# robustrobotics/multi_view_stereonet

Measured on AMD Instinct MI355X. Metric: depthmaps/sec at 512x256, 64 hypotheses, 2 src views; L1 vs ref, higher is better.
Workload: dtype f32; 1 GPU; GTA-SfM-shaped 512x256, D=64 hypotheses, 2 source views, cost-volume filter + 5 refiners; global_batch=256, parallelism=dp1 (independent images, all-gather of metric rows)

## Files before the change

include/mvsn_hip.h:

```cpp
#ifndef MVSN_HIP_H
#define MVSN_HIP_H

#include <stddef.h>
#include <stdint.h>

#ifdef __cplusplus
extern "C" {
#endif

#define MVSN_ABI_VERSION 7

#define MVSN_E_BADARG (-1)
#define MVSN_E_TOOLARGE (-2)
#define MVSN_E_WORKSPACE (-3)

typedef void *mvsn_stream_t;

int mvsn_abi_version(void);
const char *mvsn_last_error(void);

int mvsn_plane_sweep_setup(const float *T_right_in_left, const float *K_lvl0, const float *K_lvl4,
                           int n_chains, int rows4, int cols4, int num_idepth_samples,
                           float *idepth_samples, float *H_lvl4, float *H_inc, float *H_lvl0_plane0,
                           float *baseline, mvsn_stream_t stream);
int mvsn_plane_sweep_setup_sources(const float *const *T_right_in_lefts, int n_sources, const float *K_lvl0,
                                   const float *K_lvl4, int batch, int rows4, int cols4, int num_idepth_samples,
                                   float *idepth_samples, float *H_lvl4, float *H_inc, float *H_lvl0_plane0,
                                   float *baseline, mvsn_stream_t stream);

int mvsn_plane_sweep_setup_path(const float *K_lvl0_host, const float *K_lvl4_host, int rows4, int cols4);

int mvsn_homography_warp(const float *image, const float *H, int batch, int channels, int n_planes,
                         int rows, int cols, float *volume, uint8_t *mask, mvsn_stream_t stream);

#define MVSN_CHAIN_AUTO 0
#define MVSN_CHAIN_DIRECT 1
#define MVSN_CHAIN_WINOGRAD 2
#define MVSN_CHAIN_STEPWISE 3
#define MVSN_CHAIN_BANDED 4
size_t mvsn_feature_refiner_packed_floats(void);
int mvsn_pack_feature_refiner(const float *conv0_w, const float *conv0_b, const float *bn0_w,
                              const float *bn0_b, const float *res0_w, const float *res0_b,
                              const float *res0_bn_w, const float *res0_bn_b, const float *final_w,
                              const float *final_b, float *packed, mvsn_stream_t stream);
size_t mvsn_incremental_cost_volume_workspace_bytes(int n_chains, int rows, int cols);
int mvsn_incremental_cost_volume_form(int rows, int cols);
int mvsn_incremental_cost_volume_form_for(int n_chains, int rows, int cols);
size_t mvsn_incremental_cost_volume_workspace_bytes_for(int n_chains, int num_idepth_samples, int rows, int cols,
                                                        int form);
int mvsn_incremental_cost_volume_resolve(int n_chains, int num_idepth_samples, int rows, int cols, int form,
                                         int coresident_allowed, int guarded, size_t out[8]);
size_t mvsn_incremental_cost_volume_status_offset(int n_chains, int rows, int cols);
int mvsn_incremental_cost_volume_banded_groups(int n_chains, int rows, int cols);
int mvsn_incremental_cost_volume(const float *src_image_lvl4, const float *H_lvl4, const float *H_inc,
                                 const float *plane0_features, const float *left_features,
                                 const float *refiner_packed, int n_chains, int batch,
                                 int num_idepth_samples, int rows, int cols, float *cost_volume,
                                 uint8_t *mask_volume, float *feature_volume, void *workspace,
                                 size_t workspace_bytes, int form, mvsn_stream_t stream);
size_t mvsn_incremental_cost_volume_repair_workspace_bytes(int n_chains, int rows, int cols);
int mvsn_incremental_cost_volume_guarded(const float *src_image_lvl4, const float *H_lvl4, const float *H_inc,
                                         const float *plane0_features, const float *left_features,
                                         const float *refiner_packed, int n_chains, int batch,
                                         int num_idepth_samples, int rows, int cols, float *cost_volume,
                                         uint8_t *mask_volume, float *feature_volume, void *workspace,
                                         size_t workspace_bytes, int form, void *repair_workspace,
                                         size_t repair_workspace_bytes, unsigned *sticky_status, mvsn_stream_t stream);
int mvsn_incremental_cost_volume_bf16(const float *src_image_lvl4, const float *H_lvl4, const float *H_inc,
                                         const float *plane0_features, const float *left_features,
                                         const float *refiner_packed, int n_chains, int batch,
                                         int num_idepth_samples, int rows, int cols, void *cost_volume_bf16,
                                         uint8_t *mask_volume, float *feature_volume, void *workspace,
                                         size_t workspace_bytes, int form, void *repair_workspace,
                                         size_t repair_workspace_bytes, unsigned *sticky_status, mvsn_stream_t stream);

typedef struct {
  int n;
  int c_in;
  int c_out;
  int depth;
  int rows, cols;
  int kd, kh, kw;
  int stride;
  int dilation;
  int precision;
} mvsn_conv_desc;

#define MVSN_CONV_FP32 0
#define MVSN_CONV_BF16X3 1
#define MVSN_CONV_FP32_WINO 2
#define MVSN_CONV_BF16 3
int mvsn_conv_bf16x3_supported(const mvsn_conv_desc *desc);
int mvsn_conv_forward_bf16_storage(const mvsn_conv_desc *desc, const void *in, int in_is_bf16,
                                   const float *weight_packed, const float *bias, const float *in_stats,
                                   const float *in_gamma, const float *in_beta, void *out, int out_is_bf16,
                                   float *out_partials, mvsn_stream_t stream);
int mvsn_conv_winograd_supported(const mvsn_conv_desc *desc);

size_t mvsn_conv_packed_floats(const mvsn_conv_desc *desc);
int mvsn_conv_pack_weights(const mvsn_conv_desc *desc, const float *weight, float *packed,
                           mvsn_stream_t stream);
int mvsn_conv_num_tiles(const mvsn_conv_desc *desc);
int mvsn_conv_forward(const mvsn_conv_desc *desc, const float *in, const float *weight_packed,
                      const float *bias, const float *in_stats, const float *in_gamma,
                      const float *in_beta, const float *in_residual, float *out_staged, float *out,
                      float *out_partials, mvsn_stream_t stream);
int mvsn_conv_forward_blocks(const mvsn_conv_desc *desc, const float *const *in_blocks, const int *block_channels,
                             int num_blocks, const float *weight_packed, const float *bias, float *out,
                             float *out_partials, mvsn_stream_t stream);
typedef struct mvsn_apply_job {
  const float *x, *stats, *gamma, *beta;
  const float *residual, *r_stats, *r_gamma, *r_beta;
  float *out;
  int n;
  int reverse;
  long spatial;
} mvsn_apply_job;
int mvsn_conv_forward_carry(const mvsn_conv_desc *desc, const float *in, const float *weight_packed, const float *bias,
                            const float *in_stats, const float *in_gamma, const float *in_beta, float *out,
                            float *out_partials, const mvsn_apply_job *job, int *carried, mvsn_stream_t stream);
int mvsn_groupnorm_finalize(const float *partials, int n, int tiles, float *stats, mvsn_stream_t stream);
size_t mvsn_groupnorm_finalize_split_workspace_bytes(int n, int tiles);
int mvsn_groupnorm_finalize_split(const float *partials, int n, int tiles, float *stats, void *workspace,
                                  size_t workspace_bytes, mvsn_stream_t stream);
int mvsn_groupnorm_lrelu_apply(const float *x, const float *stats, int stat_tiles, const float *gamma, const float *beta,
                               const float *residual, const float *r_stats, const float *r_gamma, const float *r_beta,
                               int n, long spatial, float *out, mvsn_stream_t stream);

int mvsn_conv_to1_supported(int rows, int cols);
int mvsn_conv_to1(const float *in, const float *weight, const float *bias, const float *prior, const float *fx,
                  int n, int depth, int rows, int cols, int kd, float *out, mvsn_stream_t stream);
int mvsn_conv_to1_volume_norm(const float *in_raw, const float *in_stats, const float *in_gamma, const float *in_beta,
                              const float *weight, const float *bias, int n, int depth, int rows, int cols, float *out,
                              mvsn_stream_t stream);
int mvsn_conv_to1_block(const float *in_raw, const float *in_stats, int stat_tiles, const float *in_gamma,
                        const float *in_beta, const float *in_residual, const float *weight, const float *bias,
                        const float *prior, const float *fx, int n, int rows, int cols, float *out, mvsn_stream_t stream);

int mvsn_soft_argmin(const float *cost, const float *idepth_samples, int n, int num_idepth_samples,
                     int pixels, float *idepth, mvsn_stream_t stream);

int mvsn_soft_argmin_confidence(const float *cost, const float *idepth_samples, int n, int num_idepth_samples,
                                int pixels, float *idepth, float *confidence, mvsn_stream_t stream);
int mvsn_confidence_fuse_sources(const float *confidence, int n_sources, int batch, int pixels, float *out,
                                 mvsn_stream_t stream);
int mvsn_confidence_mask(const float *confidence, const uint8_t *valid, long count, float min_confidence,
                         uint8_t *out, mvsn_stream_t stream);
int mvsn_fusion_gather(const float *maps, const int *view, const int *pixel, int n_views, long pixels_per_view,
                       long count, float *out, mvsn_stream_t stream);

int mvsn_channel_l2_norm(const float *x, int n, int channels, long pixels, float *out, mvsn_stream_t stream);
int mvsn_idepth_scale(const float *prior, const float *fx, int n, long pixels, float *out, mvsn_stream_t stream);
int mvsn_refiner_epilogue(const float *prior, const float *fx, const float *delta, int n, long pixels, float *out,
                          mvsn_stream_t stream);

int mvsn_upsample_bilinear(const float *in, int n, int channels, int rows_in, int cols_in, int rows_out,
                           int cols_out, float *out, mvsn_stream_t stream);
int mvsn_upsample_prior(const float *in, const float *fx, int n, int rows_in, int cols_in, int rows_out, int cols_out,
                        float *out, float *out_scaled, mvsn_stream_t stream);
int mvsn_upsample_mask(const uint8_t *in, int n, int channels, int rows_in, int cols_in, int rows_out,
                       int cols_out, uint8_t *out, mvsn_stream_t stream);

int mvsn_area_downsample(const float *in, int n, int channels, int rows_in, int cols_in, float *out,
                         mvsn_stream_t stream);

int mvsn_image_pyramid_supported(int rows, int cols, int levels);
int mvsn_image_pyramid(const float *in, int n, int channels, int rows, int cols, int levels, float *const *out_levels,
                       mvsn_stream_t stream);
int mvsn_prepare_cameras(const float *K, const float *T_right_in_left, int batch, int n_sources, int levels,
                         const int *level_sizes_dev, float *K_pyr, float *T_normalised, float *T_inverse_normalised,
                         float *baseline, mvsn_stream_t stream);

int mvsn_fuse_sources(const float *raw, const float *refined, const float *baseline, const uint8_t *mask,
                      int n_sources, int batch, int num_idepth_samples, int pixels, int refined_aliases_raw,
                      float *raw_out, float *refined_out, uint8_t *mask_out, mvsn_stream_t stream);

int mvsn_idepth_reproject_blocks(int pixels);
int mvsn_idepth_reproject(const float *K, const float *T_other_in_this, const float *idepth, const float *other_idepth,
                          const uint8_t *other_mask, int batch, int rows, int cols, float *idepth_in_other,
                          float *other_sampled, uint8_t *other_mask_sampled, uint8_t *invalid, float *uv,
                          float *absdiff_partials, mvsn_stream_t stream);
int mvsn_occlusion_mask(const float *idepth_in_other, const float *other_sampled, const uint8_t *invalid,
                        const float *absdiff_partials, int batch, int pixels, uint8_t *mask, mvsn_stream_t stream);
int mvsn_masked_l1(const float *a, const float *b, const uint8_t *skip_a, const uint8_t *skip_b, long n, int accumulate,
                   float *loss, mvsn_stream_t stream);

typedef struct {
  const float *in[3];
  int channels[3], sample_mod[3];
  const float *block_scale;
  int scale_mod, scale_block;
  int head_chunks, n_blocks;
  int dilation[6];
  const float *weights, *params;
  int tail_mode;
  const float *prior, *fx;
  int fx_mod;
  float *out;
} mvsn_tower_desc;
int mvsn_tower_16x32(const mvsn_tower_desc *desc, int n_samples, mvsn_stream_t stream);

int mvsn_depth_metrics_blocks(long pixels);
int mvsn_depth_metrics(const float *idepth_est, const float *depth_true, const float *baseline, int batch, long pixels,
                       float min_depth, float max_depth, double *partials, double *rows, mvsn_stream_t stream);

size_t mvsn_fusion_workspace_bytes(int n_ref, int n_slots, int rows, int cols);
int mvsn_fusion_consistency(const float *depth, const uint8_t *valid, const float *K, const float *T_cam_in_world,
                            const int *ref_views, const int *neighbours, int n_views, int n_ref, int n_slots, int rows,
                            int cols, float max_reproj_px, float max_rel_depth, int min_consistent, float *fused_depth,
                            uint8_t *count, int64_t *total, void *workspace, size_t workspace_bytes,
                            mvsn_stream_t stream);
int mvsn_fusion_emit(const float *fused_depth, const float *images, const int *ref_views, int n_ref, int rows, int cols,
                     int n_slots, const void *workspace, size_t workspace_bytes, long capacity, float *points,
                     uint8_t *colors, int *view, int *pixel, mvsn_stream_t stream);

#define MVSN_VOXEL_STATUS_RANGE 1
#define MVSN_VOXEL_STATUS_TABLE 2
size_t mvsn_voxel_workspace_bytes(long n);
int mvsn_voxel_assign(const float *points, long n, float voxel_size, float inv_voxel_size, float origin_x,
                      float origin_y, float origin_z, int64_t *result, void *workspace, size_t workspace_bytes,
                      mvsn_stream_t stream);
int mvsn_voxel_merge(const float *points, const uint8_t *colors, long n, float voxel_size, float inv_voxel_size,
                     float origin_x, float origin_y, float origin_z, void *workspace, size_t workspace_bytes,
                     long capacity, void *accumulators, float *out_points, uint8_t *out_colors, int *count,
                     int64_t *first, int64_t *inverse, mvsn_stream_t stream);

int mvsn_depth_normals(const float *depth, const uint8_t *valid, const float *K, const float *T_cam_in_world,
                       int n_views, int rows, int cols, float max_rel_step, float *normals, mvsn_stream_t stream);
int mvsn_normals_gather(const float *normals, const int *view, const int *pixel, int n_views, long pixels_per_view,
                        long count, float *out, mvsn_stream_t stream);
int mvsn_voxel_normals(const float *normals, const int64_t *inverse, long n, long m, void *accumulators, float *out,
                       mvsn_stream_t stream);

#define MVSN_CLOUD_STATUS_RANGE 1
#define MVSN_CLOUD_STATUS_TABLE 2
size_t mvsn_cloud_workspace_bytes(long n_target);
int mvsn_cloud_index_build(const float *target, long n, float cell, float inv_cell, int64_t *status, void *workspace,
                           size_t workspace_bytes, mvsn_stream_t stream);
int mvsn_cloud_nearest(const float *query, long nq, float inv_cell, float r2, const void *workspace,
                       size_t workspace_bytes, long n_target, float *dist2, int64_t *index, int *within,
                       mvsn_stream_t stream);

size_t mvsn_cloud_register_workspace_bytes(long n_source);
int mvsn_cloud_register_system(const float *source, long n_source, const float *weights, const float *target,
                               const float *target_normals, long n_target, float inv_cell, float r2,
                               const void *index_workspace, size_t index_workspace_bytes, const float *T,
                               const float *centre, void *workspace, size_t workspace_bytes, double *H, double *b,
                               double *sums, int64_t *index, float *residual, mvsn_stream_t stream);
int mvsn_cloud_register(const float *source, long n_source, const float *weights, const float *target,
                        const float *target_normals, long n_target, float inv_cell, float r2,
                        const void *index_workspace, size_t index_workspace_bytes, const float *T_init,
                        const float *centre, int iterations, long min_points, double min_pivot, void *workspace,
                        size_t workspace_bytes, float *T_out, double *history, int *status, double *information,
                        mvsn_stream_t stream);

int mvsn_cloud_normals(const float *query, long nq, const float *viewpoint, long viewpoint_rows, float cell,
                       float inv_cell, float r2, long min_neighbours, double min_gap, const void *index_workspace,
                       size_t index_workspace_bytes, long n_target, float *normals, float *eigenvalues, int *count,
                       mvsn_stream_t stream);

int mvsn_cloud_knn(const float *query, long nq, int k, int exclude_self, float cell, float inv_cell, float r2,
                   const void *index_workspace, size_t index_workspace_bytes, long n_target, float *dist2,
                   int64_t *index, int *within, double *mean, mvsn_stream_t stream);
size_t mvsn_cloud_mean_stats_workspace_bytes(long n);
int mvsn_cloud_mean_stats(const double *mean, long n, void *workspace, size_t workspace_bytes, double *stats,
                          mvsn_stream_t stream);

int mvsn_cloud_fpfh(const float *points, const float *normals, long n, float cell, float inv_cell, float r2,
                    long min_neighbours, const void *index_workspace, size_t index_workspace_bytes, int *spfh,
                    int *pairs, float *features, mvsn_stream_t stream);
int mvsn_cloud_feature_nearest(const float *query, long nq, const float *target, long nt, int dim, int64_t *index,
                               float *dist2, float *second_dist2, mvsn_stream_t stream);
int mvsn_cloud_feature_mutual(const int64_t *index, long nq, const int64_t *back, long nt, unsigned char *mutual,
                              mvsn_stream_t stream);
size_t mvsn_cloud_ransac_workspace_bytes(void);
int mvsn_cloud_ransac(const float *source, long ns, const float *target, long nt, const int64_t *correspondences, long c,
                      float r2, double edge_similarity, long hypotheses, unsigned long long seed, void *workspace,
                      size_t workspace_bytes, float *T, double *T64, int64_t *best, unsigned char *inlier,
                      mvsn_stream_t stream);

int mvsn_tsdf_camera_batch(void);
int mvsn_tsdf_integrate(const float *depth, const uint8_t *valid, const float *weights, const float *images,
                        const float *K, const float *T_cam_in_world, int n_views, int rows, int cols, int nx, int ny,
                        int nz, float voxel_size, float origin_x, float origin_y, float origin_z, float trunc,
                        float min_depth, float *sdf_sum, float *weight, float *color_sum, mvsn_stream_t stream);
size_t mvsn_tsdf_workspace_bytes(int nx, int ny, int nz);
int mvsn_tsdf_classify(const float *sdf_sum, const float *weight, int nx, int ny, int nz, float min_weight,
                       int64_t *result, void *workspace, size_t workspace_bytes, mvsn_stream_t stream);
int mvsn_tsdf_extract(const float *sdf_sum, const float *weight, const float *color_sum, int nx, int ny, int nz,
                      float voxel_size, float origin_x, float origin_y, float origin_z, float min_weight,
                      const void *workspace, size_t workspace_bytes, long n_vertices, long n_quads, float *vertices,
                      float *normals, uint8_t *colors, int64_t *faces, int64_t *cell, mvsn_stream_t stream);

size_t mvsn_tsdf_raycast_workspace_bytes(int nx, int ny, int nz);
int mvsn_tsdf_raycast(const float *sdf_sum, const float *weight, const float *color_sum, int nx, int ny, int nz,
                      float voxel_size, float origin_x, float origin_y, float origin_z, const float *K,
                      const float *T_cam_in_world, int n_views, int rows, int cols, float min_weight, float min_depth,
                      float max_depth, float step, void *workspace, size_t workspace_bytes, float *depth,
                      float *normals, float *colors, float *weight_out, mvsn_stream_t stream);

size_t mvsn_tsdf_align_workspace_bytes(int nx, int ny, int nz, int n_views, int rows, int cols, int stride);
int mvsn_tsdf_align_system(const float *sdf_sum, const float *weight, int nx, int ny, int nz, float voxel_size,
                           float origin_x, float origin_y, float origin_z, const float *depth, const uint8_t *valid,
                           const float *weights, const float *K, const float *T_cam_in_world, int n_views, int rows,
                           int cols, int stride, float min_weight, float band, void *workspace, size_t workspace_bytes,
                           double *H, double *b, double *sums, float *residual, mvsn_stream_t stream);
int mvsn_tsdf_align(const float *sdf_sum, const float *weight, int nx, int ny, int nz, float voxel_size, float origin_x,
                    float origin_y, float origin_z, const float *depth, const uint8_t *valid, const float *weights,
                    const float *K, const float *T_cam_in_world, int n_views, int rows, int cols, int stride,
                    float min_weight, float band, int iterations, long min_pixels, double min_pivot, void *workspace,
                    size_t workspace_bytes, float *T_out, double *history, int *status, double *information,
                    mvsn_stream_t stream);

#define MVSN_MESH_STATUS_WORKSPACE 1
size_t mvsn_mesh_workspace_bytes(long n_vertices, long n_faces);
int mvsn_mesh_components_label(const int64_t *faces, long n_vertices, long n_faces, int64_t *result, void *workspace,
                               size_t workspace_bytes, mvsn_stream_t stream);
int mvsn_mesh_components_emit(const int64_t *faces, long n_vertices, long n_faces, void *workspace,
                              size_t workspace_bytes, long n_components, int64_t *vertex_label, int64_t *face_label,
                              int64_t *vertex_count, int64_t *face_count, int64_t *first, mvsn_stream_t stream);
int mvsn_mesh_select(const int64_t *vertex_label, const int64_t *face_label, const uint8_t *keep, long n_vertices,
                     long n_faces, long n_components, int64_t *result, void *workspace, size_t workspace_bytes,
                     mvsn_stream_t stream);
int mvsn_mesh_compact(const float *vertices, const float *normals, const uint8_t *colors, const int64_t *cell,
                      const int64_t *faces, const int64_t *face_label, const uint8_t *keep, long n_vertices, long n_faces,
                      long n_components, const void *workspace, size_t workspace_bytes, long n_vertices_out,
                      long n_faces_out, float *out_vertices, float *out_normals, uint8_t *out_colors, int64_t *out_cell,
                      int64_t *out_faces, int64_t *vertex_rows, int64_t *face_rows, mvsn_stream_t stream);

#define MVSN_CLUSTER_STATUS_WORKSPACE 1
size_t mvsn_cloud_cluster_workspace_bytes(long n);
int mvsn_cloud_cluster_label(const float *points, long n, float inv_cell, float r2, long min_points,
                             const void *index_workspace, size_t index_workspace_bytes, int *within, uint8_t *core,
                             int64_t *result, void *workspace, size_t workspace_bytes, mvsn_stream_t stream);
int mvsn_cloud_cluster_emit(const float *points, long n, float inv_cell, float r2, const void *index_workspace,
                            size_t index_workspace_bytes, const uint8_t *core, void *workspace, size_t workspace_bytes,
                            long n_clusters, int64_t *label, int64_t *count, int64_t *core_count, int64_t *first,
                            mvsn_stream_t stream);

#define MVSN_RENDER_MAX_RADIUS 8
size_t mvsn_cloud_render_workspace_bytes(int n_views, int rows, int cols);
int mvsn_cloud_render_camera_batch(void);
int mvsn_cloud_render(const float *points, long n, const uint8_t *colors, const float *normals, const float *K,
                      const float *T_cam_in_world, int n_views, int rows, int cols, int radius, float min_depth,
                      float max_depth, void *workspace, size_t workspace_bytes, float *depth, int64_t *index,
                      uint8_t *out_colors, float *out_normals, mvsn_stream_t stream);
int mvsn_cloud_visibility(const float *points, long n, const float *depth, const float *maps, int channels,
                          const float *K, const float *T_cam_in_world, int n_views, int rows, int cols, float rel_tol,
                          float min_depth, uint8_t *visible, int *count, float *values, mvsn_stream_t stream);

#define MVSN_MESH_SAMPLE_STATUS_NO_AREA 1
size_t mvsn_mesh_sample_workspace_bytes(long n_faces);
int mvsn_mesh_sample_prefix(const float *vertices, long n_vertices, const int64_t *faces, long n_faces, int64_t *result,
                            void *workspace, size_t workspace_bytes, mvsn_stream_t stream);
int mvsn_mesh_sample_draw(const float *vertices, long n_vertices, const int64_t *faces, long n_faces,
                          const void *workspace, size_t workspace_bytes, long n, uint64_t seed, const float *normals,
                          const uint8_t *colors, float *points, int64_t *face, float *weights, float *out_normals,
                          uint8_t *out_colors, mvsn_stream_t stream);

#define MVSN_MESH_NEAREST_BOX_CELLS 512
#define MVSN_MESH_NEAREST_STATUS_RANGE 1
int mvsn_mesh_nearest_box_cells(void);
size_t mvsn_mesh_nearest_workspace_bytes(long n_pairs, long n_large);
int mvsn_mesh_nearest_count(const float *vertices, long n_vertices, const int64_t *faces, long n_faces, float inv_cell,
                            int64_t *result, mvsn_stream_t stream);
int mvsn_mesh_nearest_build(const float *vertices, long n_vertices, const int64_t *faces, long n_faces, float inv_cell,
                            long n_pairs, long n_large, void *workspace, size_t workspace_bytes, mvsn_stream_t stream);
int mvsn_mesh_nearest(const float *query, long nq, const float *vertices, long n_vertices, const int64_t *faces,
                      long n_faces, float inv_cell, float r2, long n_pairs, long n_large, const void *workspace,
                      size_t workspace_bytes, float *dist2, int64_t *face, float *point, float *weights, int *within,
                      mvsn_stream_t stream);

int mvsn_copy(void *dst, const void *src, size_t nbytes, mvsn_stream_t stream);
int mvsn_copy_many(void *const *dst, const void *const *src, const size_t *nbytes, int count, mvsn_stream_t stream);
int mvsn_gather_focal(const float *const *K_pyr, int levels, int batch, float *fx, mvsn_stream_t stream);
int mvsn_gather_strided(const float *src, int count, long stride, float *dst, mvsn_stream_t stream);

int mvsn_debug_set_band_flags(int flags);

int mvsn_debug_set_wino_rowphase(int mode);

int mvsn_debug_wino_plan(const mvsn_conv_desc *desc, int carrying, int out[8]);

int mvsn_debug_conv_plan(const mvsn_conv_desc *desc, int mode, int out[8]);

int mvsn_selftest_mfma(mvsn_stream_t stream);

#ifdef __cplusplus
}
#endif
#endif
```

multi_view_stereonet_amd/_native.py:

```python
import ctypes
import os
from ctypes import c_char_p, c_int, c_long, c_size_t, c_void_p, POINTER, Structure

import torch

_LIB_PATH = os.path.join(os.path.dirname(os.path.abspath(__file__)), "libmvsn_hip.so")
_lib = None


class ConvDesc(Structure):
    _fields_ = [("n", c_int), ("c_in", c_int), ("c_out", c_int), ("depth", c_int), ("rows", c_int),
                ("cols", c_int), ("kd", c_int), ("kh", c_int), ("kw", c_int), ("stride", c_int),
                ("dilation", c_int), ("precision", c_int)]


class ApplyJob(Structure):
    _fields_ = [("x", c_void_p), ("stats", c_void_p), ("gamma", c_void_p), ("beta", c_void_p),
                ("residual", c_void_p), ("r_stats", c_void_p), ("r_gamma", c_void_p), ("r_beta", c_void_p),
                ("out", c_void_p), ("n", c_int), ("reverse", c_int), ("spatial", c_long)]


class TowerDesc(Structure):
    _fields_ = [("inp", c_void_p * 3), ("channels", c_int * 3), ("sample_mod", c_int * 3), ("block_scale", c_void_p),
                ("scale_mod", c_int), ("scale_block", c_int), ("head_chunks", c_int), ("n_blocks", c_int),
                ("dilation", c_int * 6), ("weights", c_void_p), ("params", c_void_p), ("tail_mode", c_int),
                ("prior", c_void_p), ("fx", c_void_p), ("fx_mod", c_int), ("out", c_void_p)]


CONV_FP32, CONV_BF16X3, CONV_FP32_WINO, CONV_BF16 = 0, 1, 2, 3
CHAIN_AUTO, CHAIN_DIRECT, CHAIN_WINOGRAD, CHAIN_STEPWISE, CHAIN_BANDED = 0, 1, 2, 3, 4
ABI_VERSION = 7


SIGNATURES = {
    "mvsn_abi_version": (c_int, []),
    "mvsn_last_error": (c_char_p, []),
    "mvsn_plane_sweep_setup": (c_int, [c_void_p] * 3 + [c_int] * 4 + [c_void_p] * 5 + [c_void_p]),
    "mvsn_plane_sweep_setup_sources": (c_int, [POINTER(c_void_p), c_int, c_void_p, c_void_p] + [c_int] * 4 + [c_void_p] * 5 + [c_void_p]),
    "mvsn_plane_sweep_setup_path": (c_int, [c_void_p, c_void_p, c_int, c_int]),
    "mvsn_gather_focal": (c_int, [POINTER(c_void_p), c_int, c_int, c_void_p, c_void_p]),
    "mvsn_homography_warp": (c_int, [c_void_p] * 2 + [c_int] * 5 + [c_void_p] * 2 + [c_void_p]),
    "mvsn_feature_refiner_packed_floats": (c_size_t, []),
    "mvsn_pack_feature_refiner": (c_int, [c_void_p] * 11 + [c_void_p]),
    "mvsn_incremental_cost_volume_workspace_bytes": (c_size_t, [c_int] * 3),
    "mvsn_incremental_cost_volume_form": (c_int, [c_int] * 2),
    "mvsn_incremental_cost_volume_form_for": (c_int, [c_int] * 3),
    "mvsn_incremental_cost_volume_workspace_bytes_for": (c_size_t, [c_int] * 5),
    "mvsn_incremental_cost_volume_resolve": (c_int, [c_int] * 7 + [POINTER(c_size_t * 8)]),
    "mvsn_incremental_cost_volume_status_offset": (c_size_t, [c_int] * 3),
    "mvsn_incremental_cost_volume_banded_groups": (c_int, [c_int] * 3),
    "mvsn_incremental_cost_volume": (c_int, [c_void_p] * 6 + [c_int] * 5 + [c_void_p] * 4 + [c_size_t, c_int, c_void_p]),
    "mvsn_incremental_cost_volume_repair_workspace_bytes": (c_size_t, [c_int] * 3),
    "mvsn_incremental_cost_volume_guarded": (c_int, [c_void_p] * 6 + [c_int] * 5 + [c_void_p] * 4 +
                                             [c_size_t, c_int, c_void_p, c_size_t, c_void_p, c_void_p]),
    "mvsn_incremental_cost_volume_bf16": (c_int, [c_void_p] * 6 + [c_int] * 5 + [c_void_p] * 4 +
                                          [c_size_t, c_int, c_void_p, c_size_t, c_void_p, c_void_p]),
    "mvsn_conv_bf16x3_supported": (c_int, [POINTER(ConvDesc)]),
    "mvsn_conv_forward_bf16_storage": (c_int, [c_void_p, c_void_p, c_int, c_void_p, c_void_p, c_void_p, c_void_p, c_void_p,
                                               c_void_p, c_int, c_void_p, c_void_p]),
    "mvsn_conv_winograd_supported": (c_int, [POINTER(ConvDesc)]),
    "mvsn_conv_packed_floats": (c_size_t, [POINTER(ConvDesc)]),
    "mvsn_conv_pack_weights": (c_int, [POINTER(ConvDesc), c_void_p, c_void_p, c_void_p]),
    "mvsn_conv_num_tiles": (c_int, [POINTER(ConvDesc)]),
    "mvsn_conv_forward": (c_int, [POINTER(ConvDesc)] + [c_void_p] * 10 + [c_void_p]),
    "mvsn_conv_forward_blocks": (c_int, [POINTER(ConvDesc), c_void_p, POINTER(c_int), c_int] + [c_void_p] * 4 + [c_void_p]),
    "mvsn_conv_forward_carry": (c_int, [POINTER(ConvDesc)] + [c_void_p] * 8 + [POINTER(ApplyJob), POINTER(c_int), c_void_p]),
    "mvsn_groupnorm_finalize": (c_int, [c_void_p, c_int, c_int, c_void_p, c_void_p]),
    "mvsn_groupnorm_finalize_split_workspace_bytes": (c_size_t, [c_int, c_int]),
    "mvsn_groupnorm_finalize_split": (c_int, [c_void_p, c_int, c_int, c_void_p, c_void_p, c_size_t, c_void_p]),
    "mvsn_groupnorm_lrelu_apply": (c_int, [c_void_p] * 2 + [c_int] + [c_void_p] * 6 + [c_int, c_long, c_void_p, c_void_p]),
    "mvsn_conv_to1_block": (c_int, [c_void_p] * 2 + [c_int] + [c_void_p] * 7 + [c_int] * 3 + [c_void_p, c_void_p]),
    "mvsn_debug_set_band_flags": (c_int, [c_int]),
    "mvsn_debug_set_wino_rowphase": (c_int, [c_int]),
    "mvsn_debug_wino_plan": (c_int, [POINTER(ConvDesc), c_int, POINTER(c_int * 8)]),
    "mvsn_debug_conv_plan": (c_int, [POINTER(ConvDesc), c_int, POINTER(c_int * 8)]),
    "mvsn_copy_many": (c_int, [c_void_p, c_void_p, c_void_p, c_int, c_void_p]),
    "mvsn_conv_to1_supported": (c_int, [c_int, c_int]),
    "mvsn_conv_to1_volume_norm": (c_int, [c_void_p] * 6 + [c_int] * 4 + [c_void_p, c_void_p]),
    "mvsn_conv_to1": (c_int, [c_void_p] * 5 + [c_int] * 5 + [c_void_p, c_void_p]),
    "mvsn_soft_argmin": (c_int, [c_void_p] * 2 + [c_int] * 3 + [c_void_p, c_void_p]),
    "mvsn_soft_argmin_confidence": (c_int, [c_void_p] * 2 + [c_int] * 3 + [c_void_p] * 2 + [c_void_p]),
    "mvsn_confidence_fuse_sources": (c_int, [c_void_p] + [c_int] * 3 + [c_void_p, c_void_p]),
    "mvsn_confidence_mask": (c_int, [c_void_p, c_void_p, c_long, ctypes.c_float, c_void_p, c_void_p]),
    "mvsn_fusion_gather": (c_int, [c_void_p] * 3 + [c_int, c_long, c_long, c_void_p, c_void_p]),
    "mvsn_channel_l2_norm": (c_int, [c_void_p, c_int, c_int, c_long, c_void_p, c_void_p]),
    "mvsn_idepth_scale": (c_int, [c_void_p, c_void_p, c_int, c_long, c_void_p, c_void_p]),
    "mvsn_refiner_epilogue": (c_int, [c_void_p, c_void_p, c_void_p, c_int, c_long, c_void_p, c_void_p]),
    "mvsn_upsample_bilinear": (c_int, [c_void_p] + [c_int] * 6 + [c_void_p, c_void_p]),
    "mvsn_upsample_prior": (c_int, [c_void_p, c_void_p] + [c_int] * 5 + [c_void_p] * 3),
    "mvsn_upsample_mask": (c_int, [c_void_p] + [c_int] * 6 + [c_void_p, c_void_p]),
    "mvsn_image_pyramid_supported": (c_int, [c_int] * 3),
    "mvsn_image_pyramid": (c_int, [c_void_p] + [c_int] * 5 + [POINTER(c_void_p), c_void_p]),
    "mvsn_prepare_cameras": (c_int, [c_void_p] * 2 + [c_int] * 3 + [c_void_p] * 5 + [c_void_p]),
    "mvsn_area_downsample": (c_int, [c_void_p] + [c_int] * 4 + [c_void_p, c_void_p]),
    "mvsn_fuse_sources": (c_int, [c_void_p] * 4 + [c_int] * 5 + [c_void_p] * 3 + [c_void_p]),
    "mvsn_idepth_reproject_blocks": (c_int, [c_int]),
    "mvsn_idepth_reproject": (c_int, [c_void_p] * 5 + [c_int] * 3 + [c_void_p] * 6 + [c_void_p]),
    "mvsn_occlusion_mask": (c_int, [c_void_p] * 4 + [c_int] * 2 + [c_void_p, c_void_p]),
    "mvsn_masked_l1": (c_int, [c_void_p] * 4 + [c_long, c_int, c_void_p, c_void_p]),
    "mvsn_tower_16x32": (c_int, [POINTER(TowerDesc), c_int, c_void_p]),
    "mvsn_depth_metrics_blocks": (c_int, [c_long]),
    "mvsn_depth_metrics": (c_int, [c_void_p] * 3 + [c_int, c_long, ctypes.c_float, ctypes.c_float, c_void_p, c_void_p, c_void_p]),
    "mvsn_fusion_workspace_bytes": (c_size_t, [c_int] * 4),
    "mvsn_fusion_consistency": (c_int, [c_void_p] * 6 + [c_int] * 5 + [ctypes.c_float] * 2 + [c_int] + [c_void_p] * 4 +
                                [c_size_t, c_void_p]),
    "mvsn_fusion_emit": (c_int, [c_void_p] * 3 + [c_int] * 4 + [c_void_p, c_size_t, c_long] + [c_void_p] * 4 + [c_void_p]),
    "mvsn_voxel_workspace_bytes": (c_size_t, [c_long]),
    "mvsn_voxel_assign": (c_int, [c_void_p, c_long] + [ctypes.c_float] * 5 + [c_void_p, c_void_p, c_size_t, c_void_p]),
    "mvsn_voxel_merge": (c_int, [c_void_p, c_void_p, c_long] + [ctypes.c_float] * 5 + [c_void_p, c_size_t, c_long] +
                         [c_void_p] * 6 + [c_void_p]),
    "mvsn_depth_normals": (c_int, [c_void_p] * 4 + [c_int] * 3 + [ctypes.c_float, c_void_p, c_void_p]),
    "mvsn_normals_gather": (c_int, [c_void_p] * 3 + [c_int, c_long, c_long, c_void_p, c_void_p]),
    "mvsn_voxel_normals": (c_int, [c_void_p, c_void_p, c_long, c_long, c_void_p, c_void_p, c_void_p]),
    "mvsn_cloud_workspace_bytes": (c_size_t, [c_long]),
    "mvsn_cloud_index_build": (c_int, [c_void_p, c_long] + [ctypes.c_float] * 2 + [c_void_p, c_void_p, c_size_t, c_void_p]),
    "mvsn_cloud_nearest": (c_int, [c_void_p, c_long] + [ctypes.c_float] * 2 + [c_void_p, c_size_t, c_long] +
                           [c_void_p] * 3 + [c_void_p]),
    "mvsn_cloud_register_workspace_bytes": (c_size_t, [c_long]),
    "mvsn_cloud_register_system": (c_int, [c_void_p, c_long] + [c_void_p] * 3 + [c_long] + [ctypes.c_float] * 2 +
                                   [c_void_p, c_size_t] + [c_void_p] * 2 + [c_void_p, c_size_t] + [c_void_p] * 5 + [c_void_p]),
    "mvsn_cloud_register": (c_int, [c_void_p, c_long] + [c_void_p] * 3 + [c_long] + [ctypes.c_float] * 2 +
                            [c_void_p, c_size_t] + [c_void_p] * 2 + [c_int, c_long, ctypes.c_double, c_void_p, c_size_t] +
                            [c_void_p] * 4 + [c_void_p]),
    "mvsn_cloud_normals": (c_int, [c_void_p, c_long, c_void_p, c_long] + [ctypes.c_float] * 3 + [c_long, ctypes.c_double] +
                           [c_void_p, c_size_t, c_long] + [c_void_p] * 3 + [c_void_p]),
    "mvsn_cloud_knn": (c_int, [c_void_p, c_long, c_int, c_int] + [ctypes.c_float] * 3 + [c_void_p, c_size_t, c_long] +
                       [c_void_p] * 4 + [c_void_p]),
    "mvsn_cloud_mean_stats_workspace_bytes": (c_size_t, [c_long]),
    "mvsn_cloud_mean_stats": (c_int, [c_void_p, c_long, c_void_p, c_size_t, c_void_p, c_void_p]),
    "mvsn_cloud_fpfh": (c_int, [c_void_p, c_void_p, c_long] + [ctypes.c_float] * 3 + [c_long, c_void_p, c_size_t] +
                        [c_void_p] * 3 + [c_void_p]),
    "mvsn_cloud_feature_nearest": (c_int, [c_void_p, c_long, c_void_p, c_long, c_int] + [c_void_p] * 3 + [c_void_p]),
    "mvsn_cloud_feature_mutual": (c_int, [c_void_p, c_long, c_void_p, c_long, c_void_p, c_void_p]),
    "mvsn_cloud_ransac_workspace_bytes": (c_size_t, []),
    "mvsn_cloud_ransac": (c_int, [c_void_p, c_long, c_void_p, c_long, c_void_p, c_long, ctypes.c_float, ctypes.c_double,
                                  c_long, ctypes.c_uint64, c_void_p, c_size_t] + [c_void_p] * 4 + [c_void_p]),
    "mvsn_tsdf_camera_batch": (c_int, []),
    "mvsn_tsdf_integrate": (c_int, [c_void_p] * 6 + [c_int] * 6 + [ctypes.c_float] * 6 + [c_void_p] * 3 + [c_void_p]),
    "mvsn_tsdf_workspace_bytes": (c_size_t, [c_int] * 3),
    "mvsn_tsdf_classify": (c_int, [c_void_p] * 2 + [c_int] * 3 + [ctypes.c_float, c_void_p, c_void_p, c_size_t, c_void_p]),
    "mvsn_tsdf_extract": (c_int, [c_void_p] * 3 + [c_int] * 3 + [ctypes.c_float] * 5 + [c_void_p, c_size_t, c_long, c_long] +
                          [c_void_p] * 5 + [c_void_p]),
    "mvsn_tsdf_raycast_workspace_bytes": (c_size_t, [c_int] * 3),
    "mvsn_tsdf_raycast": (c_int, [c_void_p] * 3 + [c_int] * 3 + [ctypes.c_float] * 4 + [c_void_p] * 2 + [c_int] * 3 +
                          [ctypes.c_float] * 4 + [c_void_p, c_size_t] + [c_void_p] * 4 + [c_void_p]),
    "mvsn_tsdf_align_workspace_bytes": (c_size_t, [c_int] * 7),
    "mvsn_tsdf_align_system": (c_int, [c_void_p] * 2 + [c_int] * 3 + [ctypes.c_float] * 4 + [c_void_p] * 5 + [c_int] * 4 +
                               [ctypes.c_float] * 2 + [c_void_p, c_size_t] + [c_void_p] * 4 + [c_void_p]),
    "mvsn_tsdf_align": (c_int, [c_void_p] * 2 + [c_int] * 3 + [ctypes.c_float] * 4 + [c_void_p] * 5 + [c_int] * 4 +
                        [ctypes.c_float] * 2 + [c_int, c_long, ctypes.c_double, c_void_p, c_size_t] + [c_void_p] * 4 + [c_void_p]),
    "mvsn_mesh_workspace_bytes": (c_size_t, [c_long] * 2),
    "mvsn_mesh_components_label": (c_int, [c_void_p, c_long, c_long, c_void_p, c_void_p, c_size_t, c_void_p]),
    "mvsn_mesh_components_emit": (c_int, [c_void_p, c_long, c_long, c_void_p, c_size_t, c_long] + [c_void_p] * 5 + [c_void_p]),
    "mvsn_mesh_select": (c_int, [c_void_p] * 3 + [c_long] * 3 + [c_void_p, c_void_p, c_size_t, c_void_p]),
    "mvsn_mesh_compact": (c_int, [c_void_p] * 7 + [c_long] * 3 + [c_void_p, c_size_t, c_long, c_long] + [c_void_p] * 7 +
                          [c_void_p]),
    "mvsn_mesh_sample_workspace_bytes": (c_size_t, [c_long]),
    "mvsn_mesh_sample_prefix": (c_int, [c_void_p, c_long, c_void_p, c_long, c_void_p, c_void_p, c_size_t, c_void_p]),
    "mvsn_mesh_sample_draw": (c_int, [c_void_p, c_long, c_void_p, c_long, c_void_p, c_size_t, c_long, ctypes.c_uint64] +
                              [c_void_p] * 7 + [c_void_p]),
    "mvsn_mesh_nearest_box_cells": (c_int, []),
    "mvsn_mesh_nearest_workspace_bytes": (c_size_t, [c_long] * 2),
    "mvsn_mesh_nearest_count": (c_int, [c_void_p, c_long, c_void_p, c_long, ctypes.c_float, c_void_p, c_void_p]),
    "mvsn_mesh_nearest_build": (c_int, [c_void_p, c_long, c_void_p, c_long, ctypes.c_float, c_long, c_long, c_void_p,
                                        c_size_t, c_void_p]),
    "mvsn_mesh_nearest": (c_int, [c_void_p, c_long, c_void_p, c_long, c_void_p, c_long] + [ctypes.c_float] * 2 +
                          [c_long, c_long, c_void_p, c_size_t] + [c_void_p] * 5 + [c_void_p]),
    "mvsn_cloud_cluster_workspace_bytes": (c_size_t, [c_long]),
    "mvsn_cloud_cluster_label": (c_int, [c_void_p, c_long] + [ctypes.c_float] * 2 + [c_long, c_void_p, c_size_t] +
                                 [c_void_p] * 3 + [c_void_p, c_size_t] + [c_void_p]),
    "mvsn_cloud_cluster_emit": (c_int, [c_void_p, c_long] + [ctypes.c_float] * 2 + [c_void_p, c_size_t, c_void_p] +
                                [c_void_p, c_size_t, c_long] + [c_void_p] * 4 + [c_void_p]),
    "mvsn_cloud_render_workspace_bytes": (c_size_t, [c_int] * 3),
    "mvsn_cloud_render_camera_batch": (c_int, []),
    "mvsn_cloud_render": (c_int, [c_void_p, c_long] + [c_void_p] * 4 + [c_int] * 4 + [ctypes.c_float] * 2 +
                          [c_void_p, c_size_t] + [c_void_p] * 4 + [c_void_p]),
    "mvsn_cloud_visibility": (c_int, [c_void_p, c_long, c_void_p, c_void_p, c_int, c_void_p, c_void_p] + [c_int] * 3 +
                              [ctypes.c_float] * 2 + [c_void_p] * 3 + [c_void_p]),
    "mvsn_copy": (c_int, [c_void_p, c_void_p, c_size_t, c_void_p]),
    "mvsn_gather_strided": (c_int, [c_void_p, c_int, c_long, c_void_p, c_void_p]),
    "mvsn_selftest_mfma": (c_int, [c_void_p]),
}


def library_path() -> str:
    return _LIB_PATH


def load():
    global _lib
    if _lib is not None:
        return _lib
    if not os.path.exists(_LIB_PATH):
        raise RuntimeError(
            f"{_LIB_PATH} is missing: the HIP extension has not been built "
            "(run `python -m multi_view_stereonet_amd.build` or __graft_entry__.build()). "
            "There is no CPU fallback for the plane-sweep path.")
    lib = ctypes.CDLL(_LIB_PATH)
    lib.mvsn_abi_version.restype, lib.mvsn_abi_version.argtypes = c_int, []
    if lib.mvsn_abi_version() != ABI_VERSION:
        raise RuntimeError(f"libmvsn_hip.so is ABI version {lib.mvsn_abi_version()}, this package needs {ABI_VERSION}: "
                           "rebuild it (python -m multi_view_stereonet_amd.build --force)")
    for name, (res, args) in SIGNATURES.items():
        fn = getattr(lib, name)
        fn.restype = res
        fn.argtypes = args
    _lib = lib
    return lib


def ptr(t):
    if t is None:
        return None
    if not t.is_cuda:
        raise RuntimeError("libmvsn_hip.so takes device (HBM) pointers; got a CPU tensor")
    if not t.is_contiguous():
        raise RuntimeError("libmvsn_hip.so takes dense tensors")
    return t.data_ptr()


def stream():
    return torch.cuda.current_stream().cuda_stream


def plane_sweep_setup_path(K_lvl0, K_lvl4, rows4: int, cols4: int):
    lib = load()
    K0, K4 = (k.detach().to("cpu", torch.float32).contiguous() for k in (K_lvl0, K_lvl4))
    return [lib.mvsn_plane_sweep_setup_path(K0[n].data_ptr(), K4[n].data_ptr(), rows4, cols4) for n in range(K0.shape[0])]


def check(rc: int, what: str):
    if rc != 0:
        msg = load().mvsn_last_error()
        raise RuntimeError(f"{what} failed (code {rc}): {msg.decode() if msg else ''}")


_coresident = {}


def _device_key(index: int) -> str:
    p = torch.cuda.get_device_properties(index)
    uuid = getattr(p, "uuid", None)
    if uuid is not None and str(uuid).strip("0-") != "":
        return str(uuid)
    return "pci-%04x-%02x-%02x" % (getattr(p, "pci_domain_id", 0), getattr(p, "pci_bus_id", index),
                                   getattr(p, "pci_device_id", 0))


def coresident_lock_path(index: int) -> str:
    root = os.environ.get("MVSN_LOCK_DIR") or "/tmp"
    return os.path.join(root, "mvsn_coresident_%s.lock" % _device_key(index).replace("/", "_"))


def coresident_right(index: int) -> bool:
    if index in _coresident:
        return _coresident[index][0]
    if os.environ.get("MVSN_CORESIDENT_LOCK", "1") == "0":
        _coresident[index] = (True, None)
        return True
    import fcntl
    try:
        old_mask = os.umask(0)
        try:
            f = os.fdopen(os.open(coresident_lock_path(index), os.O_RDWR | os.O_CREAT, 0o666), "r+")
        finally:
            os.umask(old_mask)
    except OSError:
        _coresident[index] = (True, None)
        return True
    try:
        fcntl.flock(f, fcntl.LOCK_EX | fcntl.LOCK_NB)
    except OSError:
        f.close()
        _coresident[index] = (False, None)
        return False
    try:
        f.seek(0)
        f.truncate()
        f.write("%d\n" % os.getpid())
        f.flush()
    except OSError:
        pass
    _coresident[index] = (True, f)
    return True


def release_coresident_right(index=None):
    for i in ([index] if index is not None else list(_coresident)):
        granted, f = _coresident.pop(i, (False, None))
        if f is not None:
            f.close()
```

multi_view_stereonet_amd/csrc/mvsn_conv.hip:

```cpp
#include "mvsn_resident.h"
#include "mvsn_conv_bf16x3.h"
#include "mvsn_conv_wino.h"

namespace mvsn {

constexpr int CV_THREADS = 256;
constexpr int CV_WAVES = 4;
constexpr int CV_TX = 32;
constexpr int CV_CK = 4;

#ifndef MVSN_TALL_TILE_MAX_DIL
#define MVSN_TALL_TILE_MAX_DIL 8
#endif
#ifndef MVSN_DMA_MAX_DIL
#define MVSN_DMA_MAX_DIL 8
#endif
constexpr int HD_TY = 8, HD_TX = 32, HD_ROWS = 2 * HD_TY + 3, HD_XS = 2 * HD_TX + 8;
constexpr int HD_CST = HD_ROWS * HD_XS + 4;

struct FastDiv {
  unsigned mul, shift;
};
static FastDiv make_fastdiv(unsigned d) {
  unsigned s = 0;
// ... 396 lines not shown
          }
        }
      }
    }
#pragma unroll
    for (int k = 0; k < WR; ++k) {
      const int idx = (tid + k * CV_THREADS) * 4;
      if (idx < WFL) *reinterpret_cast<floatx4 *>(wl + idx) = wreg[k];
    }
  };

#ifdef MVSN_DMA_STAMPS
  __shared__ unsigned long long ph_lds[8];
  const bool stamped = g_dma_stamps && blockIdx.x == gridDim.x / 3 && blockIdx.y == gridDim.y / 2 && tid == 0;
  unsigned long long ph_last = __builtin_readcyclecounter();
  const unsigned long long ph_t0 = ph_last;
  if (stamped) for (int k = 0; k < 8; ++k) ph_lds[k] = 0;
#endif
  stage_load(0);
  MFMA_PHASE(0);
  for (int chunk = 0; chunk < g.nchunks; ++chunk) {
    __syncthreads();
    MFMA_PHASE(1);
    stage_store(chunk);
    MFMA_PHASE(2);
    __syncthreads();
    MFMA_PHASE(3);
    if (chunk + 1 < g.nchunks) stage_load(chunk + 1);
    MFMA_PHASE(4);
    const float *wt = wl + lane;
    float fw[2][2], fb[2][NPT];
    auto read_tap = [&](int tap, int buf) {
      const int tz = tap / (KH * KW), ty = (tap / KW) % KH, tx = tap % KW;
      const float *bp = tile + (tz * g.HY + ty * g.dil) * g.XS + tx * g.dil;
      fw[buf][0] = wt[tap * 128];
      fw[buf][1] = CT == 2 ? wt[tap * 128 + 64] : 0.0f;
#pragma unroll
      for (int j = 0; j < NPT; ++j) fb[buf][j] = bp[lpos[j]];
    };
    if constexpr (KD == 1 && KW == 5 && STRIDE == 2 && V4) {
      float2 er[2][NPT][3];
      auto read_row = [&](int ky, int buf) {
        const float *bp = tile + ky * g.XS;
#pragma unroll
        for (int j = 0; j < NPT; ++j)
#pragma unroll
          for (int q = 0; q < 3; ++q) er[buf][j][q] = *reinterpret_cast<const float2 *>(bp + lpos[j] + 2 * q);
      };
      read_row(0, 0);
      fw[0][0] = wt[0], fw[0][1] = CT == 2 ? wt[64] : 0.0f;
#pragma unroll
      for (int ky = 0; ky < 5; ++ky) {
        const int rb = ky & 1;
        if (ky + 1 < 5) read_row(ky + 1, rb ^ 1);
#pragma unroll
        for (int kx = 0; kx < 5; ++kx) {
          const int tap = ky * 5 + kx, cur = tap & 1;
          if (tap + 1 < NTAPS) {
            fw[cur ^ 1][0] = wt[(tap + 1) * 128];
            fw[cur ^ 1][1] = CT == 2 ? wt[(tap + 1) * 128 + 64] : 0.0f;
          }
#pragma unroll
          for (int j = 0; j < NPT; ++j) {
            const float a = (kx & 1) ? er[rb][j][kx >> 1].y : er[rb][j][kx >> 1].x;
            acc[j][0] = mfma16x16x4(a, fw[cur][0], acc[j][0]);
            if (CT == 2) acc[j][CT - 1] = mfma16x16x4(a, fw[cur][1], acc[j][CT - 1]);
          }
        }
      }
    } else {
    read_tap(0, 0);
#pragma unroll
    for (int tap = 0; tap < NTAPS; ++tap) {
      const int cur = tap & 1;
      if (tap + 1 < NTAPS) read_tap(tap + 1, cur ^ 1);
#pragma unroll
      for (int j = 0; j < NPT; ++j) {
        acc[j][0] = mfma16x16x4(fb[cur][j], fw[cur][0], acc[j][0]);
        if (CT == 2) acc[j][CT - 1] = mfma16x16x4(fb[cur][j], fw[cur][1], acc[j][CT - 1]);
      }
    }
    }
    MFMA_PHASE(5);
  }

  conv_epilogue<NPT, CT>(g, acc, z0, y0, x0, tid, n, tile_id, bias, out, out_partials);
#ifdef MVSN_DMA_STAMPS
  MFMA_PHASE(6);
  if (stamped) {
    for (int k = 0; k < 7; ++k) g_dma_stamps[32 + k] = ph_lds[k];
    g_dma_stamps[39] = __builtin_readcyclecounter() - ph_t0;
  }
#endif
}

__device__ floatx4 g_zero16 = {0.f, 0.f, 0.f, 0.f};

template <int NPT, int IPC, int CT, int MODE>
__global__ __launch_bounds__(CV_THREADS, MODE <= 1 ? 4 : 2) void conv_dma_kernel(ConvGeom g, const float *__restrict__ in,
                                                                 const float *__restrict__ wpk,
                                                                 const float *__restrict__ bias,
                                                                 const float *__restrict__ in_stats,
                                                                 const float *__restrict__ in_gamma,
                                                                 const float *__restrict__ in_beta,
                                                                 const float *__restrict__ in_residual,
                                                                 float *__restrict__ out_staged,
                                                                 float *__restrict__ out,
                                                                 float *__restrict__ out_partials) {
  extern __shared__ __attribute__((aligned(16))) float smem[];
  constexpr ConvForm L{CV_DMA, NPT, 1, 3, 1, IPC, false};
  constexpr int NTAPS = 9;
  constexpr int WFL = L.wfl(), WSLOT = L.wslot(), NT = L.ntiles(MODE);
  constexpr int WRUNS = WSLOT / 256;
  const int tile_floats = CV_CK * g.dCST;
  const int stage_floats = tile_floats * NT + WSLOT;
  float *scsh = smem + 2 * stage_floats;

  const int tid = threadIdx.x, lane = tid & 63;
  const int wave = __builtin_amdgcn_readfirstlane(tid >> 6);
  const int n = blockIdx.y;
#ifdef MVSN_DMA_STAMPS
  unsigned long long *dbg = (blockIdx.x == gridDim.x / 3 && blockIdx.y == gridDim.y / 2 && tid == 0) ? g_dma_stamps : nullptr;
  int dbg_i = 0;
#endif
  DMA_STAMP();
#ifdef MVSN_DMA_STAMPS
  if (dbg) dbg[62] = wall_clock64();
#endif
  const int tile_id = xcd_tile_index(blockIdx.x, g.tiles);
  const int trow = fdiv(tile_id, g.fd_ntx), txi = tile_id - trow * g.ntx;
  const int tzi = fdiv(trow, g.fd_nty), tyi = trow - tzi * g.nty;
  const int z0 = tzi * g.TZ, y0 = tyi * g.TY, x0 = txi * CV_TX;
  const int gz0 = z0 - g.pd, gy0 = y0 - g.ph, gx0 = x0 - g.pw;
  const size_t in_plane = (size_t)g.H * g.W, in_chan = (size_t)g.D * in_plane;
  const float *inn = in + (size_t)n * g.cin * in_chan;
  const float *resn = (MODE == 2 && in_residual) ? in_residual + (size_t)n * g.cin * in_chan : nullptr;
  float *stgn = (MODE == 2 && out_staged) ? out_staged + (size_t)n * g.cin * in_chan : nullptr;

  int lpos[NPT];
#pragma unroll
  for (int j = 0; j < NPT; ++j) {
    const int pt = wave * NPT + j;
    const int xt = pt & 1, zz = fdiv(pt >> 1, g.fd_ty), yy = (pt >> 1) - zz * g.TY;
    const int xx = xt * 16 + (lane & 15);
    lpos[j] = (zz * g.HY + yy) * g.dXS + xx + (g.dpa - g.pw) + (lane >> 4) * g.dCST;
  }

  int goff[IPC];
  unsigned inimg = 0, interior = 0;
  const int tile_groups = g.HZ * g.HY * g.dq;
#pragma unroll
  for (int i = 0; i < IPC; ++i) {
    const int e = i * 64 + lane;
    int off = -1;
    if (i < g.dipc && e < tile_groups) {
      const int row = fdiv(e, g.fd_dq), q = e - row * g.dq;
      const int z = fdiv(row, g.fd_hy), y = row - z * g.HY;
      const int gz = gz0 + z, gy = gy0 + y, gx = x0 - g.dpa + 4 * q;
      if (gz >= 0 && gz < g.D && gy >= 0 && gy < g.H && gx >= 0 && gx < g.W) {
        off = (gz * g.H + gy) * g.W + gx;
        inimg |= 1u << i;
        if (z >= g.pd && z < g.pd + g.TZ && y >= g.ph && y < g.ph + g.TY && 4 * q >= g.dpa && 4 * q < g.dpa + CV_TX) interior |= 1u << i;
      }
    }
    goff[i] = off;
  }

  if (MODE >= 1 && tid < 32) {
    const int grp = tid >> 3;
    const float mean = in_stats[((size_t)n * 4 + grp) * 2 + 0];
    const float rstd = in_stats[((size_t)n * 4 + grp) * 2 + 1];
    const float sc = rstd * in_gamma[tid];
    scsh[tid] = sc;
    scsh[32 + tid] = in_beta[tid] - mean * sc;
  }

  const float *zero = reinterpret_cast<const float *>(&g_zero16);
  auto issue = [&](int chunk, int stage) {
    float *st = smem + stage * stage_floats;
    const int c = chunk * CV_CK + wave;
    const bool cok = c < g.cin;
    const float *src = inn + (size_t)(cok ? c : 0) * in_chan;
    float *dst = st + wave * g.dCST;
#pragma unroll
    for (int i = 0; i < IPC; ++i) {
      if (i < g.dipc) {
        const float *p = (cok && goff[i] >= 0) ? src + goff[i] : zero;
        __builtin_amdgcn_global_load_lds(MVSN_GPTR(p), MVSN_LPTR(dst + i * 256), 16, 0, 0);
      }
    }
    if constexpr (MODE == 2) {
      const float *rsrc = resn ? resn + (size_t)(cok ? c : 0) * in_chan : nullptr;
      float *rdst = st + tile_floats + wave * g.dCST;
#pragma unroll
      for (int i = 0; i < IPC; ++i) {
        if (i < g.dipc) {
          const float *p = (rsrc && cok && goff[i] >= 0) ? rsrc + goff[i] : zero;
          __builtin_amdgcn_global_load_lds(MVSN_GPTR(p), MVSN_LPTR(rdst + i * 256), 16, 0, 0);
        }
      }
    }
    const float *wsrc = wpk + (size_t)chunk * WFL;
    float *wdst = st + tile_floats * NT;
#pragma unroll
    for (int r = 0; r < (WRUNS + CV_WAVES - 1) / CV_WAVES; ++r) {
      const int run = r * CV_WAVES + wave;
      if (run < WRUNS) {
        const int idx = run * 256 + lane * 4;
        const float *p = idx < WFL ? wsrc + idx : zero;
        __builtin_amdgcn_global_load_lds(MVSN_GPTR(p), MVSN_LPTR(wdst + run * 256), 16, 0, 0);
      }
    }
  };

  floatx4 acc[NPT][CT];
#pragma unroll
  for (int j = 0; j < NPT; ++j)
#pragma unroll
    for (int t = 0; t < CT; ++t) acc[j][t] = floatx4{0.f, 0.f, 0.f, 0.f};

  issue(0, 0);
  DMA_STAMP();
  for (int chunk = 0; chunk < g.nchunks; ++chunk) {
    const int stage = chunk & 1;
    float *st = smem + stage * stage_floats;
    asm volatile("s_waitcnt vmcnt(0)" ::: "memory");
    DMA_STAMP();
    if constexpr (MODE >= 1) {
      if (chunk == 0) __syncthreads();
      const int c = chunk * CV_CK + wave;
      if (c < g.cin) {
        const float sc = scsh[c], sh = scsh[32 + c];
        float *tl = st + wave * g.dCST + lane * 4;
        float *stg = stgn ? stgn + (size_t)c * in_chan : nullptr;
#pragma unroll
        for (int i = 0; i < IPC; ++i) {
          if ((inimg >> i) & 1u) {
            floatx4 v = *reinterpret_cast<floatx4 *>(tl + i * 256);
#pragma unroll
            for (int r = 0; r < 4; ++r) v[r] = lrelu02(v[r] * sc + sh);
            if constexpr (MODE == 2) {
              const floatx4 rv = *reinterpret_cast<const floatx4 *>(tl + tile_floats + i * 256);
#pragma unroll
              for (int r = 0; r < 4; ++r) v[r] += rv[r];
            }
            *reinterpret_cast<floatx4 *>(tl + i * 256) = v;
            if (MODE == 2 && stg && ((interior >> i) & 1u)) *reinterpret_cast<floatx4 *>(stg + goff[i]) = v;
          }
        }
      }
    }
    __syncthreads();
    DMA_STAMP();
    if (chunk + 1 < g.nchunks) issue(chunk + 1, stage ^ 1);
    DMA_STAMP();

    const float *tile = st;
    const float *wt = st + tile_floats * NT + lane;
    float fw[2][2], fb[2][NPT];
    auto read_tap = [&](int tap, int buf) {
      const int tz = tap / 9, ty = (tap / 3) % 3, tx = tap % 3;
      const float *bp = tile + (tz * g.HY + ty * g.dil) * g.dXS + tx * g.dil;
      fw[buf][0] = wt[tap * 128];
      fw[buf][1] = CT == 2 ? wt[tap * 128 + 64] : 0.0f;
#pragma unroll
      for (int j = 0; j < NPT; ++j) fb[buf][j] = bp[lpos[j]];
    };
    read_tap(0, 0);
#pragma unroll
    for (int tap = 0; tap < NTAPS; ++tap) {
      const int cur = tap & 1;
      if (tap + 1 < NTAPS) read_tap(tap + 1, cur ^ 1);
#pragma unroll
      for (int j = 0; j < NPT; ++j) {
        acc[j][0] = mfma16x16x4(fb[cur][j], fw[cur][0], acc[j][0]);
        if (CT == 2) acc[j][CT - 1] = mfma16x16x4(fb[cur][j], fw[cur][1], acc[j][CT - 1]);
      }
    }
    DMA_STAMP();
  }

  conv_epilogue<NPT, CT>(g, acc, z0, y0, x0, tid, n, tile_id, bias, out, out_partials);
  DMA_STAMP();
#ifdef MVSN_DMA_STAMPS
  if (dbg) dbg[63] = wall_clock64();
#endif
}

constexpr int HD_KSTEPS = 19;
static_assert(3 * HD_CST < 65536, "k-step offsets are packed as 16-bit values");

#ifndef MVSN_HEAD_WGS_PER_CU
#define MVSN_HEAD_WGS_PER_CU 3
#endif
#ifndef MVSN_HEAD_CNTWAIT
#define MVSN_HEAD_CNTWAIT 0
#endif
#ifndef MVSN_HEAD_ABLATE
#define MVSN_HEAD_ABLATE 0
#endif
#ifndef MVSN_HEAD_ST_AUX
#define MVSN_HEAD_ST_AUX 0
#endif
__global__ __launch_bounds__(256, MVSN_HEAD_WGS_PER_CU) void conv5x5s2_head_kernel(const float *__restrict__ in, const float *__restrict__ wpk,
                                                             const float *__restrict__ bias, int H, int W, int Ho,
                                                             int Wo, int ntx, int tiles, int total,
                                                             float *__restrict__ out) {
  __shared__ __attribute__((aligned(16))) float ring[2][3 * HD_CST];
  const int tid = threadIdx.x, lane = tid & 63;
  const int wave = __builtin_amdgcn_readfirstlane(tid >> 6);
  const size_t plane = (size_t)H * W;

  const int kk = lane >> 4, cl = lane & 15;
  float wf[HD_KSTEPS][2];
  unsigned kpk[(HD_KSTEPS + 1) / 2] = {};
#pragma unroll
  for (int ks = 0; ks < HD_KSTEPS; ++ks) {
    const int k = 4 * ks + kk;
    const bool live = k < 75;
    const int ch = live ? k / 25 : 0, tap = live ? k - ch * 25 : 0;
    wf[ks][0] = live ? wpk[tap * 128 + ch * 16 + cl] : 0.0f;
    wf[ks][1] = live ? wpk[tap * 128 + 64 + ch * 16 + cl] : 0.0f;
    const unsigned ko = ch * HD_CST + (tap / 5) * HD_XS + (tap % 5) + 2;
    kpk[ks >> 1] |= (ks & 1) ? ko << 16 : ko;
  }
  const float bv0 = bias ? bias[cl] : 0.0f, bv1 = bias ? bias[16 + cl] : 0.0f;

  constexpr int CG = HD_ROWS * (HD_XS / 4);
  constexpr int CP = (CG + 63) / 64;
  constexpr int NP = (3 * CP + 3) / 4;
  int prel[NP], pqx[NP];
#pragma unroll
  for (int i = 0; i < NP; ++i) {
    const int pc = wave + 4 * i, k = pc % CP;
    const int gi = k * 64 + lane, row = gi / (HD_XS / 4), q = gi - row * (HD_XS / 4);
    pqx[i] = gi < CG ? 4 * q - 4 : -0x40000000;
    prel[i] = (row - 2) * W + 4 * q - 4;
  }
  auto issue = [&](int id, int slot) {
    const int n = id / tiles, t = id - n * tiles;
    const int tyi = t / ntx, txi = t - tyi * ntx;
    const int org = 2 * (tyi * HD_TY) * W + 2 * (txi * HD_TX), x2 = 2 * (txi * HD_TX);
    const float *inn = in + (size_t)n * 3 * plane;
#pragma unroll
    for (int i = 0; i < NP; ++i) {
      const int pc = wave + 4 * i;
      if (pc < 3 * CP) {
        const int c = pc / CP, k = pc - c * CP;
        const int gx = x2 + pqx[i];
        const unsigned voff = (gx >= 0 && gx < W) ? (unsigned)((org + prel[i]) * 4) : 0xFFFFFFFFu;
        if (pqx[i] > -0x40000000 && !(MVSN_HEAD_ABLATE & 2))
          __builtin_amdgcn_raw_ptr_buffer_load_lds(
              __builtin_amdgcn_make_buffer_rsrc(const_cast<float *>(inn + (size_t)c * plane), 0, (int)(plane * 4), 0x00020000),
              (__attribute__((address_space(3))) void *)(&ring[slot][c * HD_CST + k * 256]), 16, (int)voff, 0, 0, 0);
      }
    }
  };

  const int pbase0 = (4 * wave) * HD_XS + 2 * cl;
  const int oplane = Ho * Wo;

  int id = blockIdx.x;
  if (id < total) issue(id, 0);
  for (int it = 0; id < total; id += gridDim.x, ++it) {
    const int slot = it & 1;
    if (MVSN_HEAD_CNTWAIT && it > 0) asm volatile("s_waitcnt vmcnt(8)" ::: "memory");
    else asm volatile("s_waitcnt vmcnt(0)" ::: "memory");
    __syncthreads();
    if (id + (int)gridDim.x < total) issue(id + gridDim.x, slot ^ 1);
    const float *tile0 = &ring[0][0] + slot * (3 * HD_CST) + pbase0;

    floatx4 acc[4][2];
#pragma unroll
    for (int j = 0; j < 4; ++j) acc[j][0] = acc[j][1] = floatx4{0.f, 0.f, 0.f, 0.f};
#pragma unroll
    for (int ks = 0; ks < ((MVSN_HEAD_ABLATE & 4) ? 1 : HD_KSTEPS); ++ks) {
      const int ko = (ks & 1) ? (int)(kpk[ks >> 1] >> 16) : (int)(kpk[ks >> 1] & 0xffffu);
#pragma unroll
      for (int j = 0; j < 4; ++j) {
        const float a = tile0[ko + (j >> 1) * 2 * HD_XS + (j & 1) * 32];
        acc[j][0] = mfma16x16x4(a, wf[ks][0], acc[j][0]);
        acc[j][1] = mfma16x16x4(a, wf[ks][1], acc[j][1]);
      }
    }

    const int n = id / tiles, t = id - n * tiles;
    const int tyi = t / ntx, txi = t - tyi * ntx;
    const int y0 = tyi * HD_TY, x0 = txi * HD_TX;
    const __amdgpu_buffer_rsrc_t osrd =
        __builtin_amdgcn_make_buffer_rsrc(out + (size_t)n * 32 * oplane, 0, (int)((size_t)32 * oplane * 4), 0x00020000);
    unsigned ovoff[2];
#pragma unroll
    for (int hx = 0; hx < 2; ++hx) {
      const int ox = x0 + hx * 16 + 4 * kk;
      ovoff[hx] = ox < Wo ? (unsigned)((cl * oplane + ox) * 4) : 0xFFFFFFFFu;
    }
#pragma unroll
    for (int tt = 0; tt < 2; ++tt) {
      const float bv = tt ? bv1 : bv0;
#pragma unroll
      for (int j = 0; j < 4; ++j) {
        const int pt = wave * 4 + j;
        const int oy = y0 + (pt >> 1);
        floatx4 v = acc[j][tt];
        v[0] += bv, v[1] += bv, v[2] += bv, v[3] += bv;
        if (!(MVSN_HEAD_ABLATE & 1) || v[0] == 12345.f)
        __builtin_amdgcn_raw_buffer_store_b128(__builtin_bit_cast(__attribute__((ext_vector_type(4))) unsigned, v), osrd,
                                               oy < Ho ? (int)ovoff[pt & 1] : -1, oy < Ho ? (tt * 16 * oplane + oy * Wo) * 4 : 0, MVSN_HEAD_ST_AUX);
      }
    }
  }
}

__global__ void mfma_selftest_kernel(int *bad) {
  const int lane = threadIdx.x;
  const float a = 1.0f + (float)(lane & 15) + 17.0f * (float)(lane >> 4);
  const float b = 3.0f + 5.0f * (float)(lane >> 4) - 2.0f * (float)(lane & 15);
  floatx4 c = {0.f, 0.f, 0.f, 0.f};
  c = mfma16x16x4(a, b, c);
  int wrong = 0;
  for (int r = 0; r < 4; ++r) {
    const int i = (lane >> 4) * 4 + r, j = lane & 15;
    float ref = 0.f;
    for (int k = 0; k < 4; ++k) ref += (1.0f + i + 17.0f * k) * (3.0f + 5.0f * k - 2.0f * j);
    if (fabsf(ref - c[r]) > 1e-3f) wrong++;
  }
  if (wrong) atomicAdd(bad, wrong);
}

static bool conv_head_ok(const ConvGeom &g, int mode, bool head_call) {
  return head_call && mode == 0 && g.cin == 3 && g.cout == 32 && g.kd == 1 && g.kh == 5 && g.kw == 5 && g.stride == 2 &&
         g.dil == 1 && g.D == 1 && (g.W & 7) == 0 &&
         (size_t)g.H * g.W * 4 < ((size_t)1 << 31) && (size_t)32 * g.Ho * g.Wo * 4 < ((size_t)1 << 31);
}

static int conv_select(const ConvGeom &g, int mode, bool head_call) {
  if (conv_head_ok(g, mode, head_call)) return cv_find_form(ConvForm{CV_HEAD, 4, 1, 5, 2, 0, false});
  ConvForm f = {CV_STAGED, g.TY == 16 ? 8 : 4, g.kd, g.kh, g.stride, g.se <= 3 ? 3 : 6, g.v4 != 0};
  if (g.dma && g.dipc <= 6)
    f.kind = CV_DMA, f.se = g.dipc <= 4 ? 4 : 6;
  else if (g.kd == 3 || g.kh == 5) f.npt = g.kd == 3 ? 8 : 4, f.se = g.v4 ? 2 : 6;
  return cv_find_form(f);
}
constexpr int conv_ct(const ConvForm &f, int cout) { return f.kind != CV_HEAD && f.kh == 3 && cout <= 16 ? 1 : 2; }
constexpr int conv_mode(const ConvForm &f, int mode) { return f.dma() ? mode : (f.kd == 1 && f.kh == 3 && mode == 2 ? 2 : 0); }

struct ConvTier {
  enum Kind { WINO, BF16, DIRECT } kind;
  bool ok;
  union { WinoGeom wg; Bf16x3Geom bg; ConvGeom g; };
};
static ConvTier conv_tier(const mvsn_conv_desc *desc) {
  ConvTier t{};
  const int p = desc ? desc->precision : MVSN_CONV_FP32;
  if (p == MVSN_CONV_FP32_WINO) t.kind = ConvTier::WINO, t.ok = wino_geom(desc, &t.wg);
  else if (p == MVSN_CONV_BF16X3 || p == MVSN_CONV_BF16) t.kind = ConvTier::BF16, t.ok = bf16x3_geom(desc, &t.bg);
  else t.kind = ConvTier::DIRECT, t.ok = make_geom(desc, &t.g);
  return t;
}

}

extern "C" int mvsn_conv_bf16x3_supported(const mvsn_conv_desc *desc) {
  mvsn::Bf16x3Geom g;
  return mvsn::bf16x3_geom(desc, &g) ? 1 : 0;
}

extern "C" int mvsn_conv_forward_bf16_storage(const mvsn_conv_desc *desc, const void *in, int in_is_bf16,
                                              const float *weight_packed, const float *bias, const float *in_stats,
                                              const float *in_gamma, const float *in_beta, void *out, int out_is_bf16,
                                              float *out_partials, mvsn_stream_t stream) {
  using namespace mvsn;
  MVSN_REQUIRE(desc && in && weight_packed && out, MVSN_E_BADARG, "mvsn_conv_forward_bf16_storage: null pointer");
  MVSN_REQUIRE(desc->precision == MVSN_CONV_BF16 && desc->kd == 3, MVSN_E_BADARG,
               "mvsn_conv_forward_bf16_storage: 3x3x3 layers with desc.precision = MVSN_CONV_BF16");
  Bf16x3Geom bg;
  MVSN_REQUIRE(bf16x3_geom(desc, &bg), MVSN_E_BADARG, "mvsn_conv_forward_bf16_storage: layer has no bf16 form");
  MVSN_REQUIRE(!in_stats || (in_gamma && in_beta), MVSN_E_BADARG, "mvsn_conv_forward_bf16_storage: input transform needs gamma/beta");
  MVSN_REQUIRE(bg.n <= 65535, MVSN_E_TOOLARGE, "mvsn_conv_forward_bf16_storage: batch too large for one launch");
  MVSN_REQUIRE(((size_t)in & 3) == 0 && ((size_t)out & 7) == 0, MVSN_E_BADARG, "mvsn_conv_forward_bf16_storage: alignment");
  MVSN_REQUIRE(!in_is_bf16 || (desc->cols & 1) == 0, MVSN_E_BADARG,
               "mvsn_conv_forward_bf16_storage: a bf16 input needs an even number of columns (aligned two-element loads)");
  return bf16_storage_launch(bg, in, in_is_bf16 != 0, weight_packed, bias, in_stats, in_gamma, in_beta, out,
                             out_is_bf16 != 0, out_partials, (hipStream_t)stream);
}

extern "C" int mvsn_conv_winograd_supported(const mvsn_conv_desc *desc) {
  mvsn::WinoGeom g;
  return mvsn::wino_geom(desc, &g) ? 1 : 0;
}

extern "C" size_t mvsn_conv_packed_floats(const mvsn_conv_desc *desc) {
  const mvsn::ConvTier t = mvsn::conv_tier(desc);
  if (!t.ok) return 0;
  if (t.kind == mvsn::ConvTier::WINO) return t.wg.packed_floats;
  if (t.kind == mvsn::ConvTier::BF16) return (size_t)desc->kd * 9 * 1024;
  return (size_t)t.g.nchunks * t.g.wfloats_chunk;
}

extern "C" int mvsn_conv_num_tiles(const mvsn_conv_desc *desc) {
  const mvsn::ConvTier t = mvsn::conv_tier(desc);
  if (!t.ok) return 0;
  if (t.kind == mvsn::ConvTier::WINO) return (int)(mvsn::wino_items(t.wg) * 32);
  if (t.kind == mvsn::ConvTier::BF16) return t.bg.tiles * 4;
  return t.g.tiles * 16;
}

extern "C" int mvsn_conv_pack_weights(const mvsn_conv_desc *desc, const float *weight, float *packed,
                                      mvsn_stream_t stream) {
  using namespace mvsn;
  MVSN_REQUIRE(weight && packed, MVSN_E_BADARG, "mvsn_conv_pack_weights: null pointer");
  const ConvTier t = conv_tier(desc);
  if (t.kind == ConvTier::WINO) {
    MVSN_REQUIRE(t.ok, MVSN_E_BADARG, "mvsn_conv_pack_weights: layer has no Winograd form");
    return mvsn::wino_pack(desc, weight, packed, (hipStream_t)stream);
  }
  if (t.kind == ConvTier::BF16) {
    MVSN_REQUIRE(t.ok, MVSN_E_BADARG, "mvsn_conv_pack_weights: layer has no bf16x3 form");
    return mvsn::bf16x3_pack(desc, weight, packed, (hipStream_t)stream);
  }
  MVSN_REQUIRE(t.ok, MVSN_E_BADARG, "mvsn_conv_pack_weights: unsupported descriptor");
  const ConvGeom &g = t.g;
  const int total = g.nchunks * g.ntaps * 128;
  hipLaunchKernelGGL(mvsn::conv_pack_kernel, dim3((total + 255) / 256), dim3(256), 0, (hipStream_t)stream, weight,
                     g.cin, g.cout, g.ntaps, g.nchunks, packed);
  return mvsn::check_launch("mvsn_conv_pack_weights");
}

extern "C" int mvsn_conv_forward_blocks(const mvsn_conv_desc *desc, const float *const *in_blocks,
                                        const int *block_channels, int num_blocks, const float *weight_packed,
                                        const float *bias, float *out, float *out_partials, mvsn_stream_t stream) {
  using namespace mvsn;
  MVSN_REQUIRE(desc && in_blocks && block_channels && weight_packed && out, MVSN_E_BADARG,
               "mvsn_conv_forward_blocks: null pointer");
  MVSN_REQUIRE(num_blocks >= 1 && num_blocks <= 3, MVSN_E_BADARG, "mvsn_conv_forward_blocks: 1..3 blocks");
  MVSN_REQUIRE(desc->precision == MVSN_CONV_FP32_WINO, MVSN_E_BADARG,
               "mvsn_conv_forward_blocks: only the Winograd form takes channel blocks");
  WinoGeom wg;
  MVSN_REQUIRE(wino_geom(desc, &wg), MVSN_E_BADARG, "mvsn_conv_forward_blocks: layer has no Winograd form");
  MVSN_REQUIRE(wg.n <= 65535, MVSN_E_TOOLARGE, "mvsn_conv_forward_blocks: batch too large for one launch");
  int sum = 0;
  for (int b = 0; b < num_blocks; ++b) {
    MVSN_REQUIRE(in_blocks[b] && block_channels[b] >= 1, MVSN_E_BADARG, "mvsn_conv_forward_blocks: empty block");
    MVSN_REQUIRE((reinterpret_cast<uintptr_t>(in_blocks[b]) & 15) == 0, MVSN_E_BADARG,
                 "mvsn_conv_forward_blocks: blocks must be 16-byte aligned");
    sum += block_channels[b];
  }
  MVSN_REQUIRE(sum == wg.cin, MVSN_E_BADARG, "mvsn_conv_forward_blocks: block channels do not add up to c_in");
  WinoBlocks wb;
  wb.cb0 = block_channels[0];
  wb.cb1 = num_blocks > 1 ? block_channels[1] : 0;
  wb.in1 = num_blocks > 1 ? in_blocks[1] : in_blocks[0];
  wb.in2 = num_blocks > 2 ? in_blocks[2] : in_blocks[0];
  return wino_launch(wg, in_blocks[0], weight_packed, bias, nullptr, nullptr, nullptr, out, out_partials,
                     (hipStream_t)stream, &wb);
}

extern "C" int mvsn_conv_forward(const mvsn_conv_desc *desc, const float *in, const float *weight_packed,
                                 const float *bias, const float *in_stats, const float *in_gamma,
                                 const float *in_beta, const float *in_residual, float *out_staged, float *out,
                                 float *out_partials, mvsn_stream_t stream) {
  using namespace mvsn;
  MVSN_REQUIRE(in && weight_packed && out, MVSN_E_BADARG, "mvsn_conv_forward: null pointer");
  const ConvTier t = conv_tier(desc);
  if (t.kind == ConvTier::WINO) {
    MVSN_REQUIRE(t.ok, MVSN_E_BADARG, "mvsn_conv_forward: layer has no Winograd form");
    MVSN_REQUIRE(!in_residual && !out_staged, MVSN_E_BADARG, "mvsn_conv_forward: Winograd form has no residual folding");
    MVSN_REQUIRE(!in_stats || (in_gamma && in_beta && t.wg.cin == 32), MVSN_E_BADARG,
                 "mvsn_conv_forward: input transform needs gamma/beta and 32 channels");
    MVSN_REQUIRE(t.wg.n <= 65535, MVSN_E_TOOLARGE, "mvsn_conv_forward: batch too large for one launch");
    return wino_launch(t.wg, in, weight_packed, bias, in_stats, in_gamma, in_beta, out, out_partials,
                       (hipStream_t)stream);
  }
  if (t.kind == ConvTier::BF16) {
    MVSN_REQUIRE(t.ok, MVSN_E_BADARG, "mvsn_conv_forward: layer has no bf16x3 form");
    MVSN_REQUIRE(!in_residual && !out_staged, MVSN_E_BADARG, "mvsn_conv_forward: bf16x3 has no residual folding");
    MVSN_REQUIRE(!in_stats || (in_gamma && in_beta), MVSN_E_BADARG, "mvsn_conv_forward: input transform needs gamma/beta");
    MVSN_REQUIRE(t.bg.n <= 65535, MVSN_E_TOOLARGE, "mvsn_conv_forward: batch too large for one launch");
    return bf16x3_launch(t.bg, in, weight_packed, bias, in_stats, in_gamma, in_beta, out, out_partials,
                         (hipStream_t)stream);
  }
  const ConvGeom &g = t.g;
  MVSN_REQUIRE(t.ok, MVSN_E_BADARG, "mvsn_conv_forward: unsupported descriptor");
  MVSN_REQUIRE(!in_stats || (in_gamma && in_beta), MVSN_E_BADARG, "mvsn_conv_forward: input transform needs gamma/beta");
  MVSN_REQUIRE(!in_stats || g.cin == 32, MVSN_E_BADARG, "mvsn_conv_forward: input transform needs 32 channels");
  MVSN_REQUIRE(!out_partials || g.cout == 32, MVSN_E_BADARG, "mvsn_conv_forward: partials need 32 output channels");
  MVSN_REQUIRE(!in_residual || in_stats, MVSN_E_BADARG, "mvsn_conv_forward: in_residual needs the input transform");
  MVSN_REQUIRE(!(in_residual || out_staged) || (g.kd == 1 && g.kh == 3 && g.stride == 1), MVSN_E_BADARG,
               "mvsn_conv_forward: residual / staged output only for 2-D 3x3 stride-1 layers");
  MVSN_REQUIRE(g.n <= 65535, MVSN_E_TOOLARGE, "mvsn_conv_forward: batch too large for one launch");
  const int mode = (in_residual || out_staged) ? 2 : (in_stats ? 1 : 0);
  const int row = conv_select(g, mode, desc->precision == MVSN_CONV_FP32 && !out_partials && (((size_t)in | (size_t)out) & 15) == 0);
  MVSN_REQUIRE(row >= 0, MVSN_E_BADARG, "mvsn_conv_forward: no kernel form for this layer");
  static_assert(CV_CK == CV_WAVES, "one DMA channel per wave");
  const int kernel = (row * 2 + conv_ct(CV_FORMS[row], g.cout) - 1) * 3 + conv_mode(CV_FORMS[row], mode);
  return with_form_row(kernel, std::make_index_sequence<CV_NFORMS * 6>{}, [&](auto K) -> int {
    constexpr ConvForm F = CV_FORMS[K / 6];
    constexpr int CT = K / 3 % 2 + 1, MODE = K % 3;
    if constexpr (conv_ct(F, CT == 1 ? 16 : 32) != CT || conv_mode(F, MODE) != MODE) return MVSN_E_BADARG;
    else if constexpr (F.kind == CV_HEAD) {
      MVSN_REQUIRE((long long)g.tiles * g.n < (1ll << 31) - 65536, MVSN_E_TOOLARGE, "mvsn_conv_forward: batch too large for one launch");
      const int total = g.tiles * g.n, gx = std::min(total, MVSN_HEAD_WGS_PER_CU * device_cus());
      hipLaunchKernelGGL(conv5x5s2_head_kernel, dim3(gx), dim3(256), 0, (hipStream_t)stream, in, weight_packed, bias, g.H, g.W,
                         g.Ho, g.Wo, g.ntx, g.tiles, total, out);
      return check_launch("mvsn_conv_forward(5x5 stride-2 head)");
    } else {
      static LdsOptIn opt;
      const size_t lds = F.lds_bytes(g, MODE);
      auto run = [&](auto kern, const char *what) -> int {
        if (int rc = ensure_lds(opt, (const void *)kern, lds, what)) return rc;
        hipLaunchKernelGGL(kern, dim3(g.tiles, g.n), dim3(CV_THREADS), lds, (hipStream_t)stream, g, in, weight_packed, bias,
                           in_stats, in_gamma, in_beta, in_residual, out_staged, out, out_partials);
        return check_launch(what);
      };
      if constexpr (F.dma()) return run(conv_dma_kernel<F.npt, F.se, CT, MODE>, "mvsn_conv_forward(dma)");
      else return run(conv_mfma_kernel<F.npt, F.kd, F.kh, F.kh, F.stride, F.se, CT, MODE == 2, F.v4>, "mvsn_conv_forward");
    }
  });
}

extern "C" int mvsn_debug_conv_plan(const mvsn_conv_desc *desc, int mode, int out[8]) {
  const mvsn::ConvTier t = mvsn::conv_tier(desc);
  const int row = out && t.kind == mvsn::ConvTier::DIRECT && t.ok ? mvsn::conv_select(t.g, mode, desc->precision == MVSN_CONV_FP32) : -1;
  if (row < 0) return 0;
  const mvsn::ConvForm &f = mvsn::CV_FORMS[row];
  out[0] = row, out[1] = f.kind, out[2] = f.npt, out[3] = f.se, out[4] = f.v4, out[5] = mvsn::conv_ct(f, t.g.cout);
  out[6] = (int)f.lds_bytes(t.g, mvsn::conv_mode(f, mode)), out[7] = t.g.tiles;
  return mvsn::CV_NFORMS;
}

#ifdef MVSN_DMA_STAMPS
extern "C" int mvsn_debug_set_dma_stamps(void *buf) {
  return (int)hipMemcpyToSymbol(HIP_SYMBOL(mvsn::g_dma_stamps), &buf, sizeof(buf));
}
#endif

extern "C" int mvsn_conv_forward_carry(const mvsn_conv_desc *desc, const float *in, const float *weight_packed,
                                       const float *bias, const float *in_stats, const float *in_gamma,
                                       const float *in_beta, float *out, float *out_partials,
                                       const mvsn_apply_job *job, int *carried, mvsn_stream_t stream) {
  using namespace mvsn;
  if (carried) *carried = 0;
  if (!job)
    return mvsn_conv_forward(desc, in, weight_packed, bias, in_stats, in_gamma, in_beta, nullptr, nullptr, out,
                             out_partials, stream);
  MVSN_REQUIRE(job->x && job->stats && job->gamma && job->beta && job->out && job->n > 0 && job->spatial > 0,
               MVSN_E_BADARG, "mvsn_conv_forward_carry: bad job");
  MVSN_REQUIRE(in && weight_packed && out, MVSN_E_BADARG, "mvsn_conv_forward_carry: null pointer");
  WinoGeom wg;
  if (desc && desc->precision == MVSN_CONV_FP32_WINO && wino_geom(desc, &wg) && wino_can_carry(wg, job) &&
      (!in_stats || (in_gamma && in_beta)) && wg.n <= 65535) {
    if (carried) *carried = 1;
    return wino_launch(wg, in, weight_packed, bias, in_stats, in_gamma, in_beta, out, out_partials,
                       (hipStream_t)stream, nullptr, job);
  }
  if (int rc = mvsn_groupnorm_lrelu_apply(job->x, job->stats, 0, job->gamma, job->beta, job->residual, job->r_stats,
                                          job->r_gamma, job->r_beta, job->n, job->spatial, job->out, stream))
    return rc;
  return mvsn_conv_forward(desc, in, weight_packed, bias, in_stats, in_gamma, in_beta, nullptr, nullptr, out,
                           out_partials, stream);
}

extern "C" int mvsn_selftest_mfma(mvsn_stream_t stream) {
  int *dbad = nullptr;
  hipError_t e = hipMalloc(&dbad, sizeof(int));
  if (e != hipSuccess) return (int)e;
  (void)hipMemsetAsync(dbad, 0, sizeof(int), (hipStream_t)stream);
  hipLaunchKernelGGL(mvsn::mfma_selftest_kernel, dim3(1), dim3(64), 0, (hipStream_t)stream, dbad);
  (void)mvsn::bf16_selftest((hipStream_t)stream, dbad);
  int bad = -1;
  (void)hipMemcpyAsync(&bad, dbad, sizeof(int), hipMemcpyDeviceToHost, (hipStream_t)stream);
  (void)hipStreamSynchronize((hipStream_t)stream);
  (void)hipFree(dbad);
  if (bad != 0) {
    mvsn::set_error("mvsn_selftest_mfma: %d fragment elements differ from the scalar product", bad);
    return MVSN_E_BADARG - 100;
  }
  return 0;
}
```

multi_view_stereonet_amd/csrc/mvsn_misc.hip:

```cpp
#include "mvsn_geom.h"

namespace mvsn {

__global__ __launch_bounds__(256) void soft_argmin_kernel(const float *__restrict__ cost,
                                                          const float *__restrict__ samples, int D, int P,
                                                          float *__restrict__ out) {
  const int p = blockIdx.x * blockDim.x + threadIdx.x;
  const int n = blockIdx.y;
  if (p >= P) return;
  const float *c = cost + (size_t)n * D * P + p;
  const float *s = samples + (size_t)n * D;
  float m = -INFINITY;
  int d0 = 0;
  for (; d0 + 16 <= D; d0 += 16) {
    float v[16];
#pragma unroll
    for (int j = 0; j < 16; ++j) v[j] = c[(size_t)(d0 + j) * P];
#pragma unroll
    for (int j = 0; j < 16; ++j) m = fmaxf(m, -v[j]);
  }
  for (int d = d0; d < D; ++d) m = fmaxf(m, -c[(size_t)d * P]);
  float den = 0.0f, num = 0.0f;
  for (d0 = 0; d0 + 16 <= D; d0 += 16) {
    float v[16];
#pragma unroll
    for (int j = 0; j < 16; ++j) v[j] = c[(size_t)(d0 + j) * P];
#pragma unroll
    for (int j = 0; j < 16; ++j) {
      const float e = expf(-v[j] - m);
      den += e;
      num += e * s[d0 + j];
    }
  }
  for (int d = d0; d < D; ++d) {
    float e = expf(-c[(size_t)d * P] - m);
    den += e;
    num += e * s[d];
  }
  out[(size_t)n * P + p] = num / den;
}

__global__ __launch_bounds__(256) void soft_argmin_confidence_kernel(const float *__restrict__ cost,
                                                                     const float *__restrict__ samples, int D, int P,
                                                                     float *__restrict__ out,
                                                                     float *__restrict__ confidence) {
  const int p = blockIdx.x * blockDim.x + threadIdx.x;
  const int n = blockIdx.y;
  if (p >= P) return;
  const float *c = cost + (size_t)n * D * P + p;
  const float *s = samples + (size_t)n * D;
  float m = -INFINITY;
  int d0 = 0;
  for (; d0 + 16 <= D; d0 += 16) {
    float v[16];
#pragma unroll
    for (int j = 0; j < 16; ++j) v[j] = c[(size_t)(d0 + j) * P];
#pragma unroll
    for (int j = 0; j < 16; ++j) m = fmaxf(m, -v[j]);
  }
  for (int d = d0; d < D; ++d) m = fmaxf(m, -c[(size_t)d * P]);
  float den = 0.0f, num = 0.0f, idx = 0.0f;
  for (d0 = 0; d0 + 16 <= D; d0 += 16) {
    float v[16];
#pragma unroll
    for (int j = 0; j < 16; ++j) v[j] = c[(size_t)(d0 + j) * P];
#pragma unroll
    for (int j = 0; j < 16; ++j) {
      const float e = expf(-v[j] - m);
      den += e;
      num += e * s[d0 + j];
      idx += e * (float)(d0 + j);
    }
  }
  for (int d = d0; d < D; ++d) {
    float e = expf(-c[(size_t)d * P] - m);
    den += e;
    num += e * s[d];
    idx += e * (float)d;
  }
  out[(size_t)n * P + p] = num / den;
  const float expected = idx / den;
  float conf = NAN;
  if (expected == expected) {
    int i = (int)floorf(expected);
    i = i < 0 ? 0 : (i > D - 1 ? D - 1 : i);
    float w[4];
#pragma unroll
    for (int k = 0; k < 4; ++k) {
      const int d = i - 1 + k;
      const bool in = d >= 0 && d < D;
      w[k] = in ? c[(size_t)(in ? d : 0) * P] : INFINITY;
    }
    float sum = 0.0f;
#pragma unroll
    for (int k = 0; k < 4; ++k) sum += expf(-w[k] - m);
    conf = sum / den;
  }
  confidence[(size_t)n * P + p] = conf;
}

__global__ __launch_bounds__(256) void confidence_fuse_kernel(const float *__restrict__ conf, int S, int B, int P,
                                                              float *__restrict__ out) {
  const int p = blockIdx.x * blockDim.x + threadIdx.x;
  const int b = blockIdx.y;
  if (p >= P) return;
  float acc = conf[(size_t)b * P + p];
  for (int s = 1; s < S; ++s) {
    const float v = conf[((size_t)s * B + b) * P + p];
    acc = (v != v || v < acc) ? v : acc;
  }
  out[(size_t)b * P + p] = acc;
}

__global__ __launch_bounds__(256) void confidence_mask_kernel(const float *__restrict__ conf,
                                                              const uint8_t *__restrict__ valid, long count, float thr,
                                                              uint8_t *__restrict__ out) {
  const long i = (long)blockIdx.x * blockDim.x + threadIdx.x;
  if (i >= count) return;
  const bool keep = conf[i] >= thr && (valid == nullptr || valid[i] != 0);
  out[i] = keep ? 1 : 0;
}

__global__ __launch_bounds__(256) void channel_l2_norm_kernel(const float *__restrict__ x, int channels, long P,
                                                              float *__restrict__ out) {
  const long p = (long)blockIdx.x * blockDim.x + threadIdx.x;
  if (p >= P) return;
  const float *xp = x + (size_t)blockIdx.y * channels * P + p;
  float acc = 0.0f;
  for (int c = 0; c < channels; ++c) {
    const float v = xp[(size_t)c * P];
    acc += v * v;
  }
  out[(size_t)blockIdx.y * P + p] = sqrtf(acc);
}

template <bool EPI>
__global__ __launch_bounds__(256) void idepth_gain_kernel(const float *__restrict__ prior, const float *__restrict__ fx,
                                                          const float *__restrict__ delta, long P,
                                                          float *__restrict__ out) {
#pragma clang fp contract(off)
  const long p = (long)blockIdx.x * blockDim.x + threadIdx.x;
  if (p >= P) return;
  const float f = fx[blockIdx.y];
  const size_t i = (size_t)blockIdx.y * P + p;
  const float scaled = prior[i] * f;
  if constexpr (EPI) out[i] = relu_nan(scaled + delta[i]) / f;
  else out[i] = scaled;
}

struct ResizeTap {
  int i0, i1;
  float l0, l1;
};
__device__ __forceinline__ ResizeTap resize_tap(int dst, int in_size, int out_size) {
  float scale = (float)in_size / (float)out_size;
  float src = ((float)dst + 0.5f) * scale - 0.5f;
  if (src < 0.0f) src = 0.0f;
  ResizeTap t;
  t.i0 = (int)src;
  if (t.i0 > in_size - 1) t.i0 = in_size - 1;
  t.i1 = t.i0 + (t.i0 < in_size - 1 ? 1 : 0);
  t.l1 = src - (float)t.i0;
  t.l0 = 1.0f - t.l1;
  return t;
}

template <typename TIn, typename TOut, bool THRESH>
__global__ __launch_bounds__(256) void upsample_kernel(const TIn *__restrict__ in, int hin, int win, int hout,
                                                       int wout, TOut *__restrict__ out) {
  const int x = blockIdx.x * blockDim.x + threadIdx.x;
  const int y = blockIdx.y;
  const size_t plane = blockIdx.z;
  if (x >= wout) return;
  ResizeTap ty = resize_tap(y, hin, hout);
  ResizeTap tx = resize_tap(x, win, wout);
  const TIn *ip = in + plane * hin * win;
  float v00 = (float)ip[ty.i0 * win + tx.i0], v01 = (float)ip[ty.i0 * win + tx.i1];
  float v10 = (float)ip[ty.i1 * win + tx.i0], v11 = (float)ip[ty.i1 * win + tx.i1];
  float v = ty.l0 * (tx.l0 * v00 + tx.l1 * v01) + ty.l1 * (tx.l0 * v10 + tx.l1 * v11);
  if (THRESH)
    out[(plane * hout + y) * wout + x] = (TOut)(v > 0.5f ? 1 : 0);
  else
    out[(plane * hout + y) * wout + x] = (TOut)v;
}

__global__ __launch_bounds__(256) void upsample_gain_kernel(const float *__restrict__ in, const float *__restrict__ gain,
                                                            int hin, int win, int hout, int wout,
                                                            float *__restrict__ out, float *__restrict__ out_scaled) {
  const int x = blockIdx.x * blockDim.x + threadIdx.x;
  const int y = blockIdx.y;
  const size_t plane = blockIdx.z;
  if (x >= wout) return;
  ResizeTap ty = resize_tap(y, hin, hout);
  ResizeTap tx = resize_tap(x, win, wout);
  const float *ip = in + plane * hin * win;
  float v00 = ip[ty.i0 * win + tx.i0], v01 = ip[ty.i0 * win + tx.i1];
  float v10 = ip[ty.i1 * win + tx.i0], v11 = ip[ty.i1 * win + tx.i1];
  float v = ty.l0 * (tx.l0 * v00 + tx.l1 * v01) + ty.l1 * (tx.l0 * v10 + tx.l1 * v11);
  out[(plane * hout + y) * wout + x] = v;
  out_scaled[(plane * hout + y) * wout + x] = v * gain[plane];
}

__global__ __launch_bounds__(256) void upsample_mask16_kernel(const uint8_t *__restrict__ in, int hin, int win,
                                                              int hout, int wout, int groups_per_row,
                                                              size_t total_groups, uint8_t *__restrict__ out) {
  const size_t gid = (size_t)blockIdx.x * blockDim.x + threadIdx.x;
  if (gid >= total_groups) return;
  const int gx = (int)(gid % groups_per_row);
  const size_t rowid = gid / groups_per_row;
  const int y = (int)(rowid % hout);
  const size_t plane = rowid / hout;
  const int x16 = gx * 16;
  ResizeTap ty = resize_tap(y, hin, hout);
  const uint8_t *r0 = in + (plane * hin + ty.i0) * win;
  const uint8_t *r1 = in + (plane * hin + ty.i1) * win;
  uint32_t w[4] = {0, 0, 0, 0};
  uint8_t vals[16];
#pragma unroll
  for (int k = 0; k < 16; ++k) {
    const int x = x16 + k < wout ? x16 + k : wout - 1;
    ResizeTap tx = resize_tap(x, win, wout);
    const float v00 = (float)r0[tx.i0], v01 = (float)r0[tx.i1], v10 = (float)r1[tx.i0], v11 = (float)r1[tx.i1];
    const float v = ty.l0 * (tx.l0 * v00 + tx.l1 * v01) + ty.l1 * (tx.l0 * v10 + tx.l1 * v11);
    vals[k] = v > 0.5f ? 1 : 0;
    w[k >> 2] |= (uint32_t)vals[k] << (8 * (k & 3));
  }
  uint8_t *orow = out + rowid * wout;
  if (x16 + 15 < wout && (((size_t)(orow + x16)) & 15) == 0) {
    *reinterpret_cast<uint4 *>(orow + x16) = make_uint4(w[0], w[1], w[2], w[3]);
  } else {
#pragma unroll
    for (int k = 0; k < 16; ++k)
      if (x16 + k < wout) orow[x16 + k] = vals[k];
  }
}

__global__ __launch_bounds__(256) void upsample_mask2x_kernel(const uint8_t *__restrict__ in, int hin, int win,
                                                              int groups_per_row, size_t total_groups,
                                                              uint8_t *__restrict__ out) {
  const size_t gid = (size_t)blockIdx.x * blockDim.x + threadIdx.x;
  if (gid >= total_groups) return;
  const int gx = (int)(gid % groups_per_row);
  const size_t rowid = gid / groups_per_row;
  const uint2 w = *reinterpret_cast<const uint2 *>(in + rowid * win + gx * 8);
  typedef unsigned u32x4 __attribute__((ext_vector_type(4)));
  u32x4 o;
  o[0] = __builtin_amdgcn_perm(w.x, w.x, 0x01010000u);
  o[1] = __builtin_amdgcn_perm(w.x, w.x, 0x03030202u);
  o[2] = __builtin_amdgcn_perm(w.y, w.y, 0x01010000u);
  o[3] = __builtin_amdgcn_perm(w.y, w.y, 0x03030202u);
  uint8_t *dst = out + (rowid * 2) * (size_t)(win * 2) + gx * 16;
  __builtin_nontemporal_store(o, reinterpret_cast<u32x4 *>(dst));
  __builtin_nontemporal_store(o, reinterpret_cast<u32x4 *>(dst + win * 2));
}

__global__ __launch_bounds__(256) void area_downsample_kernel(const float *__restrict__ in, int hin, int win,
                                                              int hout, int wout, float *__restrict__ out) {
  const int x = blockIdx.x * blockDim.x + threadIdx.x;
  const int y = blockIdx.y;
  const size_t plane = blockIdx.z;
  if (x >= wout) return;
  const int y0 = (y * hin) / hout, y1 = ((y + 1) * hin + hout - 1) / hout;
  const int x0 = (x * win) / wout, x1 = ((x + 1) * win + wout - 1) / wout;
  const float *ip = in + plane * hin * win;
  float sum = 0.0f;
  for (int yy = y0; yy < y1; ++yy)
    for (int xx = x0; xx < x1; ++xx) sum += ip[yy * win + xx];
  out[(plane * hout + y) * wout + x] = sum / (float)((y1 - y0) * (x1 - x0));
}

__global__ __launch_bounds__(256) void fuse_idepth_kernel(const float *__restrict__ raw,
                                                          const float *__restrict__ refined,
                                                          const float *__restrict__ baseline, int S, int B, int P,
                                                          int alias, float *__restrict__ raw_out,
                                                          float *__restrict__ refined_out) {
  const int p = blockIdx.x * blockDim.x + threadIdx.x;
  const int b = blockIdx.y;
  if (p >= P) return;
  float sr = 0.0f, sf = 0.0f;
  for (int s = 0; s < S; ++s) {
    const size_t n = (size_t)s * B + b;
    const float base = baseline[n];
    float r = raw[n * P + p] / base;
    float f;
    if (alias) {
      r = r / base;
      f = r;
    } else {
      f = refined[n * P + p] / base;
    }
    sr += r;
    sf += f;
  }
  raw_out[(size_t)b * P + p] = sr / (float)S;
  refined_out[(size_t)b * P + p] = sf / (float)S;
}

__global__ __launch_bounds__(256) void fuse_mask_kernel(const uint8_t *__restrict__ mask, int S, int B, size_t DP,
                                                        uint8_t *__restrict__ out) {
  const size_t i = (size_t)blockIdx.x * blockDim.x + threadIdx.x;
  const int b = blockIdx.y;
  if (i >= DP) return;
  float acc = 0.0f;
  for (int s = 0; s < S; ++s) acc += (float)mask[((size_t)s * B + b) * DP + i];
  out[(size_t)b * DP + i] = (acc / (float)S) > 0.5f ? 1 : 0;
}

}

extern "C" int mvsn_soft_argmin(const float *cost, const float *idepth_samples, int n, int D, int pixels,
                                float *idepth, mvsn_stream_t stream) {
  MVSN_REQUIRE(cost && idepth_samples && idepth, MVSN_E_BADARG, "mvsn_soft_argmin: null pointer");
  MVSN_REQUIRE(n > 0 && D > 0 && pixels > 0 && n <= 65535, MVSN_E_BADARG, "mvsn_soft_argmin: bad sizes");
  hipLaunchKernelGGL(mvsn::soft_argmin_kernel, dim3((pixels + 255) / 256, n), dim3(256), 0, (hipStream_t)stream,
                     cost, idepth_samples, D, pixels, idepth);
  return mvsn::check_launch("mvsn_soft_argmin");
}

extern "C" int mvsn_soft_argmin_confidence(const float *cost, const float *idepth_samples, int n, int D, int pixels,
                                           float *idepth, float *confidence, mvsn_stream_t stream) {
  MVSN_REQUIRE(cost && idepth_samples && idepth && confidence, MVSN_E_BADARG, "mvsn_soft_argmin_confidence: null pointer");
  MVSN_REQUIRE(n > 0 && D > 0 && pixels > 0 && n <= 65535, MVSN_E_BADARG, "mvsn_soft_argmin_confidence: bad sizes");
  hipLaunchKernelGGL(mvsn::soft_argmin_confidence_kernel, dim3((pixels + 255) / 256, n), dim3(256), 0,
                     (hipStream_t)stream, cost, idepth_samples, D, pixels, idepth, confidence);
  return mvsn::check_launch("mvsn_soft_argmin_confidence");
}

extern "C" int mvsn_confidence_fuse_sources(const float *confidence, int n_sources, int batch, int pixels, float *out,
                                            mvsn_stream_t stream) {
  MVSN_REQUIRE(confidence && out, MVSN_E_BADARG, "mvsn_confidence_fuse_sources: null pointer");
  MVSN_REQUIRE(n_sources > 0 && batch > 0 && batch <= 65535 && pixels > 0, MVSN_E_BADARG,
               "mvsn_confidence_fuse_sources: bad sizes");
  hipLaunchKernelGGL(mvsn::confidence_fuse_kernel, dim3((pixels + 255) / 256, batch), dim3(256), 0, (hipStream_t)stream,
                     confidence, n_sources, batch, pixels, out);
  return mvsn::check_launch("mvsn_confidence_fuse_sources");
}

extern "C" int mvsn_confidence_mask(const float *confidence, const uint8_t *valid, long count, float min_confidence,
                                    uint8_t *out, mvsn_stream_t stream) {
  MVSN_REQUIRE(confidence && out, MVSN_E_BADARG, "mvsn_confidence_mask: null pointer");
  MVSN_REQUIRE(count > 0 && (count + 255) / 256 <= 2147483647L, MVSN_E_BADARG, "mvsn_confidence_mask: bad sizes");
  MVSN_REQUIRE(min_confidence == min_confidence, MVSN_E_BADARG, "mvsn_confidence_mask: the threshold is NaN");
  hipLaunchKernelGGL(mvsn::confidence_mask_kernel, dim3((unsigned)((count + 255) / 256)), dim3(256), 0,
                     (hipStream_t)stream, confidence, valid, count, min_confidence, out);
  return mvsn::check_launch("mvsn_confidence_mask");
}

namespace mvsn {
__global__ void gather_strided_kernel(const float *__restrict__ src, int count, long stride, float *__restrict__ dst) {
  const int i = blockIdx.x * blockDim.x + threadIdx.x;
  if (i < count) dst[i] = src[(size_t)i * stride];
}
}

namespace mvsn {
struct FocalSrc {
  const float *K[8];
};
__global__ void gather_focal_kernel(FocalSrc src, int levels, int batch, float *__restrict__ out, MVSN_VIS10) {
  const int i = blockIdx.x * blockDim.x + threadIdx.x;
  if (i < levels * batch) out[i] = src.K[i / batch][(size_t)(i % batch) * 16];
}
}

extern "C" int mvsn_gather_focal(const float *const *K_pyr, int levels, int batch, float *fx, mvsn_stream_t stream) {
  MVSN_REQUIRE(K_pyr && fx && levels >= 1 && levels <= 8 && batch > 0, MVSN_E_BADARG, "mvsn_gather_focal: bad arguments");
  mvsn::FocalSrc src = {};
  for (int l = 0; l < levels; ++l) {
    MVSN_REQUIRE(K_pyr[l], MVSN_E_BADARG, "mvsn_gather_focal: null pointer");
    src.K[l] = K_pyr[l];
  }
  const int total = levels * batch;
  hipLaunchKernelGGL(mvsn::gather_focal_kernel, dim3((total + 255) / 256), dim3(256), 0, (hipStream_t)stream, src, levels,
                     batch, fx, (const void *)src.K[0], (const void *)src.K[1], (const void *)src.K[2],
                     (const void *)src.K[3], (const void *)src.K[4], (const void *)src.K[5], (const void *)src.K[6],
                     (const void *)src.K[7], (const void *)nullptr, (const void *)nullptr);
  return mvsn::check_launch("mvsn_gather_focal");
}

extern "C" int mvsn_copy(void *dst, const void *src, size_t nbytes, mvsn_stream_t stream) {
  MVSN_REQUIRE(dst && src, MVSN_E_BADARG, "mvsn_copy: null pointer");
  if (nbytes == 0) return 0;
  hipError_t e = hipMemcpyAsync(dst, src, nbytes, hipMemcpyDeviceToDevice, (hipStream_t)stream);
  if (e != hipSuccess) {
    mvsn::set_error("mvsn_copy: %s", hipGetErrorString(e));
    return (int)e;
  }
  return 0;
}

namespace mvsn {
struct CopySizes {
  size_t n[8];
};
__global__ __launch_bounds__(256) void copy8_kernel(void *d0, const void *s0, void *d1, const void *s1, void *d2,
                                                    const void *s2, void *d3, const void *s3, void *d4, const void *s4,
                                                    void *d5, const void *s5, void *d6, const void *s6, void *d7,
                                                    const void *s7, CopySizes sz) {
  void *const d[8] = {d0, d1, d2, d3, d4, d5, d6, d7};
  const void *const s[8] = {s0, s1, s2, s3, s4, s5, s6, s7};
  const int k = blockIdx.y;
  char *dst = nullptr;
  const char *src = nullptr;
  size_t n = 0;
#pragma unroll
  for (int i = 0; i < 8; ++i)
    if (i == k) dst = (char *)d[i], src = (const char *)s[i], n = sz.n[i];
  const size_t stride = (size_t)gridDim.x * 256, t = (size_t)blockIdx.x * 256 + threadIdx.x;
  if ((((size_t)dst | (size_t)src | n) & 15) == 0) {
    for (size_t i = t; i < n / 16; i += stride) reinterpret_cast<uint4 *>(dst)[i] = reinterpret_cast<const uint4 *>(src)[i];
  } else {
    for (size_t i = t; i < n; i += stride) dst[i] = src[i];
  }
}
}

extern "C" int mvsn_copy_many(void *const *dst, const void *const *src, const size_t *nbytes, int count,
                              mvsn_stream_t stream) {
  MVSN_REQUIRE(count >= 0 && (count == 0 || (dst && src && nbytes)), MVSN_E_BADARG, "mvsn_copy_many: bad arguments");
  for (int at = 0; at < count; at += 8) {
    const int m = count - at < 8 ? count - at : 8;
    void *d[8] = {};
    const void *s[8] = {};
    mvsn::CopySizes sz = {};
    size_t largest = 0;
    for (int i = 0; i < m; ++i) {
      MVSN_REQUIRE(nbytes[at + i] == 0 || (dst[at + i] && src[at + i]), MVSN_E_BADARG, "mvsn_copy_many: null pointer");
      d[i] = dst[at + i], s[i] = src[at + i], sz.n[i] = nbytes[at + i];
      if (sz.n[i] > largest) largest = sz.n[i];
    }
    if (largest == 0) continue;
    size_t blocks = (largest / 16 + 255) / 256;
    blocks = blocks < 1 ? 1 : (blocks > 1024 ? 1024 : blocks);
    hipLaunchKernelGGL(mvsn::copy8_kernel, dim3((unsigned)blocks, m), dim3(256), 0, (hipStream_t)stream, d[0], s[0], d[1],
                       s[1], d[2], s[2], d[3], s[3], d[4], s[4], d[5], s[5], d[6], s[6], d[7], s[7], sz);
  }
  return mvsn::check_launch("mvsn_copy_many");
}

extern "C" int mvsn_gather_strided(const float *src, int count, long stride, float *dst, mvsn_stream_t stream) {
  MVSN_REQUIRE(src && dst && count > 0 && stride > 0, MVSN_E_BADARG, "mvsn_gather_strided: bad arguments");
  hipLaunchKernelGGL(mvsn::gather_strided_kernel, dim3((count + 255) / 256), dim3(256), 0, (hipStream_t)stream, src, count,
                     stride, dst);
  return mvsn::check_launch("mvsn_gather_strided");
}

extern "C" int mvsn_channel_l2_norm(const float *x, int n, int channels, long pixels, float *out,
                                    mvsn_stream_t stream) {
  MVSN_REQUIRE(x && out, MVSN_E_BADARG, "mvsn_channel_l2_norm: null pointer");
  MVSN_REQUIRE(n > 0 && n <= 65535 && channels > 0 && pixels > 0, MVSN_E_BADARG, "mvsn_channel_l2_norm: bad sizes");
  hipLaunchKernelGGL(mvsn::channel_l2_norm_kernel, dim3((unsigned)((pixels + 255) / 256), n), dim3(256), 0,
                     (hipStream_t)stream, x, channels, pixels, out);
  return mvsn::check_launch("mvsn_channel_l2_norm");
}

extern "C" int mvsn_idepth_scale(const float *prior, const float *fx, int n, long pixels, float *out,
                                 mvsn_stream_t stream) {
  MVSN_REQUIRE(prior && fx && out, MVSN_E_BADARG, "mvsn_idepth_scale: null pointer");
  MVSN_REQUIRE(n > 0 && n <= 65535 && pixels > 0, MVSN_E_BADARG, "mvsn_idepth_scale: bad sizes");
  hipLaunchKernelGGL(mvsn::idepth_gain_kernel<false>, dim3((unsigned)((pixels + 255) / 256), n), dim3(256), 0,
                     (hipStream_t)stream, prior, fx, (const float *)nullptr, pixels, out);
  return mvsn::check_launch("mvsn_idepth_scale");
}

extern "C" int mvsn_refiner_epilogue(const float *prior, const float *fx, const float *delta, int n, long pixels,
                                     float *out, mvsn_stream_t stream) {
  MVSN_REQUIRE(prior && fx && delta && out, MVSN_E_BADARG, "mvsn_refiner_epilogue: null pointer");
  MVSN_REQUIRE(n > 0 && n <= 65535 && pixels > 0, MVSN_E_BADARG, "mvsn_refiner_epilogue: bad sizes");
  hipLaunchKernelGGL(mvsn::idepth_gain_kernel<true>, dim3((unsigned)((pixels + 255) / 256), n), dim3(256), 0,
                     (hipStream_t)stream, prior, fx, delta, pixels, out);
  return mvsn::check_launch("mvsn_refiner_epilogue");
}

extern "C" int mvsn_upsample_bilinear(const float *in, int n, int channels, int rows_in, int cols_in, int rows_out,
                                      int cols_out, float *out, mvsn_stream_t stream) {
  MVSN_REQUIRE(in && out, MVSN_E_BADARG, "mvsn_upsample_bilinear: null pointer");
  MVSN_REQUIRE(n > 0 && channels > 0 && rows_in > 0 && cols_in > 0 && rows_out > 0 && cols_out > 0, MVSN_E_BADARG,
               "mvsn_upsample_bilinear: bad sizes");
  MVSN_REQUIRE((long)n * channels <= 65535 && rows_out <= 65535, MVSN_E_TOOLARGE, "mvsn_upsample_bilinear: grid");
  dim3 grid((cols_out + 255) / 256, rows_out, n * channels);
  hipLaunchKernelGGL((mvsn::upsample_kernel<float, float, false>), grid, dim3(256), 0, (hipStream_t)stream, in,
                     rows_in, cols_in, rows_out, cols_out, out);
  return mvsn::check_launch("mvsn_upsample_bilinear");
}

extern "C" int mvsn_upsample_prior(const float *in, const float *fx, int n, int rows_in, int cols_in, int rows_out,
                                   int cols_out, float *out, float *out_scaled, mvsn_stream_t stream) {
  MVSN_REQUIRE(in && fx && out && out_scaled, MVSN_E_BADARG, "mvsn_upsample_prior: null pointer");
  MVSN_REQUIRE(n > 0 && rows_in > 0 && cols_in > 0 && rows_out > 0 && cols_out > 0, MVSN_E_BADARG,
               "mvsn_upsample_prior: bad sizes");
  MVSN_REQUIRE(n <= 65535 && rows_out <= 65535, MVSN_E_TOOLARGE, "mvsn_upsample_prior: grid");
  dim3 grid((cols_out + 255) / 256, rows_out, n);
  hipLaunchKernelGGL(mvsn::upsample_gain_kernel, grid, dim3(256), 0, (hipStream_t)stream, in, fx, rows_in, cols_in,
                     rows_out, cols_out, out, out_scaled);
  return mvsn::check_launch("mvsn_upsample_prior");
}

extern "C" int mvsn_upsample_mask(const uint8_t *in, int n, int channels, int rows_in, int cols_in, int rows_out,
                                  int cols_out, uint8_t *out, mvsn_stream_t stream) {
  MVSN_REQUIRE(in && out, MVSN_E_BADARG, "mvsn_upsample_mask: null pointer");
  MVSN_REQUIRE(n > 0 && channels > 0 && rows_in > 0 && cols_in > 0 && rows_out > 0 && cols_out > 0, MVSN_E_BADARG,
               "mvsn_upsample_mask: bad sizes");
  const int groups_per_row = (cols_out + 15) / 16;
  const size_t total = (size_t)n * channels * rows_out * groups_per_row;
  MVSN_REQUIRE((total + 255) / 256 < 2147483647ull, MVSN_E_TOOLARGE, "mvsn_upsample_mask: grid");
  if (rows_out == 2 * rows_in && cols_out == 2 * cols_in && cols_in % 8 == 0 && (((size_t)in | (size_t)out) & 15) == 0) {
    const size_t groups = (size_t)n * channels * rows_in * (cols_in / 8);
    hipLaunchKernelGGL(mvsn::upsample_mask2x_kernel, dim3((unsigned)((groups + 255) / 256)), dim3(256), 0,
                       (hipStream_t)stream, in, rows_in, cols_in, cols_in / 8, groups, out);
    return mvsn::check_launch("mvsn_upsample_mask(2x)");
  }
  hipLaunchKernelGGL(mvsn::upsample_mask16_kernel, dim3((unsigned)((total + 255) / 256)), dim3(256), 0,
                     (hipStream_t)stream, in, rows_in, cols_in, rows_out, cols_out, groups_per_row, total, out);
  return mvsn::check_launch("mvsn_upsample_mask");
}

extern "C" int mvsn_area_downsample(const float *in, int n, int channels, int rows_in, int cols_in, float *out,
                                    mvsn_stream_t stream) {
  MVSN_REQUIRE(in && out, MVSN_E_BADARG, "mvsn_area_downsample: null pointer");
  MVSN_REQUIRE(n > 0 && channels > 0 && rows_in > 0 && cols_in > 0, MVSN_E_BADARG, "mvsn_area_downsample: bad sizes");
  const int rows_out = (rows_in + 1) / 2, cols_out = (cols_in + 1) / 2;
  MVSN_REQUIRE((long)n * channels <= 65535 && rows_out <= 65535, MVSN_E_TOOLARGE, "mvsn_area_downsample: grid");
  dim3 grid((cols_out + 255) / 256, rows_out, n * channels);
  hipLaunchKernelGGL(mvsn::area_downsample_kernel, grid, dim3(256), 0, (hipStream_t)stream, in, rows_in, cols_in,
                     rows_out, cols_out, out);
  return mvsn::check_launch("mvsn_area_downsample");
}

extern "C" int mvsn_fuse_sources(const float *raw, const float *refined, const float *baseline, const uint8_t *mask,
                                 int n_sources, int batch, int D, int pixels, int refined_aliases_raw,
                                 float *raw_out, float *refined_out, uint8_t *mask_out, mvsn_stream_t stream) {
  MVSN_REQUIRE(raw && baseline && mask && raw_out && refined_out && mask_out, MVSN_E_BADARG,
               "mvsn_fuse_sources: null pointer");
  MVSN_REQUIRE(refined || refined_aliases_raw, MVSN_E_BADARG, "mvsn_fuse_sources: refined is null");
  MVSN_REQUIRE(n_sources > 0 && batch > 0 && batch <= 65535 && D > 0 && pixels > 0, MVSN_E_BADARG,
               "mvsn_fuse_sources: bad sizes");
  hipLaunchKernelGGL(mvsn::fuse_idepth_kernel, dim3((pixels + 255) / 256, batch), dim3(256), 0, (hipStream_t)stream,
                     raw, refined, baseline, n_sources, batch, pixels, refined_aliases_raw, raw_out, refined_out);
  int rc = mvsn::check_launch("mvsn_fuse_sources(idepth)");
  if (rc) return rc;
  const size_t DP = (size_t)D * pixels;
  hipLaunchKernelGGL(mvsn::fuse_mask_kernel, dim3((unsigned)((DP + 255) / 256), batch), dim3(256), 0,
                     (hipStream_t)stream, mask, n_sources, batch, DP, mask_out);
  return mvsn::check_launch("mvsn_fuse_sources(mask)");
}

extern "C" int mvsn_fusion_gather(const float *maps, const int *view, const int *pixel, int n_views, long pixels_per_view,
                                  long count, float *out, mvsn_stream_t stream) {
  MVSN_REQUIRE(maps && view && pixel && out, MVSN_E_BADARG, "mvsn_fusion_gather: null pointer");
  MVSN_REQUIRE(n_views > 0 && pixels_per_view > 0 && pixels_per_view <= 2147483647L && count > 0 &&
                   (count + 255) / 256 <= 2147483647L,
               MVSN_E_BADARG, "mvsn_fusion_gather: bad sizes");
  hipLaunchKernelGGL(mvsn::gather_kernel<1>, dim3((unsigned)((count + 255) / 256)), dim3(256), 0, (hipStream_t)stream,
                     maps, view, pixel, n_views, pixels_per_view, count, out);
  return mvsn::check_launch("mvsn_fusion_gather");
}
```

multi_view_stereonet_amd/csrc/mvsn_warp.hip:

```cpp
#include "mvsn_common.h"

namespace mvsn {

__device__ __forceinline__ WarpCoord warp_coord_pinned(const float *H, float x, float y, float rows, float cols) {
  const float u0 = __builtin_fmaf(H[1], y, H[0] * x) + H[2];
  const float u1 = __builtin_fmaf(H[4], y, H[3] * x) + H[5];
  const float u2 = __builtin_fmaf(H[7], y, H[6] * x) + H[8];
  const float px = u0 / u2;
  const float py = u1 / u2;
  const float hx = px + 0.5f, hy = py + 0.5f;
  const float nx = (hx + hx) / cols - 1.0f;
  const float ny = (hy + hy) / rows - 1.0f;
  WarpCoord c;
  c.outside = (fabsf(nx) > 1.0f) || (fabsf(ny) > 1.0f);
  c.ix = __builtin_fmaf(nx + 1.0f, cols, -1.0f) * 0.5f;
  c.iy = __builtin_fmaf(ny + 1.0f, rows, -1.0f) * 0.5f;
  return c;
}

__device__ __forceinline__ float warp_blend(float ax, float ay, float bx, float by, float wa0, float wb0, float wa1,
                                            float wb1) {
  float t = ay * wb0;
  t = __builtin_fmaf(ax, wa0, t);
  t = __builtin_fmaf(bx, wa1, t);
  return __builtin_fmaf(by, wb1, t);
}

template <bool SPLIT>
__global__ __launch_bounds__(256) void homography_warp_kernel(const float *__restrict__ image,
                                                              const float *__restrict__ H, int h_bstride, int C,
                                                              int n_planes, int rows, int cols, int cgroups,
                                                              float *__restrict__ volume,
                                                              uint8_t *__restrict__ mask) {
  const int P = rows * cols;
#ifdef MVSN_WARP_NO_XCD_BANDS
  const int pbx = blockIdx.x;
#else
  const int pbx = xcd_tile_index(blockIdx.x, gridDim.x);
#endif
  const int cg = SPLIT ? blockIdx.x % cgroups : 0, pb = SPLIT ? blockIdx.x / cgroups : pbx;
  const int p = pb * blockDim.x + threadIdx.x;
  const int plane = blockIdx.y;
  const int b = blockIdx.z;
  if (p >= P) return;
  const int cper = (C + cgroups - 1) / cgroups;
  const int c_lo = SPLIT ? cg * cper : 0, c_hi = SPLIT ? (c_lo + cper < C ? c_lo + cper : C) : C;
  const float *Hp = H + (size_t)b * h_bstride + plane * 9;
  float Hl[9];
#pragma unroll
  for (int i = 0; i < 9; ++i) Hl[i] = Hp[i];
  const int y = p / cols, x = p - y * cols;
  WarpCoord c = warp_coord_pinned(Hl, (float)x, (float)y, (float)rows, (float)cols);
  Bilinear t = bilinear_taps(c.ix, c.iy, rows, cols);
  if (cg == 0) mask[((size_t)b * n_planes + plane) * P + p] = c.outside ? 1 : 0;
  const float keep = c.outside ? 0.0f : 1.0f;
  const float *img = image + (size_t)b * C * P;
  float *out = volume + (((size_t)b * C) * n_planes + plane) * P + p;
  if (cols >= 2) {
    const int xb = t.x0 < cols - 1 ? t.x0 : cols - 2;
    const bool sh = t.x0 != xb;
    const float wa0 = sh ? 0.0f : t.w00, wb0 = sh ? t.w00 : t.w01;
    const float wa1 = sh ? 0.0f : t.w10, wb1 = sh ? t.w10 : t.w11;
    const int r0 = t.y0 * cols + xb, r1 = t.y1 * cols + xb;
    typedef float f2u __attribute__((ext_vector_type(2), aligned(4)));
    for (int ch = c_lo; ch < c_hi; ++ch) {
      const float *ic = img + (size_t)ch * P;
      const f2u a = *reinterpret_cast<const f2u *>(ic + r0), bb = *reinterpret_cast<const f2u *>(ic + r1);
      const float v = warp_blend(a.x, a.y, bb.x, bb.y, wa0, wb0, wa1, wb1);
      __builtin_nontemporal_store(keep * v, out + (size_t)ch * n_planes * P);
    }
    return;
  }
  const int o00 = t.y0 * cols + t.x0, o01 = t.y0 * cols + t.x1, o10 = t.y1 * cols + t.x0, o11 = t.y1 * cols + t.x1;
  for (int ch = c_lo; ch < c_hi; ++ch) {
    const float *ic = img + (size_t)ch * P;
    float v = ic[o00] * t.w00 + ic[o01] * t.w01 + ic[o10] * t.w10 + ic[o11] * t.w11;
    out[(size_t)ch * n_planes * P] = keep * v;
  }
}

template <int PX>
__global__ __launch_bounds__(256) void homography_warp_px_kernel(const float *__restrict__ image,
                                                                 const float *__restrict__ H, int h_bstride, int C,
                                                                 int n_planes, int rows, int cols,
                                                                 float *__restrict__ volume, uint8_t *__restrict__ mask) {
  const int P = rows * cols, Q = P / PX;
  const int q = xcd_tile_index(blockIdx.x, gridDim.x) * blockDim.x + threadIdx.x;
  const int plane = blockIdx.y;
  const int b = blockIdx.z;
  if (q >= Q) return;
  const float *Hp = H + (size_t)b * h_bstride + plane * 9;
  float Hl[9];
#pragma unroll
  for (int i = 0; i < 9; ++i) Hl[i] = Hp[i];
  const int p = q * PX;
  const int y = p / cols, x = p - y * cols;
  int r0[PX], r1[PX];
  float wa0[PX], wb0[PX], wa1[PX], wb1[PX], keep[PX];
  unsigned mbits[PX / 4] = {};
#pragma unroll
  for (int k = 0; k < PX; ++k) {
    WarpCoord c = warp_coord_pinned(Hl, (float)(x + k), (float)y, (float)rows, (float)cols);
    Bilinear t = bilinear_taps(c.ix, c.iy, rows, cols);
    mbits[k >> 2] |= (c.outside ? 1u : 0u) << (8 * (k & 3));
    keep[k] = c.outside ? 0.0f : 1.0f;
    const int xb = t.x0 < cols - 1 ? t.x0 : cols - 2;
    const bool sh = t.x0 != xb;
    wa0[k] = sh ? 0.0f : t.w00, wb0[k] = sh ? t.w00 : t.w01;
    wa1[k] = sh ? 0.0f : t.w10, wb1[k] = sh ? t.w10 : t.w11;
    r0[k] = t.y0 * cols + xb, r1[k] = t.y1 * cols + xb;
  }
  unsigned *mp = reinterpret_cast<unsigned *>(mask + ((size_t)b * n_planes + plane) * P + p);
#pragma unroll
  for (int k = 0; k < PX / 4; ++k) mp[k] = mbits[k];
  const float *img = image + (size_t)b * C * P;
  float *out = volume + (((size_t)b * C) * n_planes + plane) * P + p;
  typedef float f2u __attribute__((ext_vector_type(2), aligned(4)));
  for (int ch = 0; ch < C; ++ch) {
    const float *ic = img + (size_t)ch * P;
#pragma unroll
    for (int k4 = 0; k4 < PX / 4; ++k4) {
      floatx4 v;
#pragma unroll
      for (int j = 0; j < 4; ++j) {
        const int k = k4 * 4 + j;
        const f2u a = *reinterpret_cast<const f2u *>(ic + r0[k]), bb = *reinterpret_cast<const f2u *>(ic + r1[k]);
        v[j] = keep[k] * warp_blend(a.x, a.y, bb.x, bb.y, wa0[k], wb0[k], wa1[k], wb1[k]);
      }
      __builtin_nontemporal_store(v, reinterpret_cast<floatx4 *>(out + (size_t)ch * n_planes * P + k4 * 4));
    }
  }
}

int warp_launch(const float *image, const float *H, int h_bstride, int batch, int channels, int n_planes, int rows,
                int cols, float *volume, uint8_t *mask, hipStream_t stream) {
  const int P = rows * cols;
  const long threads = (long)((P + 255) / 256) * 256 * n_planes * batch;
  int cgroups = 1;
  while (cgroups * 8 < channels && threads * cgroups < 4L * 64 * 4 * device_cus()) cgroups *= 2;
  dim3 grid((unsigned)((P + 255) / 256) * cgroups, n_planes, batch);
#ifndef MVSN_WARP_PX
#define MVSN_WARP_PX 4
#endif
  if (MVSN_WARP_PX && cgroups == 1 && cols % MVSN_WARP_PX == 0 && ((((size_t)volume | (size_t)mask) & 15) == 0) &&
      threads / MVSN_WARP_PX >= 16L * 64 * 4 * device_cus()) {
    constexpr int PX = MVSN_WARP_PX ? MVSN_WARP_PX : 4;
    hipLaunchKernelGGL(homography_warp_px_kernel<PX>, dim3((unsigned)((P / PX + 255) / 256), n_planes, batch), dim3(256), 0,
                       stream, image, H, h_bstride, channels, n_planes, rows, cols, volume, mask);
    return check_launch("mvsn_homography_warp");
  }
  if (cgroups > 1)
    hipLaunchKernelGGL(homography_warp_kernel<true>, grid, dim3(256), 0, stream, image, H, h_bstride, channels, n_planes,
                       rows, cols, cgroups, volume, mask);
  else
    hipLaunchKernelGGL(homography_warp_kernel<false>, grid, dim3(256), 0, stream, image, H, h_bstride, channels,
                       n_planes, rows, cols, 1, volume, mask);
  return check_launch("mvsn_homography_warp");
}

}

extern "C" int mvsn_homography_warp(const float *image, const float *H, int batch, int channels, int n_planes,
                                    int rows, int cols, float *volume, uint8_t *mask, mvsn_stream_t stream) {
  MVSN_REQUIRE(image && H && volume && mask, MVSN_E_BADARG, "mvsn_homography_warp: null pointer");
  MVSN_REQUIRE(batch > 0 && channels > 0 && n_planes > 0 && rows > 0 && cols > 0, MVSN_E_BADARG,
               "mvsn_homography_warp: bad sizes");
  MVSN_REQUIRE(n_planes <= 65535 && batch <= 65535, MVSN_E_TOOLARGE, "mvsn_homography_warp: grid too large");
  return mvsn::warp_launch(image, H, 9 * n_planes, batch, channels, n_planes, rows, cols, volume, mask,
                           (hipStream_t)stream);
}
```

multi_view_stereonet_amd/multi_view_stereonet.py:

```python
import ctypes
import threading
import warnings
from typing import Dict, List, Optional

import torch
import torch.nn as nn

from . import _native
from .params import REFINER_DILATIONS, build_parameter_tree

ListTensor = List[torch.Tensor]


class _Conv:

    def __init__(self, lib, weight: torch.Tensor, bias: Optional[torch.Tensor], stride: int = 1, dilation: int = 1):
        self.lib = lib
        self.cout, self.cin = int(weight.shape[0]), int(weight.shape[1])
        self.dims = weight.dim() - 2
        k = tuple(int(s) for s in weight.shape[2:])
        self.kd, self.kh, self.kw = (k if self.dims == 3 else (1,) + k)
        self.stride, self.dilation = stride, dilation
        self.bias = bias.detach().contiguous().float() if bias is not None else None
        self.weight = weight.detach().contiguous().float() if self.cout == 1 else None
# ... 347 lines not shown

    def cat0(self, parts) -> torch.Tensor:
        parts = [self.f32c(t) for t in parts]
        if len(parts) == 1:
            return parts[0]
        out = self.empty((sum(t.shape[0] for t in parts),) + tuple(parts[0].shape[1:]), torch.float32, parts[0].device)
        at = 0
        for t in parts:
            self.copy_into(out[at:at + t.shape[0]], t)
            at += t.shape[0]
        return out

    def focal(self, K: torch.Tensor) -> torch.Tensor:
        K = self.f32c(K)
        out = self.empty((K.shape[0],), torch.float32, K.device)
        self._call("mvsn_gather_strided", self.lib.mvsn_gather_strided, _native.ptr(K), K.shape[0], K[0].numel(),
                   _native.ptr(out), _native.stream())
        return out

    def _lvl(self) -> str:
        return f"[{self.level_tag.strip()}]" if self.level_tag else ""

    def _call(self, kernel: str, fn, *args, flops: float = 0.0, nbytes: float = 0.0):
        if self.timeline is None:
            _native.check(fn(*args), kernel)
            if self.recording is not None:
                self.recording.calls.append((fn, args[:-1], kernel))
            return
        a, b = torch.cuda.Event(enable_timing=True), torch.cuda.Event(enable_timing=True)
        a.record()
        _native.check(fn(*args), kernel)
        b.record()
        self.timeline.append((kernel, a, b, float(flops), float(nbytes)))

    def conv(self, c: _Conv, x: torch.Tensor, in_stats=None, in_norm: Optional[_Norm] = None, want_stats=False,
             in_residual: Optional[torch.Tensor] = None, write_staged: bool = False, carry: Optional["_Job"] = None,
             out: Optional[torch.Tensor] = None, prefer_fp32_wino: bool = False, lazy_stats: bool = False):
        lib = self.lib
        if isinstance(x, (list, tuple)):
            res = self.conv_blocks(c, x, want_stats, out=out) if (in_stats is None and in_residual is None and
                                                                  not write_staged) else None
            if res is not None:
                if carry is not None:
                    carry.run_alone(self)
                return res
            self._aten()
            x = torch.cat(list(x), 1)
        n = x.shape[0]
        depth = x.shape[2] if c.dims == 3 else 1
        rows, cols = x.shape[-2], x.shape[-1]
        d = c.desc(n, depth, rows, cols)
        packed = c.packed
        if self.conv_precision in ("bf16x3", "bf16", "bf16s") and c.packed_bx is not None and in_residual is None and \
                not write_staged and carry is None and not prefer_fp32_wino:
            dbx = c.desc(n, depth, rows, cols,
                         _native.CONV_BF16X3 if self.conv_precision == "bf16x3" else _native.CONV_BF16)
            if lib.mvsn_conv_bf16x3_supported(ctypes.byref(dbx)):
                d, packed = dbx, c.packed_bx
                self.bf16_layers += 1
        if d.precision == _native.CONV_FP32 and self.winograd and c.packed_wino is not None and in_residual is None and not write_staged and \
                (in_stats is None or self.winograd_with_input_transform) and \
                (c.dims == 2 or self.winograd_volume) and \
                (c.stride == 1 or (self.winograd_stride2 and in_stats is None and not want_stats and carry is None and
                                   self.conv_precision not in ("bf16", "bf16s"))):
            dwn = c.desc(n, depth, rows, cols, _native.CONV_FP32_WINO)
            if lib.mvsn_conv_winograd_supported(ctypes.byref(dwn)):
                d, packed = dwn, c.packed_wino
        ro, co = (rows - 1) // c.stride + 1, (cols - 1) // c.stride + 1
        shape = (n, c.cout, depth, ro, co) if c.dims == 3 else (n, c.cout, ro, co)
        if out is None:
            out = self.empty(shape, dtype=torch.float32, device=x.device)
        assert tuple(out.shape) == shape and out.is_contiguous()
        staged = self.empty(x.shape, x.dtype, x.device) if write_staged else None
        partials = None
        if want_stats:
            tiles = lib.mvsn_conv_num_tiles(ctypes.byref(d))
            partials = self.empty((n, tiles, 4, 3), dtype=torch.float32, device=x.device)
        taps = c.kd * c.kh * c.kw
        tag = (f"conv{c.dims}d k{c.kh}" + (f"s{c.stride}" if c.stride > 1 else "") +
               (f"d{c.dilation}" if c.dilation > 1 else "") + f" {c.cin}->{c.cout}" +
               (" bf16x3" if d.precision == _native.CONV_BF16X3 else "") +
               (" bf16" if d.precision == _native.CONV_BF16 else "") +
               (" wino" if d.precision == _native.CONV_FP32_WINO else "") + self.level_tag)
        nbytes = 4.0 * (x.numel() * (2 if in_residual is not None else 1) + out.numel() +
                        (staged.numel() if staged is not None else 0))
        if carry is not None:
            assert in_residual is None and not write_staged
            carried = ctypes.c_int(0)
            went = self._carried_before.get(tag, True)
            self._call("mvsn_conv_forward[" + tag + (" +pass]" if went else "] + pass"), lib.mvsn_conv_forward_carry, ctypes.byref(d),
                       _native.ptr(x), _native.ptr(packed), _native.ptr(c.bias), _native.ptr(in_stats),
                       _native.ptr(in_norm.gamma) if in_norm else None, _native.ptr(in_norm.beta) if in_norm else None,
                       _native.ptr(out), _native.ptr(partials), ctypes.byref(carry.job), ctypes.byref(carried),
                       _native.stream(), flops=2.0 * c.cin * taps * c.cout * out[:, 0].numel(),
                       nbytes=nbytes + carry.nbytes)
            self.carried_jobs += carried.value
            self._carried_before[tag] = bool(carried.value)
        else:
            self._call("mvsn_conv_forward[" + tag + "]", lib.mvsn_conv_forward, ctypes.byref(d), _native.ptr(x),
                       _native.ptr(packed), _native.ptr(c.bias), _native.ptr(in_stats),
                       _native.ptr(in_norm.gamma) if in_norm else None, _native.ptr(in_norm.beta) if in_norm else None,
                       _native.ptr(in_residual), _native.ptr(staged), _native.ptr(out), _native.ptr(partials),
                       _native.stream(), flops=2.0 * c.cin * taps * c.cout * out[:, 0].numel(), nbytes=nbytes)
        stats = None
        if want_stats:
            if (lazy_stats and n <= self.lazy_stats_max_samples and partials.shape[1] <= self.lazy_stats_max_records
                    and not (self.split_finalize and
                             self.lib.mvsn_groupnorm_finalize_split_workspace_bytes(n, partials.shape[1]))):
                stats = _Records(partials)
            else:
                stats = self.finalize_stats(partials)
        if write_staged:
            return out, stats, staged
        return out, stats

    def finalize_stats(self, partials: torch.Tensor) -> torch.Tensor:
        n, records = partials.shape[0], partials.shape[1]
        stats = self.empty((n, 4, 2), dtype=torch.float32, device=partials.device)
        ws_bytes = self.lib.mvsn_groupnorm_finalize_split_workspace_bytes(n, records) if self.split_finalize else 0
        if ws_bytes:
            ws = self.empty(ws_bytes, dtype=torch.uint8, device=partials.device)
            self._call("mvsn_groupnorm_finalize", self.lib.mvsn_groupnorm_finalize_split, _native.ptr(partials), n, records,
                       _native.ptr(stats), _native.ptr(ws), ws_bytes, _native.stream())
        else:
            self._call("mvsn_groupnorm_finalize", self.lib.mvsn_groupnorm_finalize, _native.ptr(partials), n, records,
                       _native.ptr(stats), _native.stream())
        return stats

    def conv_blocks(self, c: _Conv, blocks, want_stats=False, out: Optional[torch.Tensor] = None):
        lib = self.lib
        x0 = blocks[0]
        if not (self.winograd and self.cat_free_heads and c.packed_wino is not None and 1 <= len(blocks) <= 3
                and (self.conv_precision == "fp32" or c.packed_bx is None)
                and all(b.dtype == torch.float32 for b in blocks)):
            return None
        n, rows, cols = x0.shape[0], x0.shape[-2], x0.shape[-1]
        d = c.desc(n, 1, rows, cols, _native.CONV_FP32_WINO)
        if not lib.mvsn_conv_winograd_supported(ctypes.byref(d)) or sum(b.shape[1] for b in blocks) != c.cin:
            return None
        blocks = [self.dense(b) for b in blocks]
        if any(b.data_ptr() % 16 for b in blocks):
            return None
        if out is None:
            out = self.empty((n, c.cout, rows, cols), dtype=torch.float32, device=x0.device)
        assert tuple(out.shape) == (n, c.cout, rows, cols) and out.is_contiguous()
        partials = None
        if want_stats:
            partials = self.empty((n, lib.mvsn_conv_num_tiles(ctypes.byref(d)), 4, 3), dtype=torch.float32,
                                   device=x0.device)
        ptrs = (ctypes.c_void_p * len(blocks))(*[b.data_ptr() for b in blocks])
        chans = (ctypes.c_int * len(blocks))(*[b.shape[1] for b in blocks])
        self._keep(blocks)
        self._call(f"mvsn_conv_forward_blocks[conv2d k3 {c.cin}->{c.cout} wino{self.level_tag}]", lib.mvsn_conv_forward_blocks,
                   ctypes.byref(d), ptrs, chans, len(blocks), _native.ptr(c.packed_wino), _native.ptr(c.bias),
                   _native.ptr(out), _native.ptr(partials), _native.stream(),
                   flops=2.0 * c.cin * 9 * c.cout * out[:, 0].numel(),
                   nbytes=4.0 * (sum(b.numel() for b in blocks) + out.numel()))
        stats = None
        if want_stats:
            stats = self.finalize_stats(partials)
        return out, stats

    def conv_to1(self, c: _Conv, x: torch.Tensor, prior: Optional[torch.Tensor] = None,
                 fx: Optional[torch.Tensor] = None) -> Optional[torch.Tensor]:
        rows, cols = x.shape[-2], x.shape[-1]
        if c.cin != 32 or c.cout != 1 or c.dilation != 1 or c.stride != 1 or \
                not self.lib.mvsn_conv_to1_supported(rows, cols):
            return None
        n = x.shape[0]
        depth = x.shape[2] if c.dims == 3 else 1
        shape = (n, 1, depth, rows, cols) if c.dims == 3 else (n, 1, rows, cols)
        out = self.empty(shape, dtype=torch.float32, device=x.device)
        self._call(f"mvsn_conv_to1[{c.dims}d]", self.lib.mvsn_conv_to1, _native.ptr(x), _native.ptr(c.weight),
                   _native.ptr(c.bias), _native.ptr(prior), _native.ptr(fx), n, depth, rows, cols,
                   3 if c.dims == 3 else 1, _native.ptr(out), _native.stream(),
                   flops=2.0 * 32 * c.kd * 9 * out.numel(), nbytes=4.0 * (x.numel() + out.numel()))
        return out

    def residual_tower_unfused(self, x, first, blocks, final: _Conv, prior=None, fx=None):
        blocks = list(blocks)
        pend = None
        if first is not None:
            r0, st0 = self.conv(first[0], x, want_stats=True)
            if blocks and self.trim_tower_ends:
                pend = (r0, st0, first[1])
            else:
                x = self.gn_lrelu(r0, st0, first[1], out=r0)
        shp = x[0].shape if isinstance(x, (list, tuple)) else x.shape
        to1_ok = (final.cout == 1 and final.cin == 32 and final.dilation == 1 and final.stride == 1 and
                  final.dims == 2 and self.lib.mvsn_conv_to1_supported(shp[-2], shp[-1]))
        for i, (conv, norm) in enumerate(blocks):
            if pend is not None:
                r0, st0, n0 = pend
                r, st = self.conv(conv, r0, in_stats=st0, in_norm=n0, want_stats=True, lazy_stats=True)
            else:
                r, st = self.conv(conv, x, want_stats=True, lazy_stats=True)
            if i == len(blocks) - 1 and to1_ok and self.trim_tower_ends and pend is None:
                return self.conv_to1_block(final, r, st, norm, x, prior, fx), prior is not None
            if pend is not None:
                x = self.gn_lrelu_add2(r, st, norm, *pend, out=r)
                pend = None
            else:
                x = self.gn_lrelu(r, st, norm, residual=x, out=r)
        if final.cout == 1:
            out = self.conv_to1(final, x, prior, fx)
            if out is not None:
                return out, prior is not None
        out, _ = self.conv(final, x)
        return out, False

    def residual_tower_sliced(self, blocks_in, first, blocks, final: _Conv, prior, fx):
        n = blocks_in[0].shape[0]
        h = (n + 1) // 2
        bounds = ((0, h), (h, n))
        rows, cols = blocks_in[0].shape[-2], blocks_in[0].shape[-1]
        dev = blocks_in[0].device
        conv0, bn0 = first
        r0 = self.empty((n, 32, rows, cols), dtype=torch.float32, device=dev)
        st0 = [self.conv(conv0, [b[a:e] for b in blocks_in], want_stats=True, out=r0[a:e])[1] for a, e in bounds]
        x = [None, None]
        job = None
        last = len(blocks) - 1
        tails = []
        flip = 0
        for i, (conv, norm) in enumerate(blocks):
            r = self.empty((n, 32, rows, cols), dtype=torch.float32, device=dev)
            for s_, (a, e) in enumerate(bounds):
                if job is not None and self.carry_alternate:
                    job.job.reverse = flip
                flip ^= 1
                if i == 0:
                    _, st = self.conv(conv, r0[a:e], in_stats=st0[s_], in_norm=bn0, want_stats=True, carry=job,
                                      out=r[a:e], prefer_fp32_wino=True)
                else:
                    _, st = self.conv(conv, x[s_], want_stats=True, carry=job, out=r[a:e], prefer_fp32_wino=True)
                if i == last:
                    job = None
                    tails.append((r[a:e], st, norm, x[s_]))
                elif i == 0:
                    job = _Job(r[a:e], st, norm, r0[a:e], st0[s_], bn0)
                    x[s_] = r[a:e]
                else:
                    job = _Job(r[a:e], st, norm, x[s_])
                    x[s_] = r[a:e]
        out = self.empty((n, 1, rows, cols), dtype=torch.float32, device=dev)
        for (a, e), (r_, st, norm, x_) in zip(bounds, tails):
            self.conv_to1_block(final, r_, st, norm, x_, prior[a:e], fx[a:e], out=out[a:e])
        return out

    def gn_lrelu_add2(self, r, st, norm: _Norm, r0, st0, norm0: _Norm, out=None):
        n, spatial = r.shape[0], r[0, 0].numel()
        out = self.empty(r.shape, r.dtype, r.device) if out is None else out
        self._call("mvsn_groupnorm_lrelu_add2", self.lib.mvsn_groupnorm_lrelu_apply, _native.ptr(r), *_stats_arg(st),
                   _native.ptr(norm.gamma), _native.ptr(norm.beta), _native.ptr(r0), _native.ptr(st0),
                   _native.ptr(norm0.gamma), _native.ptr(norm0.beta), n, spatial, _native.ptr(out), _native.stream(),
                   nbytes=4.0 * r.numel() * 3)
        return out

    def conv_to1_block(self, c: _Conv, r, st, norm: _Norm, x, prior=None, fx=None, out=None):
        n, rows, cols = r.shape[0], r.shape[-2], r.shape[-1]
        if out is None:
            out = self.empty((n, 1, rows, cols), dtype=torch.float32, device=r.device)
        assert tuple(out.shape) == (n, 1, rows, cols) and out.is_contiguous()
        self._call("mvsn_conv_to1_block" + self._lvl(), self.lib.mvsn_conv_to1_block, _native.ptr(r), *_stats_arg(st),
                   _native.ptr(norm.gamma), _native.ptr(norm.beta), _native.ptr(x), _native.ptr(c.weight),
                   _native.ptr(c.bias), _native.ptr(prior), _native.ptr(fx), n, rows, cols, _native.ptr(out),
                   _native.stream(), flops=2.0 * 32 * 9 * out.numel(), nbytes=4.0 * (2 * r.numel() + out.numel()))
        return out

    def residual_tower(self, x, first, blocks, final: _Conv):
        if first is not None:
            conv0, bn0 = first
            r, st = self.conv(conv0, x, want_stats=True)
            pend = (r, st, bn0, None)
        else:
            pend = None
        cur = x
        for conv, norm in blocks:
            if pend is None:
                r, st = self.conv(conv, cur, want_stats=True)
            else:
                pr, pst, pnorm, pres = pend
                r, st, cur = self.conv(conv, pr, in_stats=pst, in_norm=pnorm, in_residual=pres, want_stats=True,
                                       write_staged=True)
            pend = (r, st, norm, cur)
        pr, pst, pnorm, pres = pend
        out, _ = self.conv(final, pr, in_stats=pst, in_norm=pnorm, in_residual=pres)
        return out

    def gn_lrelu(self, r: torch.Tensor, stats: torch.Tensor, norm: _Norm, residual: Optional[torch.Tensor] = None,
                 out: Optional[torch.Tensor] = None):
        n = r.shape[0]
        spatial = r[0, 0].numel()
        out = self.empty(r.shape, r.dtype, r.device) if out is None else out
        self._call("mvsn_groupnorm_lrelu_apply" + self._lvl(), self.lib.mvsn_groupnorm_lrelu_apply, _native.ptr(r),
                   *_stats_arg(stats), _native.ptr(norm.gamma), _native.ptr(norm.beta), _native.ptr(residual), None, None,
                   None, n, spatial, _native.ptr(out), _native.stream(),
                   nbytes=4.0 * r.numel() * (3 if residual is not None else 2))
        return out

    def use_towers(self) -> bool:
        return bool(self.towers and self.winograd and not self.fold_residual_blocks)

    def feature_network(self, image: torch.Tensor) -> List[torch.Tensor]:
        pyr = [image]
        x = image
        for i in range(3):
            x, _ = self.conv(self.fe_down[i], x)
            pyr.append(x)
        x, _ = self.conv(self.fe_down[3], x)
        if self.use_towers():
            feats = self.tower_extractor_tail(x)
            if feats is not None:
                pyr.append(feats)
                return pyr
        if self.fold_residual_blocks:
            pyr.append(self.residual_tower(x, None, self.fe_res, self.fe_final))
        else:
            pyr.append(self.residual_tower_unfused(x, None, self.fe_res, self.fe_final)[0])
        return pyr

    def cost_volume_filter(self, cost: torch.Tensor) -> torch.Tensor:
        n, _, depth, rows, cols = cost.shape
        to1 = bool(self.lib.mvsn_conv_to1_supported(rows, cols))
        if (self.carry_passes and self.carry_volume_passes and self.volume_materialise and self.winograd and self.winograd_volume and
                self.conv_precision == "fp32" and to1 and n >= 2 and (depth * rows * cols) % 256 == 0 and
                (n // 2) * 128 * depth * rows * cols >= self.carry_min_bytes):
            return self.cost_volume_filter_sliced(cost)
        if self.conv_precision == "bf16s":
            out = self.cost_volume_filter_bf16_storage(cost, to1)
            if out is not None:
                return out
        if cost.dtype != torch.float32:
            self._aten()
            cost = cost.float()
        mat = self.volume_materialise and self.winograd and self.winograd_volume and self.conv_precision == "fp32"
        x, st = self.conv(self.vf_convs[0], cost, want_stats=True, lazy_stats=mat)
        for i in range(1, 4):
            if mat:
                x = self.gn_lrelu(x, st, self.vf_norms[i - 1], out=x)
                x, st = self.conv(self.vf_convs[i], x, want_stats=True, lazy_stats=i < 3)
            else:
                x, st = self.conv(self.vf_convs[i], x, in_stats=st, in_norm=self.vf_norms[i - 1], want_stats=True)
        last = self.vf_convs[4]
        if to1:
            return self.conv_to1_volume_norm(last, x, st, self.vf_norms[3])
        out, _ = self.conv(last, x, in_stats=st, in_norm=self.vf_norms[3])
        return out[:, 0]

    def bf16_storage_supported(self, n: int, depth: int, rows: int, cols: int) -> bool:
        convs = self.vf_convs[:4]
        d = convs[0].desc(n, depth, rows, cols, _native.CONV_BF16)
        return (all(c.packed_bx is not None for c in convs) and bool(self.lib.mvsn_conv_bf16x3_supported(ctypes.byref(d)))
                and cols % 2 == 0)

    def cost_volume_filter_bf16_storage(self, cost: torch.Tensor, to1: bool) -> Optional[torch.Tensor]:
        n, _, depth, rows, cols = cost.shape
        lib = self.lib
        convs = self.vf_convs[:4]
        d = convs[0].desc(n, depth, rows, cols, _native.CONV_BF16)
        if not (to1 and self.bf16_storage_supported(n, depth, rows, cols)):
            return None
        tiles = lib.mvsn_conv_num_tiles(ctypes.byref(d))
        x, st = cost, None
        in16_0 = cost.dtype == torch.bfloat16
        for i, c in enumerate(convs):
            out16 = i < 3
            out = self.empty((n, 32, depth, rows, cols), dtype=torch.bfloat16 if out16 else torch.float32, device=cost.device)
            partials = self.empty((n, tiles, 4, 3), dtype=torch.float32, device=cost.device)
            nrm = self.vf_norms[i - 1] if i else None
            self._call("mvsn_conv_forward[conv3d k3 32->32 bf16 storage]", lib.mvsn_conv_forward_bf16_storage, ctypes.byref(d),
                       _native.ptr(x), 1 if (i or in16_0) else 0, _native.ptr(c.packed_bx), _native.ptr(c.bias), _native.ptr(st),
                       _native.ptr(nrm.gamma) if nrm else None, _native.ptr(nrm.beta) if nrm else None, _native.ptr(out),
                       1 if out16 else 0, _native.ptr(partials), _native.stream(),
                       flops=2.0 * 32 * 27 * 32 * out[:, 0].numel(),
                       nbytes=float(x.numel() * x.element_size() + out.numel() * out.element_size()))
            self.bf16_layers += 1
            st = self.finalize_stats(partials)
            x = out
        return self.conv_to1_volume_norm(self.vf_convs[4], x, st, self.vf_norms[3])

    def conv_to1_volume_norm(self, last: _Conv, x, st, nrm: _Norm, out=None):
        n, _, depth, rows, cols = x.shape
        if out is None:
            out = self.empty((n, depth, rows, cols), dtype=torch.float32, device=x.device)
        self._call("mvsn_conv_to1_volume_norm", self.lib.mvsn_conv_to1_volume_norm, _native.ptr(x), _native.ptr(st),
                   _native.ptr(nrm.gamma), _native.ptr(nrm.beta), _native.ptr(last.weight), _native.ptr(last.bias),
                   n, depth, rows, cols, _native.ptr(out), _native.stream(),
                   flops=2.0 * 32 * 27 * out.numel(), nbytes=4.0 * (x.numel() + out.numel()))
        return out

    def cost_volume_filter_sliced(self, cost: torch.Tensor) -> torch.Tensor:
        n, _, depth, rows, cols = cost.shape
        h = (n + 1) // 2
        bounds = ((0, h), (h, n))
        x = [cost[a:e] for a, e in bounds]
        job = None
        stats = [None, None]
        for i in range(4):
            r = self.empty((n, 32, depth, rows, cols), dtype=torch.float32, device=cost.device)
            for s_, (a, e) in enumerate(bounds):
                _, stats[s_] = self.conv(self.vf_convs[i], x[s_], want_stats=True, carry=job, out=r[a:e])
                job = _Job(r[a:e], stats[s_], self.vf_norms[i]) if i < 3 else None
                x[s_] = r[a:e]
        out = self.empty((n, depth, rows, cols), dtype=torch.float32, device=cost.device)
        for s_, (a, e) in enumerate(bounds):
            self.conv_to1_volume_norm(self.vf_convs[4], x[s_], stats[s_], self.vf_norms[3], out=out[a:e])
        return out

    def idepth_refiner(self, level: int, guide, prior: torch.Tensor, fx: torch.Tensor,
                       scaled: Optional[torch.Tensor] = None) -> torch.Tensor:
        self.level_tag = f" L{level}"
        try:
            return self._idepth_refiner(level, guide, prior, fx, scaled)
        finally:
            self.level_tag = ""

    def _idepth_refiner(self, level: int, guide, prior: torch.Tensor, fx: torch.Tensor,
                        scaled: Optional[torch.Tensor] = None) -> torch.Tensor:
        p = self.refiners[level]
        prior, fx = self.dense(prior), self.dense(fx)
        n, pixels = prior.shape[0], prior[0].numel()
        if scaled is None:
            scaled = self.empty(prior.shape, prior.dtype, prior.device)
            self._call("mvsn_idepth_scale", self.lib.mvsn_idepth_scale, _native.ptr(prior), _native.ptr(fx), n, pixels,
                       _native.ptr(scaled), _native.stream(), nbytes=8.0 * prior.numel())
        x_in = (list(guide) if isinstance(guide, (list, tuple)) else [guide]) + [scaled]
        rows, cols = prior.shape[-2], prior.shape[-1]
        if (self.carry_passes and not self.fold_residual_blocks and self.trim_tower_ends and n >= 2 and
                len(x_in) <= 3 and self.winograd and self.cat_free_heads and len(p["res"]) >= 2 and
                (n // 2) * 128 * rows * cols >= self.carry_min_bytes and (rows * cols) % 512 == 0 and
                all(b.dtype == torch.float32 and b.is_contiguous() for b in x_in) and
                self.lib.mvsn_conv_to1_supported(rows, cols) and p["final"].dilation == 1):
            return self.residual_tower_sliced(x_in, (p["conv0"], p["bn0"]), p["res"], p["final"], prior, fx)
        if self.fold_residual_blocks or len(x_in) > 3:
            self._aten()
            x_in = torch.cat(x_in, 1)
        if self.fold_residual_blocks:
            delta, done = self.residual_tower(x_in, (p["conv0"], p["bn0"]), p["res"], p["final"]), False
        else:
            delta, done = self.residual_tower_unfused(x_in, (p["conv0"], p["bn0"]), p["res"], p["final"],
                                                      prior=prior, fx=fx)
        if done:
            return delta
        out = self.empty(prior.shape, prior.dtype, prior.device)
        self._call("mvsn_refiner_epilogue", self.lib.mvsn_refiner_epilogue, _native.ptr(prior), _native.ptr(fx),
                   _native.ptr(self.dense(delta)), n, pixels, _native.ptr(out), _native.stream(),
                   nbytes=12.0 * prior.numel())
        return out

    def homography_warp(self, image: torch.Tensor, H: torch.Tensor, out: Optional[torch.Tensor] = None):
        B, C, rows, cols = image.shape
        n = H.shape[1]
        vol = self.empty((B, C, n, rows, cols), dtype=torch.float32, device=image.device) if out is None else out
        assert vol.shape == (B, C, n, rows, cols) and vol.is_contiguous()
        mask = self.empty((B, n, rows, cols), dtype=torch.bool, device=image.device)
        self._call("mvsn_homography_warp", self.lib.mvsn_homography_warp, _native.ptr(image), _native.ptr(H), B, C, n,
                   rows, cols, _native.ptr(vol), _native.ptr(mask), _native.stream(),
                   nbytes=4.0 * (image.numel() + vol.numel()) + mask.numel())
        return vol, mask

    def plane_sweep_setup(self, T: torch.Tensor, K0: torch.Tensor, K4: torch.Tensor, rows4: int, cols4: int, D: int):
        N, dev = T.shape[0], T.device
        f = dict(dtype=torch.float32, device=dev)
        samples = self.empty((N, D), **f)
        H4 = self.empty((N, D, 3, 3), **f)
        Hinc = self.empty((N, D, 3, 3), **f)
        H0 = self.empty((N, 1, 3, 3), **f)
        base = self.empty((N,), **f)
        self._call("mvsn_plane_sweep_setup", self.lib.mvsn_plane_sweep_setup, _native.ptr(T), _native.ptr(K0),
                   _native.ptr(K4), N, rows4, cols4, D, _native.ptr(samples), _native.ptr(H4), _native.ptr(Hinc),
                   _native.ptr(H0), _native.ptr(base), _native.stream())
        return samples, H4, Hinc, H0, base

    def plane_sweep_setup_sources(self, Ts, K0: torch.Tensor, K4: torch.Tensor, rows4: int, cols4: int, D: int):
        S = len(Ts)
        if S > 8:
            return self.plane_sweep_setup(self.cat0(list(Ts)), self.cat0([K0] * S), self.cat0([K4] * S), rows4, cols4, D)
        Ts = [self.f32c(t) for t in Ts]
        K0, K4 = self.f32c(K0), self.f32c(K4)
        B, dev = K0.shape[0], K0.device
        N = S * B
        f = dict(dtype=torch.float32, device=dev)
        samples, H4, Hinc = self.empty((N, D), **f), self.empty((N, D, 3, 3), **f), self.empty((N, D, 3, 3), **f)
        H0, base = self.empty((N, 1, 3, 3), **f), self.empty((N,), **f)
        ptrs = (ctypes.c_void_p * S)(*[_native.ptr(t) for t in Ts])
        self._keep(Ts)
        self._call("mvsn_plane_sweep_setup", self.lib.mvsn_plane_sweep_setup_sources, ptrs, S, _native.ptr(K0),
                   _native.ptr(K4), B, rows4, cols4, D, _native.ptr(samples), _native.ptr(H4), _native.ptr(Hinc),
                   _native.ptr(H0), _native.ptr(base), _native.stream())
        return samples, H4, Hinc, H0, base

    def focal_pyramid(self, K_pyr) -> torch.Tensor:
        Ks = [self.f32c(k) for k in K_pyr]
        L, B = len(Ks), Ks[0].shape[0]
        out = self.empty((L, B), torch.float32, Ks[0].device)
        if L > 8:
            for l in range(L):
                self.copy_into(out[l], self.focal(Ks[l]))
            return out
        ptrs = (ctypes.c_void_p * L)(*[_native.ptr(k) for k in Ks])
        self._keep(Ks)
        self._call("mvsn_gather_focal", self.lib.mvsn_gather_focal, ptrs, L, B, _native.ptr(out), _native.stream())
        return out

    def _keep(self, tensors):
        if self.recording is not None:
            self.recording.keep.extend(tensors)

    def incremental_cost_volume(self, src4, H4, Hinc, plane0, left_feats, want_features=False, cost_bf16=False):
        N, _, rows, cols = src4.shape
        B = left_feats.shape[0]
        D = H4.shape[1]
        dev = src4.device
        requested = {"auto": _native.CHAIN_AUTO, "direct": _native.CHAIN_DIRECT, "winograd": _native.CHAIN_WINOGRAD,
                     "stepwise": _native.CHAIN_STEPWISE, "banded": _native.CHAIN_BANDED}[self.chain_form]
        guarded = bool(cost_bf16 or self.banded_repair)
        out = (ctypes.c_size_t * 8)()

        def resolve(coresident_allowed):
            self.lib.mvsn_incremental_cost_volume_resolve(N, D, rows, cols, requested, int(coresident_allowed), int(guarded),
                                                          ctypes.byref(out))
            return int(out[0]), int(out[2]), int(out[3])
        form, ws_bytes, rws_bytes = resolve(True)
        if requested == _native.CHAIN_AUTO and form == _native.CHAIN_BANDED and not (
                self.banded_ok and not self.net_state.banded_latched and _native.coresident_right(dev.index)):
            form, ws_bytes, rws_bytes = resolve(False)
        if cost_bf16 and form == _native.CHAIN_STEPWISE:
            cost, mask, fvol = self.incremental_cost_volume(src4, H4, Hinc, plane0, left_feats, want_features)
            self._aten()
            self.last_cost_dtype = torch.bfloat16
            return cost.to(torch.bfloat16), mask, fvol
        cost = self.empty((N, 32, D, rows, cols), dtype=torch.bfloat16 if cost_bf16 else torch.float32, device=dev)
        mask = self.empty((N, D, rows, cols), dtype=torch.bool, device=dev)
        fvol = self.empty(cost.shape, torch.float32, dev) if want_features else None
        ws = self.empty(ws_bytes, dtype=torch.uint8, device=dev) if ws_bytes else None
        self.last_chain_form, self.last_chain_workspace, self.last_chain_shape = form, ws, (N, rows, cols)
        self.last_cost_dtype = cost.dtype
        P = rows * cols
        common = (_native.ptr(src4), _native.ptr(H4), _native.ptr(Hinc), _native.ptr(plane0), _native.ptr(left_feats),
                  _native.ptr(self.refiner_packed), N, B, D, rows, cols, _native.ptr(cost), _native.ptr(mask),
                  _native.ptr(fvol), _native.ptr(ws), ws_bytes, form)
        acct = dict(flops=N * (D - 1) * 2.0 * 9 * 32 * (35 + 32 + 32) * P,
                    nbytes=N * (4.0 * 67 * P + (64.0 if cost_bf16 else 128.0) * D * P + D * P))
        entry = self.lib.mvsn_incremental_cost_volume
        if cost_bf16 or (form == _native.CHAIN_BANDED and self.banded_repair):
            entry = self.lib.mvsn_incremental_cost_volume_bf16 if cost_bf16 else self.lib.mvsn_incremental_cost_volume_guarded
            rws = self.empty(rws_bytes, dtype=torch.uint8, device=dev) if rws_bytes else None
            common += (_native.ptr(rws), rws_bytes, self.net_state.status_ptr())
        self._call("mvsn_incremental_cost_volume", entry, *common, _native.stream(), **acct)
        return cost, mask, fvol

    def chain_status(self) -> int:
        if self.last_chain_form != _native.CHAIN_BANDED or self.last_chain_workspace is None:
            return 0
        ws = self.last_chain_workspace
        n, rows, cols = self.last_chain_shape
        off = self.lib.mvsn_incremental_cost_volume_status_offset(n, rows, cols)
        return int(ws[off:off + 4].view(torch.int32).item())

    def soft_argmin(self, cost: torch.Tensor, samples: torch.Tensor) -> torch.Tensor:
        N, D, rows, cols = cost.shape
        out = self.empty((N, 1, rows, cols), dtype=torch.float32, device=cost.device)
        self._call("mvsn_soft_argmin", self.lib.mvsn_soft_argmin, _native.ptr(self.dense(cost)), _native.ptr(samples),
                   N, D, rows * cols, _native.ptr(out), _native.stream(), nbytes=4.0 * (cost.numel() + out.numel()))
        return out

    def soft_argmin_confidence(self, cost: torch.Tensor, samples: torch.Tensor):
        N, D, rows, cols = cost.shape
        out = self.empty((N, 1, rows, cols), dtype=torch.float32, device=cost.device)
        conf = self.empty((N, 1, rows, cols), dtype=torch.float32, device=cost.device)
        self._call("mvsn_soft_argmin_confidence", self.lib.mvsn_soft_argmin_confidence, _native.ptr(self.dense(cost)),
                   _native.ptr(samples), N, D, rows * cols, _native.ptr(out), _native.ptr(conf), _native.stream(),
                   nbytes=4.0 * (cost.numel() + 2 * out.numel()))
        return out, conf

    def confidence_fuse_sources(self, conf: torch.Tensor, S: int, B: int) -> torch.Tensor:
        N, _, rows, cols = conf.shape
        assert N == S * B
        out = self.empty((B, 1, rows, cols), dtype=torch.float32, device=conf.device)
        self._call("mvsn_confidence_fuse_sources", self.lib.mvsn_confidence_fuse_sources, _native.ptr(self.dense(conf)),
                   S, B, rows * cols, _native.ptr(out), _native.stream(), nbytes=4.0 * (conf.numel() + out.numel()))
        return out

    def upsample(self, x: torch.Tensor, size) -> torch.Tensor:
        n, c, h, w = x.shape
        out = self.empty((n, c, int(size[0]), int(size[1])), dtype=torch.float32, device=x.device)
        self._call("mvsn_upsample_bilinear", self.lib.mvsn_upsample_bilinear, _native.ptr(x), n, c, h, w, int(size[0]),
                   int(size[1]), _native.ptr(out), _native.stream(), nbytes=4.0 * (x.numel() + out.numel()))
        return out

    def upsample_prior(self, x: torch.Tensor, fx: torch.Tensor, size):
        n, c, h, w = x.shape
        assert c == 1
        out = self.empty((n, 1, int(size[0]), int(size[1])), dtype=torch.float32, device=x.device)
        scaled = self.empty(out.shape, out.dtype, out.device)
        self._call("mvsn_upsample_prior", self.lib.mvsn_upsample_prior, _native.ptr(x), _native.ptr(fx), n, h, w,
                   int(size[0]), int(size[1]), _native.ptr(out), _native.ptr(scaled), _native.stream(),
                   nbytes=4.0 * (x.numel() + 2 * out.numel()))
        return out, scaled

    def upsample_mask(self, m: torch.Tensor, size) -> torch.Tensor:
        n, c, h, w = m.shape
        out = self.empty((n, c, int(size[0]), int(size[1])), dtype=torch.bool, device=m.device)
        self._call("mvsn_upsample_mask", self.lib.mvsn_upsample_mask, _native.ptr(m), n, c, h, w, int(size[0]),
                   int(size[1]), _native.ptr(out), _native.stream(), nbytes=float(m.numel() + out.numel()))
        return out

    def fuse_sources(self, raw, refined, baseline, mask, S, B, alias):
        N, D, rows, cols = mask.shape
        dev = raw.device
        raw_out = self.empty((B, 1, rows, cols), dtype=torch.float32, device=dev)
        ref_out = self.empty((B, 1, rows, cols), dtype=torch.float32, device=dev)
        mask_out = self.empty((B, D, rows, cols), dtype=torch.bool, device=dev)
        self._call("mvsn_fuse_sources", self.lib.mvsn_fuse_sources, _native.ptr(raw), _native.ptr(refined),
                   _native.ptr(baseline), _native.ptr(mask), S, B, D, rows * cols, 1 if alias else 0,
                   _native.ptr(raw_out), _native.ptr(ref_out), _native.ptr(mask_out), _native.stream(),
                   nbytes=float(mask.numel() + mask_out.numel()))
        return raw_out, ref_out, mask_out

    def forward(self, left_image_pyr, K_pyr, T_right_in_lefts, right_image_pyrs, D, do_filter, do_refiners,
                capture: Optional[dict] = None):
        S = len(T_right_in_lefts)
        left0 = self.f32c(left_image_pyr[0])
        B = left0.shape[0]
        rows4, cols4 = left_image_pyr[-1].shape[-2:]

        samples, H4, Hinc, H0, baseline = self.plane_sweep_setup_sources(T_right_in_lefts, K_pyr[0], K_pyr[-1], rows4,
                                                                         cols4, D)
        fx_all = self.focal_pyramid(K_pyr)

        frames = self.empty(((S + 1) * B,) + tuple(left0.shape[1:]), dtype=torch.float32, device=left0.device)
        self.copy_into(frames[:B], left0)
        for s_, pyr in enumerate(right_image_pyrs):
            self.homography_warp(self.f32c(pyr[0]), H0[s_ * B:(s_ + 1) * B],
                                 out=frames[(s_ + 1) * B:(s_ + 2) * B].unsqueeze(2))
        warped0 = frames[B:].unsqueeze(2)
        feats = self.feature_network(frames)
        left_feats = [f[:B] for f in feats]
        plane0 = feats[-1][B:]

        src4 = self.cat0([p[-1] for p in right_image_pyrs])
        cost16 = (self.conv_precision == "bf16s" and do_filter and capture is None and
                  bool(self.lib.mvsn_conv_to1_supported(rows4, cols4)) and self.bf16_storage_supported(S * B, D, rows4, cols4))
        cost, mask, fvol = self.incremental_cost_volume(src4, H4, Hinc, plane0, left_feats[-1],
                                                        want_features=capture is not None, cost_bf16=cost16)
        if do_filter:
            filtered = self.cost_volume_filter(cost)
        else:
            filtered = self.empty((cost.shape[0],) + tuple(cost.shape[2:]), dtype=torch.float32, device=cost.device)
            self._call("mvsn_channel_l2_norm", self.lib.mvsn_channel_l2_norm, _native.ptr(cost), cost.shape[0],
                       cost.shape[1], cost[0, 0].numel(), _native.ptr(filtered), _native.stream(),
                       nbytes=4.0 * (cost.numel() + filtered.numel()))
        want_conf = bool(self.confidence)
        if want_conf:
            raw, conf_chain = self.soft_argmin_confidence(filtered, samples)
        else:
            raw = self.soft_argmin(filtered, samples)

        if do_refiners[4]:
            refined = None
            if self.use_towers():
                refined = self.tower_refiner4(self.f32c(left_image_pyr[-1]), left_feats[-1], raw, fx_all[-1])
            if refined is None:
                img4 = self.cat0([left_image_pyr[-1]] * S)
                feats4 = self.cat0([left_feats[-1]] * S)
                fx4 = self.cat0([fx_all[-1]] * S)
                refined = self.idepth_refiner(4, [img4, feats4], raw, fx4)
        else:
            refined = None
        raw4, idepth4, mask4 = self.fuse_sources(raw, refined, baseline, mask, S, B, alias=refined is None)
        if capture is not None:
            capture.update(idepth_samples=samples, H=H4, H_inc=Hinc, H_lvl0_plane0=H0, baseline=baseline,
                           warped_fullres=warped0, left_features=left_feats, plane0_features=plane0,
                           cost_volume=cost, mask_volume=mask, feature_volume=fvol, filtered_cost=filtered,
                           raw_per_chain=raw)
            if want_conf:
                capture.update(confidence_per_chain=conf_chain)

        idepth = [None] * 5
        prior = [None] * 5
        masks = [None] * 5
        prior[4], idepth[4], masks[4] = raw4, idepth4, mask4
        conf = [None] * 5
        if want_conf:
            conf[4] = self.confidence_fuse_sources(conf_chain, S, B)
        for lvl in (3, 2, 1, 0):
            size = left_image_pyr[lvl].shape[-2:]
            if want_conf:
                conf[lvl] = self.upsample(conf[lvl + 1], size)
            if do_refiners[lvl]:
                fx = fx_all[lvl]
                prior[lvl], scaled = self.upsample_prior(idepth[lvl + 1], fx, size)
            else:
                prior[lvl] = self.upsample(idepth[lvl + 1], size)
            masks[lvl] = self.upsample_mask(masks[lvl + 1], size)
            if do_refiners[lvl]:
                img = self.f32c(left_image_pyr[lvl])
                guide = [img] if lvl == 0 else [img, left_feats[lvl]]
                idepth[lvl] = self.idepth_refiner(lvl, guide, prior[lvl], fx, scaled=scaled)
            else:
                idepth[lvl] = prior[lvl]
        out = {"left_idepthmap_pyr": idepth, "left_idepthmap_raw_pyr": prior, "left_idepthmap_mask_pyr": masks}
        if want_conf:
            out["left_confidence_pyr"] = conf
        return out


class MultiViewStereoNet(nn.Module):

    num_levels = 5

    def __init__(self):
        super().__init__()
        self.min_idepth = 0.0
        build_parameter_tree(self)
        self.options = EngineOptions()
        self._engine: Optional[PlaneSweepEngine] = None
        self._engine_key = None
        self.stream_lanes = 1
        self._lane_streams: List[torch.cuda.Stream] = []

    def __getstate__(self):
        state = self.__dict__.copy()
        state["_engine"], state["_engine_key"], state["_lane_streams"] = None, None, []
        state.pop("_plist", None)
        state.pop("_shared_state", None)
        state.pop("_lock", None)
        return state

    def __deepcopy__(self, memo):
        import copy
        new = self.__class__.__new__(self.__class__)
        memo[id(self)] = new
        for k, v in self.__getstate__().items():
            new.__dict__[k] = copy.deepcopy(v, memo)
        return new

    def _invalidate(self):
        self._engine = None
        self._engine_key = None
        self.__dict__.pop("_plist", None)

    def load_state_dict(self, *args, **kwargs):
        out = super().load_state_dict(*args, **kwargs)
        self._invalidate()
        return out

    def _apply(self, fn, *args, **kwargs):
        out = super()._apply(fn, *args, **kwargs)
        self._invalidate()
        return out

    def register_parameter(self, name, param):
        super().register_parameter(name, param)
        self.__dict__.pop("_plist", None)

    def refresh(self):
        self._invalidate()

    def check_device_status(self, synchronize: bool = True) -> int:
        eng = self._engine
        if eng is None:
            return 0
        if synchronize:
            torch.cuda.synchronize()
        fresh = eng.net_state.poll()
        if not self.options.banded_repair:
            status = eng.chain_status()
            if status:
                raise RuntimeError(
                    "mvsn_incremental_cost_volume(banded): inter-workgroup hand-off %d timed out -- the chain's workgroups "
                    "were not co-resident (is the device shared with other work?).  The outputs of that forward are "
                    "NaN; set net.options.banded_repair = True (the default) or net.options.chain_form = 'winograd'." % status)
        return fresh

    def reset_device_status(self):
        st = self.__dict__.get("_shared_state")
        if st is not None:
            st.rearm()

    def engine(self) -> PlaneSweepEngine:
        plist = self.__dict__.get("_plist")
        if plist is None:
            plist = self.__dict__["_plist"] = list(self.parameters())
        key = (sum(p._version for p in plist), tuple(p.data_ptr() for p in plist))
        self.__dict__["_plist_age"] = self.__dict__.get("_plist_age", 0) + 1
        if self.__dict__["_plist_age"] >= 16:
            self.__dict__["_plist_age"] = 0
            fresh = list(self.parameters())
            if len(fresh) != len(plist) or any(a is not b for a, b in zip(fresh, plist)):
                plist = self.__dict__["_plist"] = fresh
                key = (sum(p._version for p in plist), tuple(p.data_ptr() for p in plist))
                self._engine = None
        if self._engine is None or key != self._engine_key:
            self._engine = PlaneSweepEngine(self)
            self._engine_key = key
        return self._engine

    @torch.no_grad()
    def forward(self, left_image_pyr: ListTensor, K_pyr: ListTensor, T_right_in_lefts: ListTensor,
                right_image_pyrs: List[ListTensor], num_idepth_samples: int, do_cost_volume_filter: bool,
                do_refiners: List[bool], capture: Optional[dict] = None) -> Dict[str, List[Optional[torch.Tensor]]]:
        assert len(K_pyr) == self.num_levels
        assert len(left_image_pyr) == self.num_levels
        assert len(T_right_in_lefts) == len(right_image_pyrs) and len(T_right_in_lefts) >= 1
        assert len(do_refiners) == self.num_levels
        if not left_image_pyr[0].is_cuda:
            raise RuntimeError("MultiViewStereoNet (MI355X build) runs on HIP devices only: move the module and "
                               "its inputs to 'cuda'; there is no CPU implementation of the plane-sweep path")
        if next(self.parameters()).device != left_image_pyr[0].device:
            raise RuntimeError("module parameters and inputs are on different devices")
        lock = self.__dict__.get("_lock")
        if lock is None:
            lock = self.__dict__.setdefault("_lock", threading.RLock())
        with torch.cuda.device(left_image_pyr[0].device), lock:
            eng = self.engine()
            eng.net_state.poll()
            eng.net_state.tick()
            args = (int(num_idepth_samples), bool(do_cost_volume_filter), list(do_refiners))
            B = left_image_pyr[0].shape[0]
            lanes = min(self.stream_lanes, B) if capture is None else 1
            if lanes <= 1:
                S = len(T_right_in_lefts)
                if capture is None and eng.timeline is None and 0 < B * S <= self.options.plan_max_chains:
                    return self._forward_planned(eng, left_image_pyr, K_pyr, T_right_in_lefts, right_image_pyrs, args)
                return eng.forward(left_image_pyr, K_pyr, T_right_in_lefts, right_image_pyrs, *args, capture)
            return self._forward_lanes(eng, lanes, left_image_pyr, K_pyr, T_right_in_lefts, right_image_pyrs, args)

    def _forward_planned(self, eng, left_image_pyr, K_pyr, T_right_in_lefts, right_image_pyrs, args):
        S, L = len(T_right_in_lefts), len(left_image_pyr)
        flat = list(left_image_pyr) + list(K_pyr) + list(T_right_in_lefts) + [x for p in right_image_pyrs for x in p]
        opts = tuple(getattr(self.options, k) for k in EngineOptions.NAMES)
        key = (tuple((tuple(t.shape), t.dtype) for t in flat), S, args[0], args[1], tuple(args[2]), opts, eng.banded_ok,
               eng.net_state.banded_latched, torch.cuda.current_stream().cuda_stream)
        plan = eng.plans.get(key, False)

        def unflatten(ts):
            rp = ts[2 * L + S:]
            return ts[:L], ts[L:2 * L], ts[2 * L:2 * L + S], [rp[i * L:(i + 1) * L] for i in range(S)]

        if plan is None:
            return eng.forward(left_image_pyr, K_pyr, T_right_in_lefts, right_image_pyrs, *args, None)
        if plan is False:
            plan = ForwardPlan()
            plan.static_inputs = [t.detach().clone(memory_format=torch.contiguous_format) for t in flat]
            eng.recording = plan
            try:
                plan.outputs = eng.forward(*unflatten(plan.static_inputs), *args, None)
            finally:
                eng.recording = None
            plan.nbytes = sum(t.numel() * t.element_size() for t in plan.keep)
            plan.chain_info = (eng.last_chain_form, eng.last_chain_workspace, eng.last_chain_shape)
            while eng.plans and (len(eng.plans) >= 8 or plan.nbytes +
                                 sum(p.nbytes for p in eng.plans.values() if p is not None) > self.options.plan_max_bytes):
                eng.plans.pop(next(iter(eng.plans)))
            eng.plans[key] = plan if plan.replayable else None
            if not plan.replayable:
                plan.keep.clear()
        else:
            eng.copy_many(plan.static_inputs, flat)
            plan.uses += 1
            capturing = torch.cuda.is_current_stream_capturing()
            if plan.graph is None and self.options.plan_graph and plan.uses >= 2 and not capturing:
                try:
                    torch.cuda.synchronize()
                    g = torch.cuda.CUDAGraph()
                    with torch.cuda.graph(g):
                        plan.replay()
                    plan.graph = g
                except Exception:
                    plan.graph = False
            if plan.graph and not capturing:
                plan.graph.replay()
            else:
                plan.replay()
            eng.replays += 1
            eng.last_chain_form, eng.last_chain_workspace, eng.last_chain_shape = plan.chain_info
        out, news, olds = {}, [], []
        for k, lst in plan.outputs.items():
            out[k] = []
            for t in lst:
                if t is None:
                    out[k].append(None)
                    continue
                n = torch.empty_like(t)
                out[k].append(n)
                news.append(n)
                olds.append(t)
        eng.copy_many(news, olds)
        return out

    def _forward_lanes(self, eng, lanes, left_image_pyr, K_pyr, T_right_in_lefts, right_image_pyrs, args):
        B = left_image_pyr[0].shape[0]
        main = torch.cuda.current_stream()
        if len(self._lane_streams) < lanes:
            self._lane_streams = [torch.cuda.Stream() for _ in range(lanes)]
        bounds = [(B * i) // lanes for i in range(lanes + 1)]
        parts = []
        eng.banded_ok = False
        try:
            for i in range(lanes):
                lo, hi = bounds[i], bounds[i + 1]
                st = self._lane_streams[i]
                st.wait_stream(main)
                with torch.cuda.stream(st):
                    parts.append(eng.forward([x[lo:hi] for x in left_image_pyr], [k[lo:hi] for k in K_pyr],
                                             [t[lo:hi] for t in T_right_in_lefts],
                                             [[x[lo:hi] for x in p] for p in right_image_pyrs], *args, None))
        finally:
            eng.banded_ok = True
        out = {}
        for st in self._lane_streams[:lanes]:
            main.wait_stream(st)
        for key in parts[0]:
            out[key] = []
            for lvl in range(self.num_levels):
                pieces = [p[key][lvl] for p in parts]
                for t in pieces:
                    t.record_stream(main)
                out[key].append(torch.cat(pieces, 0))
        return out
```

Measured before the change: 3918 depthmaps/s.

## Batch source warps, read head conv from split frames, fuse mask pyramid

```diff
diff --git a/include/mvsn_hip.h b/include/mvsn_hip.h
--- a/include/mvsn_hip.h
+++ b/include/mvsn_hip.h
@@ -32,6 +32,8 @@
 
 int mvsn_homography_warp(const float *image, const float *H, int batch, int channels, int n_planes,
                          int rows, int cols, float *volume, uint8_t *mask, mvsn_stream_t stream);
+int mvsn_homography_warp_sources(const float *const *images, int n_sources, const float *H, int batch, int channels,
+                                 int n_planes, int rows, int cols, float *volume, uint8_t *mask, mvsn_stream_t stream);
 
 #define MVSN_CHAIN_AUTO 0
 #define MVSN_CHAIN_DIRECT 1
@@ -105,6 +107,9 @@
                       const float *bias, const float *in_stats, const float *in_gamma,
                       const float *in_beta, const float *in_residual, float *out_staged, float *out,
                       float *out_partials, mvsn_stream_t stream);
+int mvsn_conv_head_frames_supported(const mvsn_conv_desc *desc);
+int mvsn_conv_head_frames(const mvsn_conv_desc *desc, const float *in_first, int split, const float *in_rest,
+                          const float *weight_packed, const float *bias, float *out, mvsn_stream_t stream);
 int mvsn_conv_forward_blocks(const mvsn_conv_desc *desc, const float *const *in_blocks, const int *block_channels,
                              int num_blocks, const float *weight_packed, const float *bias, float *out,
                              float *out_partials, mvsn_stream_t stream);
@@ -160,6 +165,8 @@
                         float *out, float *out_scaled, mvsn_stream_t stream);
 int mvsn_upsample_mask(const uint8_t *in, int n, int channels, int rows_in, int cols_in, int rows_out,
                        int cols_out, uint8_t *out, mvsn_stream_t stream);
+int mvsn_upsample_mask_pyramid(const uint8_t *in, int n, int channels, int rows, int cols, int levels,
+                               uint8_t *const *out, mvsn_stream_t stream);
 
 int mvsn_area_downsample(const float *in, int n, int channels, int rows_in, int cols_in, float *out,
                          mvsn_stream_t stream);
diff --git a/multi_view_stereonet_amd/_native.py b/multi_view_stereonet_amd/_native.py
--- a/multi_view_stereonet_amd/_native.py
+++ b/multi_view_stereonet_amd/_native.py
@@ -40,6 +40,7 @@
     "mvsn_plane_sweep_setup_path": (c_int, [c_void_p, c_void_p, c_int, c_int]),
     "mvsn_gather_focal": (c_int, [POINTER(c_void_p), c_int, c_int, c_void_p, c_void_p]),
     "mvsn_homography_warp": (c_int, [c_void_p] * 2 + [c_int] * 5 + [c_void_p] * 2 + [c_void_p]),
+    "mvsn_homography_warp_sources": (c_int, [POINTER(c_void_p), c_int, c_void_p] + [c_int] * 5 + [c_void_p] * 2 + [c_void_p]),
     "mvsn_feature_refiner_packed_floats": (c_size_t, []),
     "mvsn_pack_feature_refiner": (c_int, [c_void_p] * 11 + [c_void_p]),
     "mvsn_incremental_cost_volume_workspace_bytes": (c_size_t, [c_int] * 3),
@@ -63,6 +64,8 @@
     "mvsn_conv_pack_weights": (c_int, [POINTER(ConvDesc), c_void_p, c_void_p, c_void_p]),
     "mvsn_conv_num_tiles": (c_int, [POINTER(ConvDesc)]),
     "mvsn_conv_forward": (c_int, [POINTER(ConvDesc)] + [c_void_p] * 10 + [c_void_p]),
+    "mvsn_conv_head_frames_supported": (c_int, [POINTER(ConvDesc)]),
+    "mvsn_conv_head_frames": (c_int, [POINTER(ConvDesc), c_void_p, c_int] + [c_void_p] * 4 + [c_void_p]),
     "mvsn_conv_forward_blocks": (c_int, [POINTER(ConvDesc), c_void_p, POINTER(c_int), c_int] + [c_void_p] * 4 + [c_void_p]),
     "mvsn_conv_forward_carry": (c_int, [POINTER(ConvDesc)] + [c_void_p] * 8 + [POINTER(ApplyJob), POINTER(c_int), c_void_p]),
     "mvsn_groupnorm_finalize": (c_int, [c_void_p, c_int, c_int, c_void_p, c_void_p]),
@@ -89,6 +92,7 @@
     "mvsn_upsample_bilinear": (c_int, [c_void_p] + [c_int] * 6 + [c_void_p, c_void_p]),
     "mvsn_upsample_prior": (c_int, [c_void_p, c_void_p] + [c_int] * 5 + [c_void_p] * 3),
     "mvsn_upsample_mask": (c_int, [c_void_p] + [c_int] * 6 + [c_void_p, c_void_p]),
+    "mvsn_upsample_mask_pyramid": (c_int, [c_void_p] + [c_int] * 5 + [POINTER(c_void_p), c_void_p]),
     "mvsn_image_pyramid_supported": (c_int, [c_int] * 3),
     "mvsn_image_pyramid": (c_int, [c_void_p] + [c_int] * 5 + [POINTER(c_void_p), c_void_p]),
     "mvsn_prepare_cameras": (c_int, [c_void_p] * 2 + [c_int] * 3 + [c_void_p] * 5 + [c_void_p]),
diff --git a/multi_view_stereonet_amd/csrc/mvsn_conv.hip b/multi_view_stereonet_amd/csrc/mvsn_conv.hip
--- a/multi_view_stereonet_amd/csrc/mvsn_conv.hip
+++ b/multi_view_stereonet_amd/csrc/mvsn_conv.hip
@@ -722,7 +722,8 @@
 #ifndef MVSN_HEAD_ST_AUX
 #define MVSN_HEAD_ST_AUX 0
 #endif
-__global__ __launch_bounds__(256, MVSN_HEAD_WGS_PER_CU) void conv5x5s2_head_kernel(const float *__restrict__ in, const float *__restrict__ wpk,
+__global__ __launch_bounds__(256, MVSN_HEAD_WGS_PER_CU) void conv5x5s2_head_kernel(const float *__restrict__ in, const float *__restrict__ in2,
+                                                             int split, const float *__restrict__ wpk,
                                                              const float *__restrict__ bias, int H, int W, int Ho,
                                                              int Wo, int ntx, int tiles, int total,
                                                              float *__restrict__ out) {
@@ -730,6 +731,7 @@
   const int tid = threadIdx.x, lane = tid & 63;
   const int wave = __builtin_amdgcn_readfirstlane(tid >> 6);
   const size_t plane = (size_t)H * W;
+  const float *in2s = in2 - (size_t)split * 3 * plane;
 
   const int kk = lane >> 4, cl = lane & 15;
   float wf[HD_KSTEPS][2];
@@ -761,7 +763,7 @@
     const int n = id / tiles, t = id - n * tiles;
     const int tyi = t / ntx, txi = t - tyi * ntx;
     const int org = 2 * (tyi * HD_TY) * W + 2 * (txi * HD_TX), x2 = 2 * (txi * HD_TX);
-    const float *inn = in + (size_t)n * 3 * plane;
+    const float *inn = (n < split ? in : in2s) + (size_t)n * 3 * plane;
 #pragma unroll
     for (int i = 0; i < NP; ++i) {
       const int pc = wave + 4 * i;
@@ -1021,7 +1023,7 @@
     else if constexpr (F.kind == CV_HEAD) {
       MVSN_REQUIRE((long long)g.tiles * g.n < (1ll << 31) - 65536, MVSN_E_TOOLARGE, "mvsn_conv_forward: batch too large for one launch");
       const int total = g.tiles * g.n, gx = std::min(total, MVSN_HEAD_WGS_PER_CU * device_cus());
-      hipLaunchKernelGGL(conv5x5s2_head_kernel, dim3(gx), dim3(256), 0, (hipStream_t)stream, in, weight_packed, bias, g.H, g.W,
+      hipLaunchKernelGGL(conv5x5s2_head_kernel, dim3(gx), dim3(256), 0, (hipStream_t)stream, in, in, g.n, weight_packed, bias, g.H, g.W,
                          g.Ho, g.Wo, g.ntx, g.tiles, total, out);
       return check_launch("mvsn_conv_forward(5x5 stride-2 head)");
     } else {
@@ -1037,6 +1039,32 @@
       else return run(conv_mfma_kernel<F.npt, F.kd, F.kh, F.kh, F.stride, F.se, CT, MODE == 2, F.v4>, "mvsn_conv_forward");
     }
   });
+}
+
+extern "C" int mvsn_conv_head_frames_supported(const mvsn_conv_desc *desc) {
+  mvsn::ConvGeom g;
+  return desc && desc->precision == MVSN_CONV_FP32 && mvsn::make_geom(desc, &g) && mvsn::conv_head_ok(g, 0, true) ? 1 : 0;
+}
+
+extern "C" int mvsn_conv_head_frames(const mvsn_conv_desc *desc, const float *in_first, int split, const float *in_rest,
+                                     const float *weight_packed, const float *bias, float *out, mvsn_stream_t stream) {
+  using namespace mvsn;
+  MVSN_REQUIRE(desc && weight_packed && out, MVSN_E_BADARG, "mvsn_conv_head_frames: null pointer");
+  MVSN_REQUIRE(mvsn_conv_head_frames_supported(desc), MVSN_E_BADARG, "mvsn_conv_head_frames: layer or shape has no head form");
+  ConvGeom g;
+  make_geom(desc, &g);
+  MVSN_REQUIRE(split >= 0 && split <= g.n, MVSN_E_BADARG, "mvsn_conv_head_frames: split outside 0..n");
+  MVSN_REQUIRE((split == 0 || in_first) && (split == g.n || in_rest), MVSN_E_BADARG, "mvsn_conv_head_frames: null pointer");
+  if (split == 0) in_first = in_rest;
+  if (split == g.n) in_rest = in_first;
+  MVSN_REQUIRE((((size_t)in_first | (size_t)in_rest | (size_t)out) & 15) == 0, MVSN_E_BADARG,
+               "mvsn_conv_head_frames: 16-byte aligned tensors");
+  MVSN_REQUIRE(g.n <= 65535, MVSN_E_TOOLARGE, "mvsn_conv_head_frames: batch too large for one launch");
+  MVSN_REQUIRE((long long)g.tiles * g.n < (1ll << 31) - 65536, MVSN_E_TOOLARGE, "mvsn_conv_head_frames: batch too large for one launch");
+  const int total = g.tiles * g.n, gx = std::min(total, MVSN_HEAD_WGS_PER_CU * device_cus());
+  hipLaunchKernelGGL(conv5x5s2_head_kernel, dim3(gx), dim3(256), 0, (hipStream_t)stream, in_first, in_rest, split, weight_packed,
+                     bias, g.H, g.W, g.Ho, g.Wo, g.ntx, g.tiles, total, out);
+  return check_launch("mvsn_conv_head_frames");
 }
 
 extern "C" int mvsn_debug_conv_plan(const mvsn_conv_desc *desc, int mode, int out[8]) {
diff --git a/multi_view_stereonet_amd/csrc/mvsn_misc.hip b/multi_view_stereonet_amd/csrc/mvsn_misc.hip
--- a/multi_view_stereonet_amd/csrc/mvsn_misc.hip
+++ b/multi_view_stereonet_amd/csrc/mvsn_misc.hip
@@ -252,6 +252,52 @@
   uint8_t *dst = out + (rowid * 2) * (size_t)(win * 2) + gx * 16;
   __builtin_nontemporal_store(o, reinterpret_cast<u32x4 *>(dst));
   __builtin_nontemporal_store(o, reinterpret_cast<u32x4 *>(dst + win * 2));
+}
+
+struct MaskLevels {
+  uint8_t *out[8];
+};
+__global__ __launch_bounds__(256) void upsample_mask_pyramid_kernel(const uint8_t *__restrict__ in, int win,
+                                                                    int groups_per_row, size_t total_groups, int levels,
+                                                                    MaskLevels lv, MVSN_VIS10) {
+  __shared__ uint2 src[256];
+  const size_t g0 = (size_t)blockIdx.x * 256;
+  __shared__ int2 pos[256];
+  if (g0 + threadIdx.x < total_groups) {
+    src[threadIdx.x] = *reinterpret_cast<const uint2 *>(in + (g0 + threadIdx.x) * 8);
+    const size_t rowid = (g0 + threadIdx.x) / groups_per_row;
+    pos[threadIdx.x] = make_int2((int)rowid, (int)(g0 + threadIdx.x - rowid * groups_per_row));
+  }
+  __syncthreads();
+  typedef unsigned u32x4 __attribute__((ext_vector_type(4)));
+#pragma unroll 1
+  for (int l = 1; l <= levels; ++l) {
+    uint8_t *out = lv.out[0];
+#pragma unroll
+    for (int i = 1; i < 8; ++i)
+      if (i == l - 1) out = lv.out[i];
+    const int f = 1 << l, kb = l - 1;
+    const size_t wout = (size_t)win << l;
+    for (int idx = threadIdx.x; idx < (256 << kb) * f; idx += 256) {
+      const int k = idx & ((1 << kb) - 1), gl = (idx >> kb) & 255, r = idx >> (kb + 8);
+      if (g0 + gl >= total_groups) continue;
+      const uint2 w = src[gl];
+      u32x4 o;
+      if (l == 1) {
+        o[0] = __builtin_amdgcn_perm(w.x, w.x, 0x01010000u);
+        o[1] = __builtin_amdgcn_perm(w.x, w.x, 0x03030202u);
+        o[2] = __builtin_amdgcn_perm(w.y, w.y, 0x01010000u);
+        o[3] = __builtin_amdgcn_perm(w.y, w.y, 0x03030202u);
+      } else {
+        const unsigned long long ww = ((unsigned long long)w.y << 32) | w.x;
+#pragma unroll
+        for (int i = 0; i < 4; ++i) o[i] = (unsigned)((ww >> (8 * ((16 * k + 4 * i) >> l))) & 0xffu) * 0x01010101u;
+      }
+      const int2 at = pos[gl];
+      uint8_t *dst = out + (((size_t)at.x << l) + r) * wout + ((size_t)at.y * 8 << l) + 16 * k;
+      __builtin_nontemporal_store(o, reinterpret_cast<u32x4 *>(dst));
+    }
+  }
 }
 
 __global__ __launch_bounds__(256) void area_downsample_kernel(const float *__restrict__ in, int hin, int win,
@@ -515,6 +561,40 @@
   return mvsn::check_launch("mvsn_upsample_mask");
 }
 
+extern "C" int mvsn_upsample_mask_pyramid(const uint8_t *in, int n, int channels, int rows, int cols, int levels,
+                                          uint8_t *const *out, mvsn_stream_t stream) {
+  MVSN_REQUIRE(in && out, MVSN_E_BADARG, "mvsn_upsample_mask_pyramid: null pointer");
+  MVSN_REQUIRE(n > 0 && channels > 0 && rows > 0 && cols > 0 && levels >= 1 && levels <= 8, MVSN_E_BADARG,
+               "mvsn_upsample_mask_pyramid: bad sizes");
+  size_t align = (size_t)in;
+  for (int l = 0; l < levels; ++l) {
+    MVSN_REQUIRE(out[l], MVSN_E_BADARG, "mvsn_upsample_mask_pyramid: null pointer");
+    align |= (size_t)out[l];
+  }
+  const size_t in_rows = (size_t)n * channels * rows;
+  MVSN_REQUIRE(((long long)rows << levels) <= 2147483647ll && ((long long)cols << levels) <= 2147483647ll, MVSN_E_TOOLARGE,
+               "mvsn_upsample_mask_pyramid: level size");
+  if (cols % 8 != 0 || (align & 15) != 0 || in_rows > 2147483647ull) {
+    const uint8_t *from = in;
+    for (int l = 0; l < levels; ++l) {
+      if (int rc = mvsn_upsample_mask(from, n, channels, rows << l, cols << l, rows << (l + 1), cols << (l + 1), out[l], stream))
+        return rc;
+      from = out[l];
+    }
+    return 0;
+  }
+  const size_t groups = in_rows * (cols / 8);
+  MVSN_REQUIRE((groups + 255) / 256 < 2147483647ull, MVSN_E_TOOLARGE, "mvsn_upsample_mask_pyramid: grid");
+  mvsn::MaskLevels lv = {};
+  for (int l = 0; l < 8; ++l) lv.out[l] = out[l < levels ? l : 0];
+  hipLaunchKernelGGL(mvsn::upsample_mask_pyramid_kernel, dim3((unsigned)((groups + 255) / 256)), dim3(256), 0,
+                     (hipStream_t)stream, in, cols, cols / 8, groups, levels, lv, (const void *)lv.out[0],
+                     (const void *)lv.out[1], (const void *)lv.out[2], (const void *)lv.out[3], (const void *)lv.out[4],
+                     (const void *)lv.out[5], (const void *)lv.out[6], (const void *)lv.out[7], (const void *)nullptr,
+                     (const void *)nullptr);
+  return mvsn::check_launch("mvsn_upsample_mask_pyramid");
+}
+
 extern "C" int mvsn_area_downsample(const float *in, int n, int channels, int rows_in, int cols_in, float *out,
                                     mvsn_stream_t stream) {
   MVSN_REQUIRE(in && out, MVSN_E_BADARG, "mvsn_area_downsample: null pointer");
diff --git a/multi_view_stereonet_amd/csrc/mvsn_warp.hip b/multi_view_stereonet_amd/csrc/mvsn_warp.hip
--- a/multi_view_stereonet_amd/csrc/mvsn_warp.hip
+++ b/multi_view_stereonet_amd/csrc/mvsn_warp.hip
@@ -27,11 +27,9 @@
 }
 
 template <bool SPLIT>
-__global__ __launch_bounds__(256) void homography_warp_kernel(const float *__restrict__ image,
-                                                              const float *__restrict__ H, int h_bstride, int C,
-                                                              int n_planes, int rows, int cols, int cgroups,
-                                                              float *__restrict__ volume,
-                                                              uint8_t *__restrict__ mask) {
+__device__ __forceinline__ void warp_pixel(const float *__restrict__ img, int b, const float *__restrict__ H, int h_bstride,
+                                           int C, int n_planes, int rows, int cols, int cgroups,
+                                           float *__restrict__ volume, uint8_t *__restrict__ mask) {
   const int P = rows * cols;
 #ifdef MVSN_WARP_NO_XCD_BANDS
   const int pbx = blockIdx.x;
@@ -41,7 +39,6 @@
   const int cg = SPLIT ? blockIdx.x % cgroups : 0, pb = SPLIT ? blockIdx.x / cgroups : pbx;
   const int p = pb * blockDim.x + threadIdx.x;
   const int plane = blockIdx.y;
-  const int b = blockIdx.z;
   if (p >= P) return;
   const int cper = (C + cgroups - 1) / cgroups;
   const int c_lo = SPLIT ? cg * cper : 0, c_hi = SPLIT ? (c_lo + cper < C ? c_lo + cper : C) : C;
@@ -54,7 +51,6 @@
   Bilinear t = bilinear_taps(c.ix, c.iy, rows, cols);
   if (cg == 0) mask[((size_t)b * n_planes + plane) * P + p] = c.outside ? 1 : 0;
   const float keep = c.outside ? 0.0f : 1.0f;
-  const float *img = image + (size_t)b * C * P;
   float *out = volume + (((size_t)b * C) * n_planes + plane) * P + p;
   if (cols >= 2) {
     const int xb = t.x0 < cols - 1 ? t.x0 : cols - 2;
@@ -79,15 +75,23 @@
   }
 }
 
+template <bool SPLIT>
+__global__ __launch_bounds__(256) void homography_warp_kernel(const float *__restrict__ image,
+                                                              const float *__restrict__ H, int h_bstride, int C,
+                                                              int n_planes, int rows, int cols, int cgroups,
+                                                              float *__restrict__ volume,
+                                                              uint8_t *__restrict__ mask) {
+  const int b = blockIdx.z;
+  warp_pixel<SPLIT>(image + (size_t)b * C * rows * cols, b, H, h_bstride, C, n_planes, rows, cols, cgroups, volume, mask);
+}
+
 template <int PX>
-__global__ __launch_bounds__(256) void homography_warp_px_kernel(const float *__restrict__ image,
-                                                                 const float *__restrict__ H, int h_bstride, int C,
-                                                                 int n_planes, int rows, int cols,
-                                                                 float *__restrict__ volume, uint8_t *__restrict__ mask) {
+__device__ __forceinline__ void warp_pixels(const float *__restrict__ img, int b, const float *__restrict__ H, int h_bstride,
+                                            int C, int n_planes, int rows, int cols, float *__restrict__ volume,
+                                            uint8_t *__restrict__ mask) {
   const int P = rows * cols, Q = P / PX;
   const int q = xcd_tile_index(blockIdx.x, gridDim.x) * blockDim.x + threadIdx.x;
   const int plane = blockIdx.y;
-  const int b = blockIdx.z;
   if (q >= Q) return;
   const float *Hp = H + (size_t)b * h_bstride + plane * 9;
   float Hl[9];
@@ -113,7 +117,6 @@
   unsigned *mp = reinterpret_cast<unsigned *>(mask + ((size_t)b * n_planes + plane) * P + p);
 #pragma unroll
   for (int k = 0; k < PX / 4; ++k) mp[k] = mbits[k];
-  const float *img = image + (size_t)b * C * P;
   float *out = volume + (((size_t)b * C) * n_planes + plane) * P + p;
   typedef float f2u __attribute__((ext_vector_type(2), aligned(4)));
   for (int ch = 0; ch < C; ++ch) {
@@ -130,6 +133,34 @@
       __builtin_nontemporal_store(v, reinterpret_cast<floatx4 *>(out + (size_t)ch * n_planes * P + k4 * 4));
     }
   }
+}
+
+template <int PX>
+__global__ __launch_bounds__(256) void homography_warp_px_kernel(const float *__restrict__ image,
+                                                                 const float *__restrict__ H, int h_bstride, int C,
+                                                                 int n_planes, int rows, int cols,
+                                                                 float *__restrict__ volume, uint8_t *__restrict__ mask) {
+  const int b = blockIdx.z;
+  warp_pixels<PX>(image + (size_t)b * C * rows * cols, b, H, h_bstride, C, n_planes, rows, cols, volume, mask);
+}
+
+struct WarpSources {
+  const float *image[8];
+};
+template <int PX>
+__global__ __launch_bounds__(256) void homography_warp_sources_kernel(WarpSources src, int batch,
+                                                                      const float *__restrict__ H, int h_bstride, int C,
+                                                                      int n_planes, int rows, int cols,
+                                                                      float *__restrict__ volume,
+                                                                      uint8_t *__restrict__ mask, MVSN_VIS10) {
+  const int n = blockIdx.z, s = n / batch;
+  const float *img = src.image[0];
+#pragma unroll
+  for (int i = 1; i < 8; ++i)
+    if (i == s) img = src.image[i];
+  img += (size_t)(n - s * batch) * C * rows * cols;
+  if constexpr (PX == 1) warp_pixel<false>(img, n, H, h_bstride, C, n_planes, rows, cols, 1, volume, mask);
+  else warp_pixels<PX>(img, n, H, h_bstride, C, n_planes, rows, cols, volume, mask);
 }
 
 int warp_launch(const float *image, const float *H, int h_bstride, int batch, int channels, int n_planes, int rows,
@@ -158,6 +189,50 @@
   return check_launch("mvsn_homography_warp");
 }
 
+int warp_sources_launch(const float *const *images, int n_sources, const float *H, int batch, int channels, int n_planes,
+                        int rows, int cols, float *volume, uint8_t *mask, hipStream_t stream) {
+  const int P = rows * cols, N = n_sources * batch, h_bstride = 9 * n_planes;
+  const long threads = (long)((P + 255) / 256) * 256 * n_planes * N;
+  if (channels > 8 && threads < 4L * 64 * 4 * device_cus()) {
+    for (int s = 0; s < n_sources; ++s)
+      if (int rc = warp_launch(images[s], H + (size_t)s * batch * h_bstride, h_bstride, batch, channels, n_planes, rows, cols,
+                               volume + (size_t)s * batch * channels * n_planes * P, mask + (size_t)s * batch * n_planes * P, stream))
+        return rc;
+    return 0;
+  }
+  WarpSources src = {};
+  for (int s = 0; s < 8; ++s) src.image[s] = images[s < n_sources ? s : 0];
+  auto run = [&](auto kern, unsigned gx) {
+    hipLaunchKernelGGL(kern, dim3(gx, n_planes, N), dim3(256), 0, stream, src, batch, H, h_bstride, channels, n_planes, rows,
+                       cols, volume, mask, (const void *)src.image[0], (const void *)src.image[1], (const void *)src.image[2],
+                       (const void *)src.image[3], (const void *)src.image[4], (const void *)src.image[5],
+                       (const void *)src.image[6], (const void *)src.image[7], (const void *)nullptr,
+                       (const void *)nullptr);
+    return check_launch("mvsn_homography_warp_sources");
+  };
+  if (MVSN_WARP_PX && cols % MVSN_WARP_PX == 0 && ((((size_t)volume | (size_t)mask) & 15) == 0) &&
+      threads / MVSN_WARP_PX >= 16L * 64 * 4 * device_cus()) {
+    constexpr int PX = MVSN_WARP_PX ? MVSN_WARP_PX : 4;
+    return run(homography_warp_sources_kernel<PX>, (unsigned)((P / PX + 255) / 256));
+  }
+  return run(homography_warp_sources_kernel<1>, (unsigned)((P + 255) / 256));
+}
+
+}
+
+extern "C" int mvsn_homography_warp_sources(const float *const *images, int n_sources, const float *H, int batch,
+                                            int channels, int n_planes, int rows, int cols, float *volume, uint8_t *mask,
+                                            mvsn_stream_t stream) {
+  MVSN_REQUIRE(images && H && volume && mask, MVSN_E_BADARG, "mvsn_homography_warp_sources: null pointer");
+  MVSN_REQUIRE(n_sources >= 1 && n_sources <= 8, MVSN_E_BADARG, "mvsn_homography_warp_sources: 1..8 sources");
+  for (int s = 0; s < n_sources; ++s)
+    MVSN_REQUIRE(images[s], MVSN_E_BADARG, "mvsn_homography_warp_sources: null pointer");
+  MVSN_REQUIRE(batch > 0 && channels > 0 && n_planes > 0 && rows > 0 && cols > 0, MVSN_E_BADARG,
+               "mvsn_homography_warp_sources: bad sizes");
+  MVSN_REQUIRE(n_planes <= 65535 && (long)batch * n_sources <= 65535, MVSN_E_TOOLARGE,
+               "mvsn_homography_warp_sources: grid too large");
+  return mvsn::warp_sources_launch(images, n_sources, H, batch, channels, n_planes, rows, cols, volume, mask,
+                                   (hipStream_t)stream);
 }
 
 extern "C" int mvsn_homography_warp(const float *image, const float *H, int batch, int channels, int n_planes,
diff --git a/multi_view_stereonet_amd/multi_view_stereonet.py b/multi_view_stereonet_amd/multi_view_stereonet.py
--- a/multi_view_stereonet_amd/multi_view_stereonet.py
+++ b/multi_view_stereonet_amd/multi_view_stereonet.py
@@ -673,10 +673,34 @@
     def use_towers(self) -> bool:
         return bool(self.towers and self.winograd and not self.fold_residual_blocks)
 
-    def feature_network(self, image: torch.Tensor) -> List[torch.Tensor]:
-        pyr = [image]
-        x = image
-        for i in range(3):
+    def head_frames_ok(self, n: int, rows: int, cols: int) -> bool:
+        c = self.fe_down[0]
+        return bool(c.packed_bx is None and c.packed_wino is None and
+                    self.lib.mvsn_conv_head_frames_supported(ctypes.byref(c.desc(n, 1, rows, cols))))
+
+    def conv_head_frames(self, first: torch.Tensor, rest: torch.Tensor, c: Optional[_Conv] = None) -> torch.Tensor:
+        c = self.fe_down[0] if c is None else c
+        n, (rows, cols) = first.shape[0] + rest.shape[0], first.shape[-2:]
+        assert first.shape[1:] == rest.shape[1:] and first.is_contiguous() and rest.is_contiguous()
+        d = c.desc(n, 1, rows, cols)
+        out = self.empty((n, c.cout, (rows - 1) // 2 + 1, (cols - 1) // 2 + 1), dtype=torch.float32, device=first.device)
+        self._call(f"mvsn_conv_forward[conv2d k{c.kh}s2 {c.cin}->{c.cout}{self.level_tag}]", self.lib.mvsn_conv_head_frames,
+                   ctypes.byref(d), _native.ptr(first) if first.shape[0] else None, first.shape[0],
+                   _native.ptr(rest) if rest.shape[0] else None, _native.ptr(c.packed),
+                   _native.ptr(c.bias), _native.ptr(out), _native.stream(),
+                   flops=2.0 * c.cin * c.kh * c.kw * c.cout * out[:, 0].numel(),
+                   nbytes=4.0 * (first.numel() + rest.numel() + out.numel()))
+        return out
+
+    def feature_network(self, image) -> List[torch.Tensor]:
+        if isinstance(image, tuple):
+            pyr = [image[0]]
+            x = self.conv_head_frames(*image)
+        else:
+            pyr = [image]
+            x, _ = self.conv(self.fe_down[0], image)
+        pyr.append(x)
+        for i in range(1, 3):
             x, _ = self.conv(self.fe_down[i], x)
             pyr.append(x)
         x, _ = self.conv(self.fe_down[3], x)
@@ -829,6 +853,25 @@
         self._call("mvsn_homography_warp", self.lib.mvsn_homography_warp, _native.ptr(image), _native.ptr(H), B, C, n,
                    rows, cols, _native.ptr(vol), _native.ptr(mask), _native.stream(),
                    nbytes=4.0 * (image.numel() + vol.numel()) + mask.numel())
+        return vol, mask
+
+    def homography_warp_sources(self, images, H: torch.Tensor):
+        S = len(images)
+        B, C, rows, cols = images[0].shape
+        n = H.shape[1]
+        vol = self.empty((S * B, C, n, rows, cols), dtype=torch.float32, device=H.device)
+        mask = self.empty((S * B, n, rows, cols), dtype=torch.bool, device=H.device)
+        acct = dict(nbytes=4.0 * (S * images[0].numel() + vol.numel()) + mask.numel())
+        if S > 8:
+            for s_, img in enumerate(images):
+                self._call("mvsn_homography_warp", self.lib.mvsn_homography_warp, _native.ptr(img),
+                           _native.ptr(H[s_ * B:(s_ + 1) * B]), B, C, n, rows, cols, _native.ptr(vol[s_ * B:(s_ + 1) * B]),
+                           _native.ptr(mask[s_ * B:(s_ + 1) * B]), _native.stream(), nbytes=acct["nbytes"] / S)
+            return vol, mask
+        ptrs = (ctypes.c_void_p * S)(*[_native.ptr(t) for t in images])
+        self._keep(list(images))
+        self._call("mvsn_homography_warp", self.lib.mvsn_homography_warp_sources, ptrs, S, _native.ptr(H), B, C, n, rows,
+                   cols, _native.ptr(vol), _native.ptr(mask), _native.stream(), **acct)
         return vol, mask
 
     def plane_sweep_setup(self, T: torch.Tensor, K0: torch.Tensor, K4: torch.Tensor, rows4: int, cols4: int, D: int):
@@ -978,6 +1021,17 @@
                    int(size[1]), _native.ptr(out), _native.stream(), nbytes=float(m.numel() + out.numel()))
         return out
 
+    def upsample_mask_pyramid(self, m: torch.Tensor, sizes) -> Optional[List[torch.Tensor]]:
+        n, c, h, w = m.shape
+        if not (1 <= len(sizes) <= 8 and m.is_contiguous() and
+                all((int(s[0]), int(s[1])) == (h << (l + 1), w << (l + 1)) for l, s in enumerate(sizes))):
+            return None
+        outs = [self.empty((n, c, int(s[0]), int(s[1])), dtype=torch.bool, device=m.device) for s in sizes]
+        ptrs = (ctypes.c_void_p * len(outs))(*[_native.ptr(o) for o in outs])
+        self._call("mvsn_upsample_mask", self.lib.mvsn_upsample_mask_pyramid, _native.ptr(m), n, c, h, w, len(outs), ptrs,
+                   _native.stream(), nbytes=float(m.numel() + sum(o.numel() for o in outs)))
+        return outs
+
     def fuse_sources(self, raw, refined, baseline, mask, S, B, alias):
         N, D, rows, cols = mask.shape
         dev = raw.device
@@ -1001,13 +1055,18 @@
                                                                          cols4, D)
         fx_all = self.focal_pyramid(K_pyr)
 
-        frames = self.empty(((S + 1) * B,) + tuple(left0.shape[1:]), dtype=torch.float32, device=left0.device)
-        self.copy_into(frames[:B], left0)
-        for s_, pyr in enumerate(right_image_pyrs):
-            self.homography_warp(self.f32c(pyr[0]), H0[s_ * B:(s_ + 1) * B],
-                                 out=frames[(s_ + 1) * B:(s_ + 2) * B].unsqueeze(2))
-        warped0 = frames[B:].unsqueeze(2)
-        feats = self.feature_network(frames)
+        rights0 = [self.f32c(pyr[0]) for pyr in right_image_pyrs]
+        if (self.head_frames_ok((S + 1) * B, left0.shape[-2], left0.shape[-1]) and left0.data_ptr() % 16 == 0 and
+                all(r.shape == left0.shape for r in rights0)):
+            warped0, _ = self.homography_warp_sources(rights0, H0)
+            feats = self.feature_network((left0, warped0.squeeze(2)))
+        else:
+            frames = self.empty(((S + 1) * B,) + tuple(left0.shape[1:]), dtype=torch.float32, device=left0.device)
+            self.copy_into(frames[:B], left0)
+            for s_, r in enumerate(rights0):
+                self.homography_warp(r, H0[s_ * B:(s_ + 1) * B], out=frames[(s_ + 1) * B:(s_ + 2) * B].unsqueeze(2))
+            warped0 = frames[B:].unsqueeze(2)
+            feats = self.feature_network(frames)
         left_feats = [f[:B] for f in feats]
         plane0 = feats[-1][B:]
 
@@ -1056,6 +1115,9 @@
         conf = [None] * 5
         if want_conf:
             conf[4] = self.confidence_fuse_sources(conf_chain, S, B)
+        pyr_masks = self.upsample_mask_pyramid(mask4, [left_image_pyr[lvl].shape[-2:] for lvl in (3, 2, 1, 0)])
+        if pyr_masks is not None:
+            masks[3], masks[2], masks[1], masks[0] = pyr_masks
         for lvl in (3, 2, 1, 0):
             size = left_image_pyr[lvl].shape[-2:]
             if want_conf:
@@ -1065,7 +1127,8 @@
                 prior[lvl], scaled = self.upsample_prior(idepth[lvl + 1], fx, size)
             else:
                 prior[lvl] = self.upsample(idepth[lvl + 1], size)
-            masks[lvl] = self.upsample_mask(masks[lvl + 1], size)
+            if pyr_masks is None:
+                masks[lvl] = self.upsample_mask(masks[lvl + 1], size)
             if do_refiners[lvl]:
                 img = self.f32c(left_image_pyr[lvl])
                 guide = [img] if lvl == 0 else [img, left_feats[lvl]]
```

Measured after the change: 3922 depthmaps/s (median of 6 runs). No clear change (+0.1%).
